# Makiato1999/HRI-EMO

Measured on AMD Instinct MI355X. Metric: utterances/sec fwd+bwd, d=768 T_a=400 T_t=128 N_e=6, higher is better.
Workload: dtype bf16; 1 GPU; FusionWithEmotionDecoder fwd+bwd (train mode, dropout 0.1), d=768 T_a=400 T_t=128 N_e=6 H=8, 2 fusion + 2 decoder layers, all-False masks (BASELINE cfg2); global_batch=64, batch_per_gpu=64, parallelism=dp1, grad_allreduce=none, launch=hipGraph replay, streams=2

## Files before the change

hri-emo_amd/__init__.py:

```python
from . import _lib
from .models.cross_modal_block_tacfn import CrossModalBlock, CrossModalTransformer
from .models.beta_gate_tacfn import BetaGate
from .models.emotion_decoder import EmotionDecoder, ExplainableDecoderLayer
from .models.fusion_with_emotion_decoder import FusionWithEmotionDecoder
from .models.mosei_fusion_with_emotion_decoder import MoseiFusionWithEmotionDecoder
from .models.fusion_classifier import FusionClassifier

from .dp import EvalStep
from ._ops import set_gemm_mode, gemm_mode, enable_fused_wgrad, set_precision, precision, set_varlen, varlen, set_varlen_maps, varlen_maps, set_mfma_maps, mfma_maps, set_ingest, ingest, set_pooled_gate_fp32, pooled_gate_fp32

__all__ = ["EvalStep", "set_gemm_mode", "gemm_mode", "enable_fused_wgrad", "set_precision", "precision", "set_varlen", "varlen", "set_varlen_maps", "varlen_maps", "set_mfma_maps", "mfma_maps", "set_ingest", "ingest", "set_pooled_gate_fp32", "pooled_gate_fp32", "CrossModalBlock", "CrossModalTransformer", "BetaGate", "EmotionDecoder", "ExplainableDecoderLayer",
           "FusionWithEmotionDecoder", "MoseiFusionWithEmotionDecoder", "FusionClassifier"]
```

hri-emo_amd/_lib.py:

```python
import ctypes
import os

_HERE = os.path.dirname(os.path.abspath(__file__))
LIB_PATH = os.environ.get("HRIEMO_LIB") or os.path.join(_HERE, "libhriemo.so")

_C = {"p": ctypes.c_void_p, "i": ctypes.c_int, "l": ctypes.c_long, "f": ctypes.c_float,
      "Q": ctypes.c_ulonglong, "I": ctypes.c_uint}

_SIGS = {
    "hriemo_gemm_bf16": ("iiiiiplplplipipliplp", "i"),
    "hriemo_gemm_force_config": ("i", "i"),
    "hriemo_gemm_debug_flags": ("i", "i"),
    "hriemo_gemm_colsum_rows": ("iiiii", "i"),
    "hriemo_gemm_plan": ("iiiiiilppp", "i"),
    "hriemo_gemm_bf16_group_tn": ("piip", "i"),
    "hriemo_gemm_bf16_split": ("iiiiiplplplpliiplp", "i"),
    "hriemo_gemm_bf16_colsum": ("iiiiiplplplplpp", "i"),
    "hriemo_mx8_scale_ld": ("i", "l"),
    "hriemo_quant_mx8": ("pliiiplplp", "i"),
    "hriemo_gemm_mx8": ("iiiplplplplplipiplp", "i"),
    "hriemo_gemm_mx8_q": ("iiiplplplplplpiplplp", "i"),
    "hriemo_gemm_mx8_force_config": ("i", "i"),
    "hriemo_attn_fwd": ("plplplplppiiiiifQpIipp", "i"),
    "hriemo_attn_fwd_q": ("plplplplppiiiiifQpIipplplp", "i"),
# ... 10 lines not shown
    "hriemo_attn_plan": ("iiiiiipppppp", "i"),
    "hriemo_split_bf16x3": ("pliipiip", "i"),
    "hriemo_attn_fwd_f32": ("plplplplppiiiiifQpIip", "i"),
    "hriemo_attn_probs_f32": ("plplpppiiiiifQpIip", "i"),
    "hriemo_add_ln_f32": ("ppppppiiffQpIlp", "i"),
    "hriemo_dropout_f32": ("ppliipfQpIlp", "i"),
    "hriemo_masked_mean_f32": ("pppiiip", "i"),
    "hriemo_gate_input_f32": ("pppiip", "i"),
    "hriemo_sigmoid_beta_f32": ("pppiip", "i"),
    "hriemo_fuse_f32": ("ppipippiiip", "i"),
    "hriemo_split3_f32": ("pliipiiplp", "i"),
    "hriemo_colsum_f32_workspace_bytes": ("ii", "l"),
    "hriemo_colsum_f32": ("pliiplpipp", "i"),
    "hriemo_add_ln_bwd_f32_workspace_bytes": ("ii", "l"),
    "hriemo_add_ln_bwd_f32": ("pppppppppiiiffQpIlpp", "i"),
    "hriemo_attn_bwd_f32": ("plplplplplppplplplpiiiiifQpIip", "i"),
    "hriemo_gate_dpre_f32": ("ppipipppiiip", "i"),
    "hriemo_gate_input_bwd_f32": ("pppppiip", "i"),
    "hriemo_gate_dy_f32": ("ppipppiiiip", "i"),
    "hriemo_rowdot_bwd_f32": ("ppppppiiip", "i"),
    "hriemo_attn_fwd_f32_varlen": ("plplplplpppiiiiifQpIip", "i"),
    "hriemo_attn_bwd_f32_varlen": ("plplplplplpppplplplpiiiiifQpIip", "i"),
    "hriemo_add_ln_f32_rows": ("ppppppiiffQpIlpp", "i"),
    "hriemo_add_ln_bwd_f32_rows": ("pppppppppiiiffQpIlppp", "i"),
    "hriemo_masked_mean_f32_packed": ("ppipiiip", "i"),
    "hriemo_fuse_f32_packed": ("pppiippiipppiiiip", "i"),
    "hriemo_gate_dpre_f32_packed": ("ppippiippiipppiiip", "i"),
    "hriemo_gate_dy_f32_packed": ("ppipippipiiiip", "i"),
    "hriemo_attn_probs": ("plplpppiiiiifQpIip", "i"),
    "hriemo_attn_probs_mfma": ("plplpppiiiiifQpIip", "i"),
    "hriemo_attn_probs_varlen": ("plplppppiiiiiiifQpIip", "i"),
    "hriemo_attn_probs_f32_varlen": ("plplppppiiiiiiifQpIip", "i"),
    "hriemo_add_ln_fwd": ("pppppppppiiffQpIlp", "i"),
    "hriemo_add_ln_fwd_mx8": ("pppppppppiiffQpIlpplp", "i"),
    "hriemo_add_ln_fwd_rows": ("pppppppppiiffQpIlpplpp", "i"),
    "hriemo_add_ln_bwd_rows": ("ppppppppppppiiifQpIlppp", "i"),
    "hriemo_add_ln_bwd_workspace_bytes": ("ii", "l"),
    "hriemo_add_ln_bwd": ("ppppppppppppiiifQpIlpp", "i"),
    "hriemo_colsum_workspace_bytes": ("ii", "l"),
    "hriemo_colsum_bf16": ("pliipipp", "i"),
    "hriemo_cast_f32_to_bf16": ("pplp", "i"),
    "hriemo_cast_bf16_to_f32": ("pplp", "i"),
    "hriemo_cast_f32_to_bf16_batch": ("pip", "i"),
    "hriemo_cast_copy_batch": ("pip", "i"),
    "hriemo_pack_rows": ("pppiiiipppp", "i"),
    "hriemo_unpack_rows": ("pppiiippp", "i"),
    "hriemo_ingest_rows": ("pilpiiiiipppplpp", "i"),
    "hriemo_seq_tables": ("ppiiiiippppppp", "i"),
    "hriemo_gather_rows": ("plppiplp", "i"),
    "hriemo_gather_rows_aug": ("piippipllQIiIIiIIfp", "i"),
    "hriemo_dropout_bf16": ("pplifQpIlp", "i"),
    "hriemo_gemm_ln_supported": ("i", "i"),
    "hriemo_gemm_ln_fwd": ("iiiplplppppppppppffQpIlpp", "i"),
    "hriemo_expand_rows": ("pppilp", "i"),
    "hriemo_seed_bump": ("pp", "i"),
    "hriemo_rowdot_fwd": ("pppppiip", "i"),
    "hriemo_rowdot_bwd": ("pppppppiiip", "i"),
    "hriemo_pool_chunks": ("i", "i"),
    "hriemo_ln_pool_fwd": ("pppppppppiiiifp", "i"),
    "hriemo_gate_input": ("ppppiiiipppp" + "p", "i"),
    "hriemo_sigmoid_beta": ("pppiip", "i"),
    "hriemo_fuse_fwd": ("ppppiiip", "i"),
    "hriemo_add_ln_bwd_partial_rows": ("ii", "i"),
    "hriemo_rowops_force_variant": ("i", "i"),
    "hriemo_colsum_partial_rows": ("ii", "i"),
    "hriemo_colreduce_batch": ("pipip", "i"),
    "hriemo_debug_hog": ("iipp", "i"),
    "hriemo_sumsq_f32": ("plpip", "i"),
    "hriemo_adamw_flat": ("pppplfffffifpp", "i"),
    "hriemo_optim_finalize": ("pippppp", "i"),
    "hriemo_adamw_flat_dev": ("pppplppp", "i"),
    "hriemo_grad_begin": ("plpp", "i"),
    "hriemo_optim_finalize_ctl": ("pipppppp", "i"),
    "hriemo_optim_finalize_groups": ("pipippppp", "i"),
    "hriemo_adamw_flat_groups": ("pppplppippip", "i"),
    "hriemo_optim_finalize_avg": ("pipippppppp", "i"),
    "hriemo_adamw_flat_dev_avg": ("pppplppppp", "i"),
    "hriemo_adamw_flat_groups_avg": ("pppplppippippp", "i"),
    "hriemo_swap_fp32": ("pplp", "i"),
    "hriemo_sumsq_units": ("plpipp", "i"),
    "hriemo_optim_finalize_units": ("pippipipppppppp", "i"),
    "hriemo_adamw_flat_units": ("pppplpppippipip", "i"),
    "hriemo_adamw_flat_units_avg": ("pppplpppippipippp", "i"),
    "hriemo_health_sweep": ("pppplpippipipp", "i"),
    "hriemo_health_fold": ("ppiipppiipp", "i"),
    "hriemo_act_probe_rows": ("", "i"),
    "hriemo_act_log_plan": ("iiiippppp", "i"),
    "hriemo_act_probe": ("piiilppiippiiiippp", "i"),
    "hriemo_act_log_fold": ("pppiiiipp", "i"),
    "hriemo_masked_mean_fwd": ("ppppiiip", "i"),
    "hriemo_rowsum_f32": ("ppilp", "i"),
    "hriemo_gate_input_pooled": ("pppiip", "i"),
    "hriemo_fusion_loss": ("ppppiiiffpppp", "i"),
    "hriemo_fusion_loss_ce": ("pppiiiffpppp", "i"),
    "hriemo_fusion_loss_n": ("ppppiiiffppppp", "i"),
    "hriemo_fusion_loss_ce_n": ("pppiiiffppppp", "i"),
    "hriemo_stats_update": ("ppppfpipiiippippp", "i"),
    "hriemo_predict_log": ("ppipiiipppipp", "i"),
    "hriemo_attn_log_plan": ("ppiipppp", "i"),
    "hriemo_attn_log_close": ("pp", "i"),
    "hriemo_attn_log_append": ("piippip", "i"),
    "hriemo_attn_probs_varlen_log": ("plplppppiiiiiiifQpIipip", "i"),
    "hriemo_attn_probs_varlen_log_fp32": ("plplppppiiiiiiifQpIipip", "i"),
    "hriemo_stats_counts": ("ppiippipp", "i"),
    "hriemo_stats_auc_tiles": ("i", "i"),
    "hriemo_stats_auc": ("ppiipppp", "i"),
    "hriemo_scalar_gate_dx":("pipippppiiip", "i"),
    "hriemo_fuse_bwd_dw": ("ppppiiip", "i"),
    "hriemo_gate_dpre": ("pippp" + "iip", "i"),
    "hriemo_gate_input_bwd": ("ppppppiip", "i"),
    "hriemo_ln_pool_bwd_chunks": ("i", "i"),
    "hriemo_ln_pool_pair_supported": ("i", "i"),
    "hriemo_ln_pool_fwd_pair": ("pppppppppi" * 2 + "iiifp", "i"),
    "hriemo_ln_pool_bwd_pair": ("pip" + "ppppppppppip" * 2 + "iiip", "i"),
    "hriemo_ln_pool_bwd_workspace_bytes": ("iii", "l"),
    "hriemo_ln_pool_bwd": ("pipipppppppppp" + "iiiipp", "i"),
    "hriemo_ln_pool2_fwd": ("p" * 9 + "iiiifp", "i"),
    "hriemo_ln_pool2_fwd_pair": (("p" * 9 + "i") * 2 + "iiifp", "i"),
    "hriemo_pooled_fuse_fwd": ("pipipipppiip", "i"),
    "hriemo_pooled_fuse_bwd": ("ppppipppiip", "i"),
    "hriemo_ln_pool_vec_bwd": ("pi" + "p" * 10 + "iiiipp", "i"),
    "hriemo_ln_pool_vec_bwd_pair": ("i" + ("p" * 11 + "ip") * 2 + "iiip", "i"),
    "hriemo_pool32_ln_fwd": ("pppppp" + "iiiifp", "i"),
    "hriemo_pool32_gate_input": ("ppippipppiip", "i"),
    "hriemo_pool32_ln_bwd_workspace_bytes": ("iii", "l"),
    "hriemo_pool32_ln_bwd": ("pippppppp" + "iiiifpp", "i"),
    "hriemo_ingest_padded": ("pilpiiiippp", "i"),
    "hriemo_ln_pool_fwd_packed": ("pppiippppppipiiifp", "i"),
    "hriemo_ln_pool_fwd_packed_pair": ("pppiippppppi" * 2 + "piiifp", "i"),
    "hriemo_fuse_fwd_packed": ("pppppiiiip", "i"),
    "hriemo_fuse_fwd_packed_q": ("pppppiiiipplp", "i"),
    "hriemo_fuse_bwd_dw_packed": ("pppppiiiip", "i"),
    "hriemo_ln_pool_bwd_packed": ("ppipippppiipppppp" + "iiiipp", "i"),
    "hriemo_ln_pool_bwd_packed_pair": ("ppip" + "ppppiippppppip" * 2 + "iiip", "i"),
    "hriemo_prof_enable": ("i", "i"),
    "hriemo_prof_nclass": ("", "i"),
    "hriemo_prof_collect": ("ippp", "i"),
    "hriemo_abi_version": ("", "i"),
}

_lib = None


def lib():
    global _lib
    if _lib is None:
        if not os.path.exists(LIB_PATH):
            raise RuntimeError(
                f"{LIB_PATH} not found: build it with `make -C hri-emo_amd/csrc` (or __graft_entry__.build()). "
                "There is no CPU/eager fallback for this path.")
        L = ctypes.CDLL(LIB_PATH)
        for name, (args, res) in _SIGS.items():
            fn = getattr(L, name)
            fn.argtypes = [_C[c] for c in args]
            fn.restype = _C[res]
        L.hriemo_last_error.restype = ctypes.c_char_p
        L.hriemo_last_error.argtypes = []
        L.hriemo_prof_name.restype = ctypes.c_char_p
        L.hriemo_prof_name.argtypes = [ctypes.c_int]
        _lib = L
    return _lib


def call(name, *args):
    L = lib()
    rc = getattr(L, name)(*args)
# ... 3 lines not shown
```

hri-emo_amd/_ops.py:

```python
import itertools
import os as _os
import threading
from collections import namedtuple

import torch

from . import _lib

BF16 = torch.bfloat16
_EPS = 1e-5
_apply_tls = threading.local()


def _stream():
    return torch.cuda.current_stream().cuda_stream


def _p(t):
    return None if t is None else t.data_ptr()


def _require_fp32_master(p):
    if p.dtype != torch.float32:
        raise TypeError(f"hri_emo_amd: parameter of dtype {p.dtype}; keep the module's parameters in fp32 "
                        "(the bf16 compute copies are made internally, as under torch.autocast)")


def _require_fp32_masters(*ps):
    for p in ps:
        if p is not None:
            _require_fp32_master(p)


def _require_gpu(t):
    if not t.is_cuda:
        raise RuntimeError(
            "hri_emo_amd runs on MI355X only: got a CPU tensor. There is no CPU fallback for this path "
            "(move the module and its inputs to 'cuda').")


_ws_cache = {}
_ws_retired = []
GRAPHS_ALIVE = 0


def workspace(nbytes, device, slot=0):
    key = (device.index, slot, torch.cuda.current_stream(device).cuda_stream)
    t = _ws_cache.get(key)
    if t is None or t.numel() * 4 < nbytes:
        if t is not None and GRAPHS_ALIVE > 0:
            _ws_retired.append(t)
        n = max(int(nbytes), 64 << 20) // 4 + 16
        t = torch.empty(n, dtype=torch.float32, device=device)
        _ws_cache[key] = t
    return t


_side_streams = {}
TWO_STREAMS = _os_env_flag = None


def side_stream(device):
    global TWO_STREAMS
    if TWO_STREAMS is None:
        import os
        TWO_STREAMS = os.environ.get("HRIEMO_TWO_STREAMS", "1") != "0"
    if not TWO_STREAMS:
        return None
    s = _side_streams.get(device.index)
    if s is None:
        s = torch.cuda.Stream(device=device)
        _side_streams[device.index] = s
    return s


class StepContext:
    __slots__ = ("capturing", "capture_origin", "seq_override", "join_scope", "half_reports", "stationary", "forms", "prologue",
                 "act_log")

    def __init__(self):
        self.capturing, self.capture_origin, self.seq_override, self.join_scope, self.half_reports = False, None, None, 0, {}
        self.stationary, self.forms, self.prologue = False, None, None
        self.act_log = None


CTX = StepContext()


class use_context:

    def __init__(self, ctx):
        self.ctx, self.prev = ctx, None

    def __enter__(self):
        global CTX
        self.prev, CTX = CTX, self.ctx
        return self.ctx

    def __exit__(self, *exc):
        global CTX
        CTX = self.prev
        return False


def probe(key, half, x, seq):
    log = CTX.act_log
    if log is None or not log.open[half]:
        return
    site = log.index.get(key)
    if site is not None:
        log.probe(site, half, x.detach(), seq)


def fork(child, parent):
    if CTX.capturing and CTX.capture_origin is not None and parent != CTX.capture_origin and child != CTX.capture_origin:
        raise RuntimeError("hri_emo_amd: a stream was forked from a stream that is itself a fork of the capture stream; ROCm 7.2 "
                           "crashes in hipStreamEndCapture on nested forks -- fork helper streams from the capturing stream only "
                           "(join the side stream back first), or run this step eagerly")
    child.wait_stream(parent)


_main_streams = {}


def note_main_stream(stream):
    _main_streams[stream.device.index] = stream


def branch_streams(device):
    out = [_main_streams.get(device.index, torch.cuda.current_stream(device))]
    side = _side_streams.get(device.index)
    if side is not None:
        out.append(side)
    return out


def share(t, stream):
    if t is not None:
        t.record_stream(stream)
    return t


class TextBranch:

    def __init__(self, side, main):
        self.side, self.main = side, main

    def fork(self, *handed):
        if self.side is not None:
            fork(self.side, self.main)
            for x in handed:
                share(x, self.side)

    def run(self):
        return torch.cuda.stream(self.side)

    def join(self, *back):
        if self.side is not None:
            self.main.wait_stream(self.side)
            for x in back:
                share(x, self.main)


_site_counter = itertools.count(1)


def new_site_base():
    return next(_site_counter) * 4


_seed_words = {}
STEP_ID = 0


def begin_step():
    global STEP_ID
    STEP_ID += 1
    CTX.half_reports.clear()

WEIGHTS_EPOCH = 0


def bump_weights_epoch():
    global WEIGHTS_EPOCH
    WEIGHTS_EPOCH += 1


def seed_word(device):
    t = _seed_words.get(device.index)
    if t is None:
        t = torch.zeros(1, dtype=torch.int64, device=device)
        _seed_words[device.index] = t
    return t


DROP_LOG = None
_ones = {}


def one(device):
    t = _ones.get(device.index)
    if t is None:
        t = _ones[device.index] = torch.ones((), dtype=torch.float32, device=device)
    return t


def _is_one(g):
    t = _ones.get(g.device.index) if g.is_cuda else None
    return t is not None and g.data_ptr() == t.data_ptr() and g.dim() == 0


def bump_seed_word(device):
    _lib.call("hriemo_seed_bump", _p(seed_word(device)), _stream())


def next_seed(training):
    if not training:
        return 0
    return int(torch.randint(0, 2 ** 62, (1,)).item())


def form_stale(ent, ver, device=None, once_per_step=True):
    fresh = ent is not None and ent[0] == ver and (device is None or ent[1].device == device)
    if not CTX.capturing:
        return not fresh
    if CTX.stationary:
        if not fresh:
            raise RuntimeError("hri_emo_amd: a weight form is stale inside the capture of a stationary step (internal error: the "
                               "weights pass should have refreshed it) -- no cast is recorded")
        return False
    return not once_per_step or not fresh or len(ent) < 3 or ent[2] != STEP_ID


class FormLog:

    def __init__(self):
        self.known, self.new = set(), []

    def take(self):
        new, self.new = self.new, []
        self.known.update(k for k, _, _ in new)
        return new


def _note_form(key, fn, *args):
    log = CTX.forms
    if log is not None and key not in log.known:
        log.new.append((key, fn, args))


class Shadows:

    def __init__(self):
        self._d = {}

    def get(self, p):
        key = id(p)
        _note_form(("get", id(self), key), self.get, p)
        ent = self._d.get(key)
        ver = (p._version, p.data_ptr(), WEIGHTS_EPOCH)
        if form_stale(ent, ver, p.device):
            s = ent[1] if ent is not None and ent[1].device == p.device and ent[1].shape == p.shape else \
                torch.empty(p.shape, dtype=BF16, device=p.device)
            _require_gpu(p)
            _require_fp32_master(p)
            src = p.detach()
            if not src.is_contiguous():
                src = src.contiguous()
            _lib.call("hriemo_cast_f32_to_bf16", _p(src), _p(s), src.numel(), _stream())
            ent = (ver, s, STEP_ID)
            self._d[key] = ent
        return ent[1]

    def prefetch(self, params):
        for p in params:
            self.get(p)

    def stale(self, p):
        ent = self._d.get(id(p))
        ver = (p._version, p.data_ptr(), WEIGHTS_EPOCH)
        need = form_stale(ent, ver, p.device)
        dst = ent[1] if ent is not None and ent[1].device == p.device and ent[1].shape == p.shape else None
        return need, dst, ver

    def get_cat(self, parts):
        key = ("cat",) + tuple((id(p), r0, r1) for p, r0, r1 in parts)
        _note_form(("get_cat", id(self), key), self.get_cat, parts)
        ent = self._d.get(key)
        ver = tuple((p._version, p.data_ptr()) for p, _, _ in parts) + (WEIGHTS_EPOCH,)
        dev = parts[0][0].device
        if form_stale(ent, ver, dev):
            rows = sum(r1 - r0 for _, r0, r1 in parts)
            K = parts[0][0].shape[1]
            s = ent[1] if ent is not None and ent[1].device == dev else torch.empty((rows, K), dtype=BF16, device=dev)
            at = 0
            for p, r0, r1 in parts:
                _require_gpu(p)
                _require_fp32_master(p)
                src = p.detach()
                if not src.is_contiguous():
                    src = src.contiguous()
                _lib.call("hriemo_cast_f32_to_bf16", _p(src[r0:r1]), _p(s[at:at + (r1 - r0)]), (r1 - r0) * K, _stream())
                at += r1 - r0
            ent = (ver, s, STEP_ID)
            self._d[key] = ent
        return ent[1]

    def get_cat_wb(self, wparts, bparts):
# ... 80 lines not shown


FUSED_WGRAD = True


def enable_fused_wgrad(params, on=True):
    for p in params:
        p._hriemo_fused_grad = bool(on)


class GradSink:

    def __init__(self, params):
        self.params = params
        self.fused = FUSED_WGRAD and all(
            getattr(p, "_hriemo_fused_grad", False)
            and p.grad is not None and p.grad.dtype == torch.float32 and p.grad.is_contiguous()
            and p.grad.device == p.device and p.grad.shape == p.shape for p in params)
        if self.fused:
            for p in params:
                if hasattr(p, "_hriemo_grad_ready"):
                    p._hriemo_sink_managed = True

    def buf(self, p):
        return p.grad if self.fused else torch.empty(p.shape, dtype=torch.float32, device=p.device)

    def ret(self, t):
        return None if self.fused else t

    def done(self, skip=(), after_flush=()):
        if self.fused:
            for p in self.params:
                if any(p is q for q in skip):
                    continue
                hook = getattr(p, "_hriemo_grad_ready", None)
                if hook is not None:
                    if (p.dim() < 2 or any(p is q for q in after_flush)) and _small_dw.touches(p.grad):
                        _small_dw.add_hook(hook, p, True)
                    elif (p.dim() < 2 or any(p is q for q in after_flush)) and DEFER_REDUCE and _in_backward():
                        _deferred.add_hook(hook, p)
                    elif p.dim() >= 2 and _small_dw.touches(p.grad):
                        _small_dw.add_hook(hook, p)
                    else:
                        hook(p)


def prefetch_batch(pairs):
    _note_form(("prefetch_batch",) + tuple((id(sh), id(p)) for sh, p in pairs), prefetch_batch, pairs)
    jobs, upd = [], []
    for sh, p in pairs:
        need, dst, ver = sh.stale(p)
        if not need:
            continue
        _require_gpu(p)
        _require_fp32_master(p)
        if not p.is_contiguous() or p.data_ptr() % 16:
            sh.get(p)
            continue
        if dst is None:
            dst = torch.empty(p.shape, dtype=BF16, device=p.device)
        jobs.append((p.data_ptr(), dst.data_ptr(), p.numel()))
        upd.append((sh, id(p), ver, dst))
    if jobs:
        host = torch.tensor(jobs, dtype=torch.int64)
        _lib.call("hriemo_cast_f32_to_bf16_batch", host.data_ptr(), len(jobs), _stream())
        for sh, key, ver, dst in upd:
            sh._d[key] = (ver, dst, STEP_ID)


def padded_shadow(sh, p, kp):
    key = (id(p), "pad")
    _note_form(("padded_shadow", id(sh), key), padded_shadow, sh, p, kp)
    ent = sh._d.get(key)
    ver = (p._version, p.data_ptr(), WEIGHTS_EPOCH)
    if form_stale(ent, ver, p.device, once_per_step=False):
        _require_gpu(p)
        _require_fp32_master(p)
        s_ = ent[1] if ent is not None and ent[1].device == p.device else \
            torch.zeros((p.shape[0], kp), dtype=BF16, device=p.device)
        s_[:, :p.shape[1]].copy_(p.detach())
        ent = (ver, s_)
        sh._d[key] = ent
    return ent[1]


def to_bf16(x):
    return x if x.dtype == BF16 else x.to(BF16)


def mask_u8(mask, B, L):
    if mask is None:
        return None
    if mask.shape != (B, L):
        raise ValueError(f"key_padding_mask shape {tuple(mask.shape)} != {(B, L)}")
    m = mask.contiguous()
    return m.view(torch.uint8) if m.dtype == torch.bool else m.to(torch.uint8)


def gemm(ta, tb, M, N, K, A, lda, B, ldb, C, ldc, c_f32=False, bias=None, epi=0, aux=None, ldaux=0, accumulate=False):
    ws = workspace(64 << 20, C.device) if c_f32 else None
    _lib.call("hriemo_gemm_bf16", ta, tb, M, N, K, _p(A), lda, _p(B), ldb, _p(C), ldc, int(c_f32), _p(bias), epi,
              _p(aux), ldaux, int(accumulate), _p(ws), ws.numel() * 4 if ws is not None else 0, _stream())


def linear_fwd(x, w16, bias, relu=False, out_f32=False):
    M, K = x.shape
    N = w16.shape[0]
    y = torch.empty((M, N), dtype=torch.float32 if out_f32 else BF16, device=x.device)
    gemm(0, 0, M, N, K, x, x.stride(0), w16, w16.stride(0), y, N, c_f32=out_f32, bias=bias, epi=1 if relu else 0)
    return y


def linear_dx(dy, w16, epi=0, aux=None):
    M, N = dy.shape
    K = w16.shape[1]
    dx = torch.empty((M, K), dtype=BF16, device=dy.device)
    gemm(0, 1, M, K, N, dy, dy.stride(0), w16, w16.stride(0), dx, K, epi=epi, aux=aux,
         ldaux=aux.stride(0) if aux is not None else 0)
    return dx


FOLD_FFN_BIAS = True


def fold_ffn_bias():
    return FOLD_FFN_BIAS


def linear_dx_masked_colsum(dy, w16, aux, bias_out, accumulate):
    M, N = dy.shape
    K = w16.shape[1]
    dx = torch.empty((M, K), dtype=BF16, device=dy.device)
    rows = _lib.lib().hriemo_gemm_colsum_rows(0, 1, M, K, N)
    part = torch.empty(rows * K, dtype=torch.float32, device=dy.device)
    _lib.call("hriemo_gemm_bf16_colsum", 0, 1, M, K, N, _p(dy), dy.stride(0), _p(w16), w16.stride(0), _p(dx), K, _p(aux), aux.stride(0),
              _p(part), _stream())
    if accumulate and DEFER_REDUCE and _in_backward():
        _deferred.add(part, K, rows, K, 1, [bias_out], True)
    else:
        red = _DeferredReduce()
        red.device = dy.device
        red.add(part, K, rows, K, 1, [bias_out], accumulate, schedule=False)
        red.flush()
    return dx


def linear_dw(dy, x, out, accumulate=False):
    M, N = dy.shape
    K = x.shape[1]
    if accumulate and M <= SMALL_DW_ROWS and _small_dw.enabled():
        _small_dw.add(dy, x, out)
        return
    gemm(1, 1, N, K, M, dy, dy.stride(0), x, x.stride(0), out, out.stride(0), c_f32=True, accumulate=accumulate)


def linear_dw_split(dy, x, out, out2, split, accumulate=False):
    M, N = dy.shape
    K = x.shape[1]
    ws = workspace(64 << 20, out.device)
    _lib.call("hriemo_gemm_bf16_split", 1, 1, N, K, M, _p(dy), dy.stride(0), _p(x), x.stride(0), _p(out), out.stride(0), _p(out2),
              out2.stride(0), split, int(accumulate), _p(ws), ws.numel() * 4, _stream())


GEMM_MODE = None


# ... 2118 lines not shown
```

hri-emo_amd/csrc/optim.hip:

```cpp
#include "common.h"

enum { HY_LR = 0, HY_BETA1, HY_BETA2, HY_EPS, HY_WD, HY_MAX_NORM };
enum { ST_STEP = 0, ST_SKIP, ST_COEF, ST_STEP_SIZE, ST_ISB2, ST_DECAY, ST_GRAD_NORM, ST_SKIPPED };
enum { CTL_N_VALID = 0, CTL_FIRST, CTL_LAST };
enum { AG_MAX_GROUPS = 16, AG_MAX_SEGS = 2048 };
enum { AH_MODE = 0, AH_DECAY, AH_START, AH_EVERY };
enum { AS_N = 0, AS_W, AS_FLAG, AS_STAMP };
enum { AV_NONE = 0, AV_UPDATE = 1, AV_FIRST = 2, AV_EMA = 1, AV_SWA = 2 };

template <bool HOLD>
__global__ __launch_bounds__(256) void optim_finalize_kernel(const float* __restrict__ partial, int nblocks, const float* __restrict__ hyper,
                                                             const float* __restrict__ grad_scale, const float* __restrict__ found_inf,
                                                             float* __restrict__ state, const int* __restrict__ ctl) {
  __shared__ float red[4];
  if (HOLD && ctl[CTL_LAST] == 0) {
    if (threadIdx.x == 0) state[ST_SKIP] = 1.f;
    return;
  }
  float s = 0.f;
  for (int i = threadIdx.x; i < nblocks; i += 256) s += partial[i];
  s = wave_sum(s);
  if ((threadIdx.x & 63) == 0) red[threadIdx.x >> 6] = s;
  __syncthreads();
  if (threadIdx.x != 0) return;
  const float sum = red[0] + red[1] + red[2] + red[3];
  const float gs = grad_scale != nullptr ? grad_scale[0] : 1.f;
  const float norm = sqrtf(sum) / gs;
  const bool finite = (__float_as_uint(norm) & 0x7f800000u) != 0x7f800000u;
  const bool skip = !finite || (found_inf != nullptr && !(found_inf[0] == 0.f));
  state[ST_GRAD_NORM] = norm;
  if (skip) {
    state[ST_SKIP] = 1.f;
    state[ST_SKIPPED] += 1.f;
    return;
  }
  const float lr = hyper[HY_LR], b1 = hyper[HY_BETA1], b2 = hyper[HY_BETA2], wd = hyper[HY_WD], max_norm = hyper[HY_MAX_NORM];
  const float step = state[ST_STEP] + 1.f;
  const float bc1 = 1.f - powf(b1, step), bc2 = 1.f - powf(b2, step);
  float coef = 1.f;
  if (max_norm > 0.f) coef = fminf(1.f, max_norm / (norm + 1e-6f));
  state[ST_STEP] = step;
  state[ST_SKIP] = 0.f;
  state[ST_COEF] = coef / gs;
  state[ST_STEP_SIZE] = lr / bc1;
  state[ST_ISB2] = 1.f / sqrtf(bc2);
  state[ST_DECAY] = 1.f - lr * wd;
}

struct AdamScalars { float b1, b2, eps, coef, step, isb2, decay; };

__device__ __forceinline__ f32x4 adamw_vec4(float* __restrict__ p, const float* __restrict__ g, float* __restrict__ m, float* __restrict__ v,
                                           long i, const AdamScalars& s) {
  const float b1 = s.b1, b2 = s.b2, eps = s.eps, coef = s.coef, step = s.step, isb2 = s.isb2, decay = s.decay;
  f32x4 pp = *(const f32x4*)(p + i * 4), mm = *(const f32x4*)(m + i * 4), vv = *(const f32x4*)(v + i * 4);
  const f32x4 gg = *(const f32x4*)(g + i * 4) * coef;
#pragma unroll
  for (int e = 0; e < 4; ++e) {
    pp[e] *= decay;
    mm[e] += (gg[e] - mm[e]) * (1.f - b1);
    vv[e] = vv[e] * b2 + gg[e] * gg[e] * (1.f - b2);
    pp[e] -= step * mm[e] / (sqrtf(vv[e]) * isb2 + eps);
  }
  *(f32x4*)(p + i * 4) = pp; *(f32x4*)(m + i * 4) = mm; *(f32x4*)(v + i * 4) = vv;
  return pp;
}

struct AvgStep { int kind; float w; };

__device__ __forceinline__ AvgStep avg_step(const float* __restrict__ state, const float* __restrict__ avg_state) {
  const float flag = avg_state[AS_FLAG];
  AvgStep a = {AV_NONE, 0.f};
  if (avg_state[AS_STAMP] == state[ST_STEP] && (flag == (float)AV_UPDATE || flag == (float)AV_FIRST)) {
    a.kind = flag == (float)AV_FIRST ? AV_FIRST : AV_UPDATE;
    a.w = avg_state[AS_W];
  }
  return a;
}

__device__ __forceinline__ void avg_vec4(float* __restrict__ avg, long i, const f32x4 pp, const AvgStep a) {
  if (a.kind == AV_FIRST) {
    *(f32x4*)(avg + i * 4) = pp;
    return;
  }
  f32x4 aa = *(const f32x4*)(avg + i * 4);
#pragma unroll
  for (int e = 0; e < 4; ++e) aa[e] = __builtin_fmaf(a.w, pp[e] - aa[e], aa[e]);
  *(f32x4*)(avg + i * 4) = aa;
}

template <bool AVG>
__device__ __forceinline__ void adamw_flat_dev_body(float* __restrict__ p, const float* __restrict__ g, float* __restrict__ m,
                                                    float* __restrict__ v, long n, const float* __restrict__ hyper,
                                                    const float* __restrict__ state, float* __restrict__ avg,
                                                    const float* __restrict__ avg_state) {
  if (state[ST_SKIP] != 0.f) return;
  const AdamScalars s = {hyper[HY_BETA1], hyper[HY_BETA2], hyper[HY_EPS], state[ST_COEF], state[ST_STEP_SIZE], state[ST_ISB2], state[ST_DECAY]};
  const long nv = n >> 2;
  if (AVG) {
    const AvgStep a = avg_step(state, avg_state);
    if (a.kind != AV_NONE) {
      for (long i = (long)blockIdx.x * 256 + threadIdx.x; i < nv; i += (long)gridDim.x * 256) avg_vec4(avg, i, adamw_vec4(p, g, m, v, i, s), a);
      return;
    }
  }
  for (long i = (long)blockIdx.x * 256 + threadIdx.x; i < nv; i += (long)gridDim.x * 256) adamw_vec4(p, g, m, v, i, s);
}

__global__ __launch_bounds__(256) void adamw_flat_dev_kernel(float* __restrict__ p, const float* __restrict__ g, float* __restrict__ m,
                                                             float* __restrict__ v, long n, const float* __restrict__ hyper,
                                                             const float* __restrict__ state) {
  adamw_flat_dev_body<false>(p, g, m, v, n, hyper, state, nullptr, nullptr);
}

__global__ __launch_bounds__(256) void adamw_flat_dev_avg_kernel(float* __restrict__ p, const float* __restrict__ g, float* __restrict__ m,
                                                                 float* __restrict__ v, long n, const float* __restrict__ hyper,
                                                                 const float* __restrict__ state, float* __restrict__ avg,
                                                                 const float* __restrict__ avg_state) {
  adamw_flat_dev_body<true>(p, g, m, v, n, hyper, state, avg, avg_state);
}

struct ClipUnits {
  const int* __restrict__ unit_chunks;
  const int* __restrict__ unit_group;
  int U;
  float* __restrict__ clip_state;
};

__device__ __forceinline__ float wave_min(float v) {
#pragma unroll
  for (int o = 32; o >= 1; o >>= 1) v = fminf(v, __shfl_xor(v, o));
  return v;
}

template <bool AVG, bool UNITS>
__device__ __forceinline__ void optim_finalize_groups_body(const float* __restrict__ partial, int nblocks, const float* __restrict__ hyper,
                                                           int G, const float* __restrict__ grad_scale,
                                                           const float* __restrict__ found_inf, float* __restrict__ state,
                                                           const int* __restrict__ ctl, const float* __restrict__ avg_hyper,
                                                           float* __restrict__ avg_state, const ClipUnits units) {
  __shared__ float red[4];
  extern __shared__ float unit_sum[];
  if (ctl != nullptr && ctl[CTL_LAST] == 0) {
    if (threadIdx.x == 0) state[ST_SKIP] = 1.f;
    return;
  }
  const float step = state[ST_STEP] + 1.f;
  if (UNITS) {
    constexpr int UF = 8, UW = 8;
    const int lane = threadIdx.x & 63;
    for (int u0 = (threadIdx.x >> 6) * UF; u0 < units.U; u0 += 4 * UF) {
      int c1[UF], c[UF];
      float a[UF];
#pragma unroll
      for (int k = 0; k < UF; ++k) {
        const int u = u0 + k < units.U ? u0 + k : units.U - 1;
        int lo = units.unit_chunks[u], hi = units.unit_chunks[u + 1];
        lo = lo < 0 ? 0 : (lo > nblocks ? nblocks : lo);
        hi = hi < lo ? lo : (hi > nblocks ? nblocks : hi);
        c[k] = lo + lane; c1[k] = hi;
      }
#pragma unroll
      for (int k = 0; k < UF; ++k) {
        a[k] = c[k] < c1[k] ? partial[c[k]] : 0.f;
        c[k] += 64;
      }
#pragma unroll
      for (int k = 0; k < UF; ++k)
        for (; c[k] < c1[k]; c[k] += 64 * UW) {
          float x[UW];
#pragma unroll
          for (int j = 0; j < UW; ++j) x[j] = c[k] + 64 * j < c1[k] ? partial[c[k] + 64 * j] : 0.f;
#pragma unroll
          for (int j = 0; j < UW; ++j) a[k] += x[j];
        }
#pragma unroll
      for (int k = 0; k < UF; ++k) a[k] = wave_sum(a[k]);
      if (lane == 0) {
#pragma unroll
        for (int k = 0; k < UF; ++k)
          if (u0 + k < units.U) unit_sum[u0 + k] = a[k];
      }
    }
    __syncthreads();
  }
  const float* __restrict__ terms = UNITS ? unit_sum : partial;
  const int nterms = UNITS ? units.U : nblocks;
  float s = 0.f;
  for (int i = threadIdx.x; i < nterms; i += 256) s += terms[i];
  s = wave_sum(s);
  if ((threadIdx.x & 63) == 0) red[threadIdx.x >> 6] = s;
  __syncthreads();
  const int grp = threadIdx.x;
  if (!UNITS && grp >= G) return;
  const float sum = red[0] + red[1] + red[2] + red[3];
  const float gs = grad_scale != nullptr ? grad_scale[0] : 1.f;
  const float norm = sqrtf(sum) / gs;
  const bool finite = (__float_as_uint(norm) & 0x7f800000u) != 0x7f800000u;
  const bool skip = !finite || (found_inf != nullptr && !(found_inf[0] == 0.f));
  float min_coef = 0.f;
  if (UNITS) {
    float lo = __builtin_inff();
// ... 22 lines not shown
  if (skip) {
    if (grp == 0) {
      state[ST_SKIP] = 1.f;
      state[ST_SKIPPED] += 1.f;
    }
    return;
  }
  const float* hy = hyper + grp * 8;
  float* stg = state + grp * 8;
  const float lr = hy[HY_LR], b1 = hy[HY_BETA1], b2 = hy[HY_BETA2], wd = hy[HY_WD], max_norm = hyper[HY_MAX_NORM];
  const float bc1 = 1.f - powf(b1, step), bc2 = 1.f - powf(b2, step);
  if (grp == 0) {
    float coef = 1.f;
    if (max_norm > 0.f) coef = fminf(1.f, max_norm / (norm + 1e-6f));
    state[ST_STEP] = step;
    state[ST_SKIP] = 0.f;
    state[ST_COEF] = UNITS ? min_coef : coef / gs;
  }
  stg[ST_STEP_SIZE] = lr / bc1;
  stg[ST_ISB2] = 1.f / sqrtf(bc2);
  stg[ST_DECAY] = 1.f - lr * wd;
  if (AVG && grp == 0) {
    const float mode = avg_hyper[AH_MODE], since = step - avg_hyper[AH_START];
    float flag = (float)AV_NONE;
    if ((mode == (float)AV_EMA || mode == (float)AV_SWA) && since > 0.f && fmodf(since, avg_hyper[AH_EVERY]) == 0.f) {
      const float n_avg = avg_state[AS_N];
      flag = n_avg == 0.f ? (float)AV_FIRST : (float)AV_UPDATE;
      avg_state[AS_W] = mode == (float)AV_EMA ? 1.f - avg_hyper[AH_DECAY] : 1.f / (n_avg + 1.f);
      avg_state[AS_N] = n_avg + 1.f;
    }
    avg_state[AS_FLAG] = flag;
    avg_state[AS_STAMP] = step;
  }
}

__global__ __launch_bounds__(256) void optim_finalize_groups_kernel(const float* __restrict__ partial, int nblocks, const float* __restrict__ hyper,
                                                                    int G, const float* __restrict__ grad_scale,
                                                                    const float* __restrict__ found_inf, float* __restrict__ state,
                                                                    const int* __restrict__ ctl) {
  optim_finalize_groups_body<false, false>(partial, nblocks, hyper, G, grad_scale, found_inf, state, ctl, nullptr, nullptr, ClipUnits{});
}

__global__ __launch_bounds__(256) void optim_finalize_avg_kernel(const float* __restrict__ partial, int nblocks, const float* __restrict__ hyper,
                                                                 int G, const float* __restrict__ grad_scale,
                                                                 const float* __restrict__ found_inf, float* __restrict__ state,
                                                                 const int* __restrict__ ctl, const float* __restrict__ avg_hyper,
                                                                 float* __restrict__ avg_state) {
  optim_finalize_groups_body<true, false>(partial, nblocks, hyper, G, grad_scale, found_inf, state, ctl, avg_hyper, avg_state, ClipUnits{});
}

template <bool AVG>
__global__ __launch_bounds__(256) void optim_finalize_units_kernel(const float* __restrict__ partial, int C, const int* __restrict__ unit_chunks,
                                                                   const int* __restrict__ unit_group, int U, const float* __restrict__ hyper,
                                                                   int G, const float* __restrict__ grad_scale,
                                                                   const float* __restrict__ found_inf, float* __restrict__ state,
                                                                   const int* __restrict__ ctl, float* __restrict__ clip_state,
                                                                   const float* __restrict__ avg_hyper, float* __restrict__ avg_state) {
  const ClipUnits units = {unit_chunks, unit_group, U, clip_state};
  optim_finalize_groups_body<AVG, true>(partial, C, hyper, G, grad_scale, found_inf, state, ctl, avg_hyper, avg_state, units);
}

__global__ __launch_bounds__(256) void sumsq_units_kernel(const float* __restrict__ g, long n, const long long* __restrict__ chunks,
                                                          float* __restrict__ partial) {
  __shared__ float red[4];
  const long long* row = chunks + (long)blockIdx.x * 4;
  long long start = row[0], len = row[1];
  start = (start < 0 ? 0 : (start > n ? n : start)) & ~3LL;
  len = (len < 0 ? 0 : (len > n - start ? n - start : len)) & ~3LL;
  const long nv = (long)(len >> 2);
  const float* gb = g + start;
  float s = 0.f;
#pragma unroll 4
  for (long i = threadIdx.x; i < nv; i += 256) {
    const f32x4 t = *(const f32x4*)(gb + i * 4);
#pragma unroll
    for (int e = 0; e < 4; ++e) s = __builtin_fmaf(t[e], t[e], s);
  }
  s = wave_sum(s);
  if ((threadIdx.x & 63) == 0) red[threadIdx.x >> 6] = s;
  __syncthreads();
  if (threadIdx.x == 0) partial[blockIdx.x] = ((red[0] + red[1]) + red[2]) + red[3];
}

template <bool AVG, bool UNITS>
__device__ __forceinline__ void adamw_flat_groups_body(float* __restrict__ p, const float* __restrict__ g, float* __restrict__ m,
                                                       float* __restrict__ v, long n, const long long* __restrict__ seg,
                                                       const int* __restrict__ seg_group, int S, const float* __restrict__ hyper,
                                                       const float* __restrict__ state, int G, float* __restrict__ avg,
                                                       const float* __restrict__ avg_state, const int* __restrict__ seg_unit,
                                                       const float* __restrict__ clip_state, int U) {
  if (state[ST_SKIP] != 0.f) return;
  AvgStep a = {AV_NONE, 0.f};
  if (AVG) a = avg_step(state, avg_state);
  extern __shared__ __attribute__((aligned(16))) long long ag_lds[];
  long long* segb = ag_lds;
  float* sc = (float*)(segb + (S + 1));
  float* uc = sc + G * 8;
  unsigned short* su = (unsigned short*)(uc + (UNITS ? U : 0));
  unsigned char* sg = (unsigned char*)(su + (UNITS ? S : 0));
  for (int i = threadIdx.x; i <= S; i += 256) {
    segb[i] = seg[i];
    if (i < S) {
      const int q = seg_group[i];
      sg[i] = (unsigned char)(q < 0 ? 0 : (q >= G ? G - 1 : q));
      if (UNITS) {
        const int w = seg_unit[i];
        su[i] = (unsigned short)(w < 0 ? 0 : (w >= U ? U - 1 : w));
      }
    }
  }
  if (UNITS)
    for (int u = threadIdx.x; u < U; u += 256) uc[u] = clip_state[2 * u + 1];
  if (threadIdx.x < G) {
    const float* hy = hyper + threadIdx.x * 8;
    const float* stg = state + threadIdx.x * 8;
    float* o = sc + threadIdx.x * 8;
    o[0] = hy[HY_BETA1]; o[1] = hy[HY_BETA2]; o[2] = hy[HY_EPS]; o[3] = state[ST_COEF];
    o[4] = stg[ST_STEP_SIZE]; o[5] = stg[ST_ISB2]; o[6] = stg[ST_DECAY]; o[7] = 0.f;
  }
  __syncthreads();
  AdamScalars s = {0.f, 0.f, 0.f, 0.f, 0.f, 0.f, 0.f};
  long long cur_lo = 0, cur_hi = 0;
  const long nv = n >> 2;
  for (long i = (long)blockIdx.x * 256 + threadIdx.x; i < nv; i += (long)gridDim.x * 256) {
    const long long x = (long long)i * 4;
    if (x < cur_lo || x >= cur_hi) {
      int lo = 1, hi = S;
      while (lo < hi) {
        const int mid = (lo + hi) >> 1;
        if (segb[mid] > x) hi = mid; else lo = mid + 1;
      }
      cur_lo = segb[lo - 1]; cur_hi = segb[lo];
      const float* o = sc + (int)sg[lo - 1] * 8;
      s.b1 = o[0]; s.b2 = o[1]; s.eps = o[2]; s.coef = UNITS ? uc[su[lo - 1]] : o[3]; s.step = o[4]; s.isb2 = o[5]; s.decay = o[6];
    }
    const f32x4 pp = adamw_vec4(p, g, m, v, i, s);
    if (AVG && a.kind != AV_NONE) avg_vec4(avg, i, pp, a);
  }
}

__global__ __launch_bounds__(256) void adamw_flat_groups_kernel(float* __restrict__ p, const float* __restrict__ g, float* __restrict__ m,
                                                                float* __restrict__ v, long n, const long long* __restrict__ seg,
                                                                const int* __restrict__ seg_group, int S, const float* __restrict__ hyper,
                                                                const float* __restrict__ state, int G) {
  adamw_flat_groups_body<false, false>(p, g, m, v, n, seg, seg_group, S, hyper, state, G, nullptr, nullptr, nullptr, nullptr, 0);
}

__global__ __launch_bounds__(256) void adamw_flat_groups_avg_kernel(float* __restrict__ p, const float* __restrict__ g, float* __restrict__ m,
                                                                    float* __restrict__ v, long n, const long long* __restrict__ seg,
                                                                    const int* __restrict__ seg_group, int S, const float* __restrict__ hyper,
                                                                    const float* __restrict__ state, int G, float* __restrict__ avg,
                                                                    const float* __restrict__ avg_state) {
  adamw_flat_groups_body<true, false>(p, g, m, v, n, seg, seg_group, S, hyper, state, G, avg, avg_state, nullptr, nullptr, 0);
}

template <bool AVG>
__global__ __launch_bounds__(256) void adamw_flat_units_kernel(float* __restrict__ p, const float* __restrict__ g, float* __restrict__ m,
                                                               float* __restrict__ v, long n, const long long* __restrict__ seg,
                                                               const int* __restrict__ seg_group, const int* __restrict__ seg_unit, int S,
                                                               const float* __restrict__ hyper, const float* __restrict__ state, int G,
                                                               const float* __restrict__ clip_state, int U, float* __restrict__ avg,
                                                               const float* __restrict__ avg_state) {
  adamw_flat_groups_body<AVG, true>(p, g, m, v, n, seg, seg_group, S, hyper, state, G, avg, avg_state, seg_unit, clip_state, U);
}

typedef __attribute__((ext_vector_type(4))) unsigned u32x4;

__global__ __launch_bounds__(256) void swap_fp32_kernel(float* __restrict__ a, float* __restrict__ b, long n) {
  const long nv = n >> 2;
  for (long i = (long)blockIdx.x * 256 + threadIdx.x; i < nv; i += (long)gridDim.x * 256) {
    const u32x4 x = *(const u32x4*)(a + i * 4), y = *(const u32x4*)(b + i * 4);
    *(u32x4*)(a + i * 4) = y; *(u32x4*)(b + i * 4) = x;
  }
}

__global__ __launch_bounds__(256) void grad_begin_kernel(float* __restrict__ flat, long n, const int* __restrict__ ctl) {
  if (ctl[CTL_FIRST] == 0) return;
  const long nv = n >> 2;
  const f32x4 zero = {0.f, 0.f, 0.f, 0.f};
  for (long i = (long)blockIdx.x * 256 + threadIdx.x; i < nv; i += (long)gridDim.x * 256) *(f32x4*)(flat + i * 4) = zero;
}

extern "C" int hriemo_grad_begin(float* flat, long n, const int* ctl, hipStream_t st) {
  HRIEMO_CHECK(flat != nullptr && n > 0 && n % 4 == 0, "grad_begin: n=%ld must be a positive multiple of 4", n);
  HRIEMO_CHECK(((uintptr_t)flat % 16) == 0, "grad_begin: unaligned buffer");
  HRIEMO_CHECK(ctl != nullptr && ((uintptr_t)ctl % 4) == 0, "grad_begin: ctl is the int32 step-control block in device memory");
  long gsz = (n / 4 + 255) / 256;
  if (gsz > 4096) gsz = 4096;
  hipLaunchKernelGGL(grad_begin_kernel, dim3((int)gsz), dim3(256), 0, st, flat, n, ctl);
  HRIEMO_LAUNCH_CHECK("grad_begin_kernel");
  return 0;
}

extern "C" int hriemo_optim_finalize(const float* partial, int nblocks, const float* hyper, const float* grad_scale, const float* found_inf,
                                     float* state, hipStream_t st) {
  HRIEMO_CHECK(partial != nullptr && hyper != nullptr && state != nullptr, "optim_finalize: partial, hyper and state are required");
  HRIEMO_CHECK(nblocks > 0 && nblocks <= 4096, "optim_finalize: nblocks=%d out of range (1..4096)", nblocks);
  hipLaunchKernelGGL(optim_finalize_kernel<false>, dim3(1), dim3(256), 0, st, partial, nblocks, hyper, grad_scale, found_inf, state,
                     (const int*)nullptr);
  HRIEMO_LAUNCH_CHECK("optim_finalize_kernel");
  return 0;
}

extern "C" int hriemo_optim_finalize_ctl(const float* partial, int nblocks, const float* hyper, const float* grad_scale,
                                         const float* found_inf, float* state, const int* ctl, hipStream_t st) {
  HRIEMO_CHECK(partial != nullptr && hyper != nullptr && state != nullptr, "optim_finalize_ctl: partial, hyper and state are required");
  HRIEMO_CHECK(nblocks > 0 && nblocks <= 4096, "optim_finalize_ctl: nblocks=%d out of range (1..4096)", nblocks);
  HRIEMO_CHECK(ctl != nullptr && ((uintptr_t)ctl % 4) == 0, "optim_finalize_ctl: ctl is the int32 step-control block in device memory");
  hipLaunchKernelGGL(optim_finalize_kernel<true>, dim3(1), dim3(256), 0, st, partial, nblocks, hyper, grad_scale, found_inf, state, ctl);
  HRIEMO_LAUNCH_CHECK("optim_finalize_kernel<hold>");
  return 0;
}

extern "C" int hriemo_adamw_flat_dev(float* p, const float* g, float* m, float* v, long n, const float* hyper, const float* state,
                                     hipStream_t st) {
  HRIEMO_CHECK(n > 0 && n % 4 == 0, "adamw_flat_dev: n=%ld must be a positive multiple of 4", n);
  HRIEMO_CHECK(((uintptr_t)p % 16) == 0 && ((uintptr_t)g % 16) == 0 && ((uintptr_t)m % 16) == 0 && ((uintptr_t)v % 16) == 0,
               "adamw_flat_dev: unaligned buffer");
  HRIEMO_CHECK(hyper != nullptr && state != nullptr, "adamw_flat_dev: hyper and state are required");
  long gsz = (n / 4 + 255) / 256;
  if (gsz > 4096) gsz = 4096;
  hipLaunchKernelGGL(adamw_flat_dev_kernel, dim3((int)gsz), dim3(256), 0, st, p, g, m, v, n, hyper, state);
  HRIEMO_LAUNCH_CHECK("adamw_flat_dev_kernel");
  return 0;
}

extern "C" int hriemo_optim_finalize_groups(const float* partial, int nblocks, const float* hyper, int G, const float* grad_scale,
                                            const float* found_inf, float* state, const int* ctl, hipStream_t st) {
  HRIEMO_CHECK(partial != nullptr && hyper != nullptr && state != nullptr, "optim_finalize_groups: partial, hyper and state are required");
  HRIEMO_CHECK(nblocks > 0 && nblocks <= 4096, "optim_finalize_groups: nblocks=%d out of range (1..4096)", nblocks);
  HRIEMO_CHECK(G >= 1 && G <= AG_MAX_GROUPS, "optim_finalize_groups: G=%d groups (1 .. %d)", G, (int)AG_MAX_GROUPS);
  HRIEMO_CHECK(((uintptr_t)ctl % 4) == 0, "optim_finalize_groups: ctl is the int32 step-control block in device memory (or NULL)");
  hipLaunchKernelGGL(optim_finalize_groups_kernel, dim3(1), dim3(256), 0, st, partial, nblocks, hyper, G, grad_scale, found_inf, state, ctl);
  HRIEMO_LAUNCH_CHECK("optim_finalize_groups_kernel");
  return 0;
}

extern "C" int hriemo_adamw_flat_groups(float* p, const float* g, float* m, float* v, long n, const long long* seg, const int* seg_group,
                                        int S, const float* hyper, const float* state, int G, hipStream_t st) {
  HRIEMO_CHECK(n > 0 && n % 4 == 0, "adamw_flat_groups: n=%ld must be a positive multiple of 4", n);
  HRIEMO_CHECK(p != nullptr && g != nullptr && m != nullptr && v != nullptr, "adamw_flat_groups: p, g, m and v are required");
  HRIEMO_CHECK(((uintptr_t)p % 16) == 0 && ((uintptr_t)g % 16) == 0 && ((uintptr_t)m % 16) == 0 && ((uintptr_t)v % 16) == 0,
               "adamw_flat_groups: unaligned buffer");
  HRIEMO_CHECK(hyper != nullptr && state != nullptr, "adamw_flat_groups: hyper and state are required");
  HRIEMO_CHECK(G >= 1 && G <= AG_MAX_GROUPS, "adamw_flat_groups: G=%d groups (1 .. %d)", G, (int)AG_MAX_GROUPS);
  HRIEMO_CHECK(S >= 1 && S <= AG_MAX_SEGS, "adamw_flat_groups: S=%d segments (1 .. %d)", S, (int)AG_MAX_SEGS);
// ... 100 lines not shown
  HRIEMO_CHECK(G >= 1 && G <= AG_MAX_GROUPS, "optim_finalize_units: G=%d groups (1 .. %d)", G, (int)AG_MAX_GROUPS);
  HRIEMO_CHECK(unit_chunks != nullptr && unit_group != nullptr && ((uintptr_t)unit_chunks % 4) == 0 && ((uintptr_t)unit_group % 4) == 0,
               "optim_finalize_units: unit_chunks (int32 [U + 1]) and unit_group (int32 [U]) are required, 4-byte aligned");
  HRIEMO_CHECK(clip_state != nullptr && ((uintptr_t)clip_state % 4) == 0, "optim_finalize_units: clip_state (fp32 [U][2]) is required, 4-byte aligned");
  HRIEMO_CHECK(((uintptr_t)ctl % 4) == 0, "optim_finalize_units: ctl is the int32 step-control block in device memory (or NULL)");
  HRIEMO_CHECK((avg_hyper == nullptr) == (avg_state == nullptr) && ((uintptr_t)avg_hyper % 4) == 0 && ((uintptr_t)avg_state % 4) == 0,
               "optim_finalize_units: avg_hyper and avg_state (fp32 [4] each, device memory) come together or not at all");
  const size_t cb = (size_t)U * 8;
  HRIEMO_CHECK(!spans_overlap(clip_state, cb, partial, (size_t)C * 4) && !spans_overlap(clip_state, cb, state, (size_t)G * 32) &&
                   !spans_overlap(clip_state, cb, hyper, (size_t)G * 32) && !spans_overlap(clip_state, cb, unit_chunks, (size_t)(U + 1) * 4) &&
                   !spans_overlap(clip_state, cb, unit_group, (size_t)U * 4),
               "optim_finalize_units: clip_state overlaps partial, state, hyper, unit_chunks or unit_group");
  const size_t lds = (size_t)U * sizeof(float);
  if (avg_hyper != nullptr)
    hipLaunchKernelGGL(optim_finalize_units_kernel<true>, dim3(1), dim3(256), lds, st, partial, C, unit_chunks, unit_group, U, hyper, G,
                       grad_scale, found_inf, state, ctl, clip_state, avg_hyper, avg_state);
  else
    hipLaunchKernelGGL(optim_finalize_units_kernel<false>, dim3(1), dim3(256), lds, st, partial, C, unit_chunks, unit_group, U, hyper, G,
                       grad_scale, found_inf, state, ctl, clip_state, avg_hyper, avg_state);
  HRIEMO_LAUNCH_CHECK("optim_finalize_units_kernel");
  return 0;
}

static int adamw_flat_units_launch(const char* who, float* p, const float* g, float* m, float* v, long n, const long long* seg,
                                   const int* seg_group, const int* seg_unit, int S, const float* hyper, const float* state, int G,
                                   const float* clip_state, int U, float* avg, const float* avg_state, hipStream_t st) {
  HRIEMO_CHECK(n > 0 && n % 4 == 0, "%s: n=%ld must be a positive multiple of 4", who, n);
  HRIEMO_CHECK(p != nullptr && g != nullptr && m != nullptr && v != nullptr, "%s: p, g, m and v are required", who);
  HRIEMO_CHECK(((uintptr_t)p % 16) == 0 && ((uintptr_t)g % 16) == 0 && ((uintptr_t)m % 16) == 0 && ((uintptr_t)v % 16) == 0 &&
                   ((uintptr_t)avg % 16) == 0, "%s: unaligned buffer", who);
  HRIEMO_CHECK(hyper != nullptr && state != nullptr, "%s: hyper and state are required", who);
  HRIEMO_CHECK(G >= 1 && G <= AG_MAX_GROUPS, "%s: G=%d groups (1 .. %d)", who, G, (int)AG_MAX_GROUPS);
  HRIEMO_CHECK(S >= 1 && S <= AG_MAX_SEGS, "%s: S=%d segments (1 .. %d)", who, S, (int)AG_MAX_SEGS);
  HRIEMO_CHECK(U >= 1 && U <= CU_MAX_UNITS, "%s: U=%d units (1 .. %d)", who, U, (int)CU_MAX_UNITS);
  HRIEMO_CHECK(U <= S, "%s: U=%d units over S=%d segments: every unit owns at least one segment", who, U, S);
  HRIEMO_CHECK((long)S <= n / 4, "%s: S=%d segments over n=%ld elements: more segments than 16-byte vectors", who, S, n);
  HRIEMO_CHECK(seg != nullptr && seg_group != nullptr && seg_unit != nullptr,
               "%s: seg (int64 [S + 1]), seg_group and seg_unit (int32 [S]) are required", who);
  HRIEMO_CHECK(((uintptr_t)seg % 8) == 0, "%s: seg (int64 [S + 1]) is not 8-byte aligned", who);
  HRIEMO_CHECK(((uintptr_t)seg_group % 4) == 0 && ((uintptr_t)seg_unit % 4) == 0, "%s: seg_group / seg_unit (int32 [S]) is not 4-byte aligned", who);
  HRIEMO_CHECK(clip_state != nullptr && ((uintptr_t)clip_state % 4) == 0, "%s: clip_state (fp32 [U][2]) is required, 4-byte aligned", who);
  long gsz = (n / 4 + 255) / 256;
  if (gsz > 4096) gsz = 4096;
  const size_t lds = (size_t)(S + 1) * sizeof(long long) + (size_t)G * 8 * sizeof(float) + (size_t)U * sizeof(float) + (size_t)S * 2 + (size_t)S;
  if (avg != nullptr) {
    HRIEMO_CHECK(avg_state != nullptr, "%s: avg_state is required", who);
    HRIEMO_CHECK(!ranges_overlap(avg, p, (size_t)n * 4) && !ranges_overlap(avg, g, (size_t)n * 4) && !ranges_overlap(avg, m, (size_t)n * 4) &&
                     !ranges_overlap(avg, v, (size_t)n * 4), "%s: avg overlaps p, g, m or v", who);
    hipLaunchKernelGGL(adamw_flat_units_kernel<true>, dim3((int)gsz), dim3(256), lds, st, p, g, m, v, n, seg, seg_group, seg_unit, S, hyper, state,
                       G, clip_state, U, avg, avg_state);
  } else {
    hipLaunchKernelGGL(adamw_flat_units_kernel<false>, dim3((int)gsz), dim3(256), lds, st, p, g, m, v, n, seg, seg_group, seg_unit, S, hyper, state,
                       G, clip_state, U, (float*)nullptr, (const float*)nullptr);
  }
  HRIEMO_LAUNCH_CHECK("adamw_flat_units_kernel");
  return 0;
}

extern "C" int hriemo_adamw_flat_units(float* p, const float* g, float* m, float* v, long n, const long long* seg, const int* seg_group,
                                       const int* seg_unit, int S, const float* hyper, const float* state, int G, const float* clip_state,
                                       int U, hipStream_t st) {
  return adamw_flat_units_launch("adamw_flat_units", p, g, m, v, n, seg, seg_group, seg_unit, S, hyper, state, G, clip_state, U, nullptr,
                                 nullptr, st);
}

extern "C" int hriemo_adamw_flat_units_avg(float* p, const float* g, float* m, float* v, long n, const long long* seg, const int* seg_group,
                                           const int* seg_unit, int S, const float* hyper, const float* state, int G,
                                           const float* clip_state, int U, float* avg, const float* avg_state, hipStream_t st) {
  HRIEMO_CHECK(avg != nullptr, "adamw_flat_units_avg: avg is required");
  return adamw_flat_units_launch("adamw_flat_units_avg", p, g, m, v, n, seg, seg_group, seg_unit, S, hyper, state, G, clip_state, U, avg,
                                 avg_state, st);
}

extern "C" int hriemo_swap_fp32(float* a, float* b, long n, hipStream_t st) {
  HRIEMO_CHECK(n > 0 && n % 4 == 0, "swap_fp32: n=%ld must be a positive multiple of 4", n);
  HRIEMO_CHECK(a != nullptr && b != nullptr && ((uintptr_t)a % 16) == 0 && ((uintptr_t)b % 16) == 0, "swap_fp32: two 16-byte aligned buffers are required");
  HRIEMO_CHECK(!ranges_overlap(a, b, (size_t)n * 4), "swap_fp32: the buffers overlap (or are one buffer)");
  long gsz = (n / 4 + 255) / 256;
  if (gsz > 4096) gsz = 4096;
  hipLaunchKernelGGL(swap_fp32_kernel, dim3((int)gsz), dim3(256), 0, st, a, b, n);
  HRIEMO_LAUNCH_CHECK("swap_fp32_kernel");
  return 0;
}
```

hri-emo_amd/csrc/rowops.hip:

```cpp
#include "common.h"
#include <string.h>
#include <stdlib.h>

#define EPS_DEFAULT 1e-5f

struct RowDrop { uint64_t seed; const unsigned long long* seed_dev; uint32_t site, thr16; float inv_keep; const long long* rowmap; };
static RowDrop row_drop(float p, uint64_t seed, const unsigned long long* seed_dev, uint32_t site) {
  DropCfg d = make_drop(p, seed, site);
  RowDrop r; r.seed = seed; r.seed_dev = seed_dev; r.site = site; r.thr16 = d.thr16; r.inv_keep = d.inv_keep; r.rowmap = nullptr;
  return r;
}
__device__ __forceinline__ uint32_t row_key(const RowDrop& dr) {
  return dr.thr16 != 0 ? site_key(eff_seed(dr.seed, dr.seed_dev), dr.site, 0u) : 0u;
}

template <int NCH>
__device__ __forceinline__ void block_colsum(float* lds_row, const float (&acc)[NCH][8], int nchunk, int lane, int wave, int nwave) {
  for (int w = 0; w < nwave; ++w) {
    if (wave == w) {
#pragma unroll
      for (int c = 0; c < NCH; ++c) {
        const int ch = lane + 64 * c;
        if (ch < nchunk) {
#pragma unroll
          for (int j = 0; j < 8; ++j) {
            if (w == 0) lds_row[ch * 8 + j] = acc[c][j];
            else lds_row[ch * 8 + j] += acc[c][j];
          }
        }
      }
    }
    __syncthreads();
  }
}

__device__ __forceinline__ void row_keep8(uint32_t key32, uint32_t thr16, uint32_t row, int ch, bool (&kp)[8]) {
  if (thr16 == 0) {
#pragma unroll
    for (int j = 0; j < 8; ++j) kp[j] = true;
    return;
  }
  const uint32_t hb = drop_base(key32, row, (uint32_t)(ch * 4));
#pragma unroll
  for (int pr = 0; pr < 4; ++pr) {
    const uint32_t x = mix24(hb + (uint32_t)pr * DROP_CB);
    kp[2 * pr] = keep_lo(x, thr16);
    kp[2 * pr + 1] = keep_hi(x, thr16);
  }
}

__device__ __forceinline__ void load_resid(const bf16_t* X, const float* X32, long off, float* xf) {
  if (X32 != nullptr) {
    const f32x4 a = *(const f32x4*)(X32 + off), b = *(const f32x4*)(X32 + off + 4);
    xf[0] = a[0]; xf[1] = a[1]; xf[2] = a[2]; xf[3] = a[3]; xf[4] = b[0]; xf[5] = b[1]; xf[6] = b[2]; xf[7] = b[3];
  } else if (X != nullptr) {
    bf8_to_f32(*(const bf16x8*)(X + off), xf);
  } else {
#pragma unroll
    for (int j = 0; j < 8; ++j) xf[j] = 0.f;
  }
}

template <int NCH>
__device__ __forceinline__ void load_cols(const float* __restrict__ v, int nchunk, int lane, float (&out)[NCH][8]) {
#pragma unroll
  for (int c = 0; c < NCH; ++c) {
    const int ch = lane + 64 * c;
#pragma unroll
    for (int j = 0; j < 8; ++j) out[c][j] = 0.f;
    if (ch < nchunk) {
      const f32x4 a = *(const f32x4*)(v + ch * 8), b = *(const f32x4*)(v + ch * 8 + 4);
#pragma unroll
      for (int e = 0; e < 4; ++e) { out[c][e] = a[e]; out[c][4 + e] = b[e]; }
    }
  }
}

template <int NCH>
__global__ __launch_bounds__(256) void add_ln_fwd_kernel(const bf16_t* __restrict__ G, const bf16_t* __restrict__ X,
                                                         const float* __restrict__ X32, const float* __restrict__ gamma,
                                                         const float* __restrict__ beta, bf16_t* __restrict__ Y,
                                                         float* __restrict__ Y32, float* __restrict__ mean_o,
                                                         float* __restrict__ rstd_o, int M, int d, float eps, RowDrop dr,
// ... 1953 lines not shown
  for (int l = wave; l < L; l += 4) {
    const bool valid = mask == nullptr || mask[(long)b * L + l] == 0;
    if (lane == 0 && valid) c += 1.f;
    if (valid && ch < nchunk) {
      const bf16x8 v = *(const bf16x8*)(X + ((long)b * L + l) * d + ch * 8);
#pragma unroll
      for (int j = 0; j < 8; ++j) acc[j] += (float)v[j];
    }
  }
#pragma unroll
  for (int j = 0; j < 8; ++j) red[wave][lane][j] = acc[j];
  if (lane == 0) cred[wave] = c;
  __syncthreads();
  if (wave == 0) {
    const float n = fmaxf(cred[0] + cred[1] + cred[2] + cred[3], 1.f);
    if (ch < nchunk) {
#pragma unroll
      for (int j = 0; j < 8; ++j)
        pooled[(long)b * d + ch * 8 + j] = (red[0][lane][j] + red[1][lane][j] + red[2][lane][j] + red[3][lane][j]) / n;
    }
    if (lane == 0 && blockIdx.x == 0) cnt[b] = n;
  }
}

__global__ __launch_bounds__(256) void rowsum_f32_kernel(const float* __restrict__ x, float* __restrict__ out, long n) {
  __shared__ float red[4];
  const int b = blockIdx.x;
  float s = 0.f;
  for (long i = threadIdx.x; i < n; i += 256) s += x[(long)b * n + i];
  s = wave_sum(s);
  if ((threadIdx.x & 63) == 0) red[threadIdx.x >> 6] = s;
  __syncthreads();
  if (threadIdx.x == 0) out[b] = red[0] + red[1] + red[2] + red[3];
}

__global__ void scalar_gate_dx_kernel(const bf16_t* __restrict__ dH, int Lf, const float* __restrict__ beta, int is_a,
                                      const float* __restrict__ dpool, const float* __restrict__ cnt, const uint8_t* __restrict__ mask,
                                      bf16_t* __restrict__ dX, int B, int L, int d) {
  const int nch = d >> 3;
  const long nv = (long)B * L * nch;
  for (long v = (long)blockIdx.x * blockDim.x + threadIdx.x; v < nv; v += (long)gridDim.x * blockDim.x) {
    const int ch = (int)(v % nch);
    const long row = v / nch;
    const int b = (int)(row / L), l = (int)(row - (long)b * L);
    const float coef = is_a ? beta[b] : 1.f - beta[b];
    const bool valid = mask == nullptr || mask[row] == 0;
    const float ic = valid ? 1.f / cnt[b] : 0.f;
    float o[8];
#pragma unroll
    for (int j = 0; j < 8; ++j) o[j] = ic * dpool[(long)b * d + ch * 8 + j];
    if (l < Lf) {
      const bf16x8 g = *(const bf16x8*)(dH + ((long)b * Lf + l) * d + ch * 8);
#pragma unroll
      for (int j = 0; j < 8; ++j) o[j] += coef * (float)g[j];
    }
    *(bf16x8*)(dX + row * d + ch * 8) = f32_to_bf8(o);
  }
}

__global__ __launch_bounds__(256) void gate_input_pooled_kernel(const float* __restrict__ a_pool, const float* __restrict__ t_pool,
                                                                bf16_t* __restrict__ gin, int d) {
  const int b = blockIdx.x;
  bf16_t* g = gin + (long)b * 4 * d;
  for (int c = threadIdx.x; c < d; c += 256) {
    const float a = a_pool[(long)b * d + c], t = t_pool[(long)b * d + c];
    g[c] = (bf16_t)a; g[d + c] = (bf16_t)t; g[2 * d + c] = (bf16_t)fabsf(a - t); g[3 * d + c] = (bf16_t)(a * t);
  }
}

__global__ __launch_bounds__(256) void sumsq_f32_kernel(const float* __restrict__ x, long n, float* __restrict__ partial) {
  __shared__ float red[4];
  float s = 0.f;
  const long nv = n >> 2;
  for (long v = (long)blockIdx.x * 256 + threadIdx.x; v < nv; v += (long)gridDim.x * 256) {
    const f32x4 t = *(const f32x4*)(x + v * 4);
    s += t[0] * t[0] + t[1] * t[1] + t[2] * t[2] + t[3] * t[3];
  }
  s = wave_sum(s);
  if ((threadIdx.x & 63) == 0) red[threadIdx.x >> 6] = s;
  __syncthreads();
  if (threadIdx.x == 0) partial[blockIdx.x] = red[0] + red[1] + red[2] + red[3];
}

__global__ __launch_bounds__(256) void adamw_flat_kernel(float* __restrict__ p, const float* __restrict__ g, float* __restrict__ m,
                                                         float* __restrict__ v, long n, float lr, float b1, float b2, float eps,
                                                         float wd, float bc1, float bc2, float max_norm, const float* __restrict__ norm2) {
  float coef = 1.f;
  if (max_norm > 0.f) coef = fminf(1.f, max_norm / (sqrtf(norm2[0]) + 1e-6f));
  const float step = lr / bc1, isb2 = 1.f / sqrtf(bc2);
  const long nv = n >> 2;
  for (long i = (long)blockIdx.x * 256 + threadIdx.x; i < nv; i += (long)gridDim.x * 256) {
    f32x4 pp = *(const f32x4*)(p + i * 4), mm = *(const f32x4*)(m + i * 4), vv = *(const f32x4*)(v + i * 4);
    const f32x4 gg = *(const f32x4*)(g + i * 4) * coef;
#pragma unroll
    for (int e = 0; e < 4; ++e) {
      pp[e] *= 1.f - lr * wd;
      mm[e] += (gg[e] - mm[e]) * (1.f - b1);
      vv[e] = vv[e] * b2 + gg[e] * gg[e] * (1.f - b2);
      pp[e] -= step * mm[e] / (sqrtf(vv[e]) * isb2 + eps);
    }
    *(f32x4*)(p + i * 4) = pp; *(f32x4*)(m + i * 4) = mm; *(f32x4*)(v + i * 4) = vv;
  }
}

extern "C" int hriemo_sumsq_f32(const float* x, long n, float* partial, int nblocks, hipStream_t st) {
  HRIEMO_CHECK(n > 0 && n % 4 == 0 && nblocks > 0 && nblocks <= 4096, "sumsq_f32: n=%ld must be a positive multiple of 4, 0 < nblocks <= 4096", n);
  HRIEMO_CHECK(((uintptr_t)x % 16) == 0, "sumsq_f32: unaligned buffer");
  hipLaunchKernelGGL(sumsq_f32_kernel, dim3(nblocks), dim3(256), 0, st, x, n, partial);
  HRIEMO_LAUNCH_CHECK("sumsq_f32_kernel");
  return 0;
}

extern "C" int hriemo_adamw_flat(float* p, const float* g, float* m, float* v, long n, float lr, float beta1, float beta2, float eps,
                                 float weight_decay, int step, float max_norm, const float* norm2, hipStream_t st) {
  HRIEMO_CHECK(n > 0 && n % 4 == 0 && step >= 1, "adamw_flat: n=%ld must be a positive multiple of 4 and step >= 1", n);
  HRIEMO_CHECK(((uintptr_t)p % 16) == 0 && ((uintptr_t)g % 16) == 0 && ((uintptr_t)m % 16) == 0 && ((uintptr_t)v % 16) == 0, "adamw_flat: unaligned buffer");
  HRIEMO_CHECK(max_norm <= 0.f || norm2 != nullptr, "adamw_flat: clipping needs the squared gradient norm");
  const float bc1 = 1.f - powf(beta1, (float)step), bc2 = 1.f - powf(beta2, (float)step);
  long gsz = (n / 4 + 255) / 256;
  if (gsz > 4096) gsz = 4096;
  hipLaunchKernelGGL(adamw_flat_kernel, dim3((int)gsz), dim3(256), 0, st, p, g, m, v, n, lr, beta1, beta2, eps, weight_decay, bc1, bc2,
                     max_norm, norm2);
  HRIEMO_LAUNCH_CHECK("adamw_flat_kernel");
  return 0;
}

#define LAUNCH_PF(KERNEL, N, ...)                                         \
  if ((N) <= 2) hipLaunchKernelGGL((KERNEL<N, ((N) <= 2)>), __VA_ARGS__); \
  else hipLaunchKernelGGL((KERNEL<N, false>), __VA_ARGS__)
#define LAUNCH_PAIR(D, K1, K2, ...) \
  if ((D) <= 512) hipLaunchKernelGGL(K1, __VA_ARGS__); else hipLaunchKernelGGL(K2, __VA_ARGS__)

extern "C" int hriemo_ln_pool_pair_supported(int d) { return d % 8 == 0 && d <= 1024 ? 1 : 0; }
static int check_pair_width(const char* who, int d) {
  HRIEMO_CHECK(hriemo_ln_pool_pair_supported(d), "%s: d=%d (pairs are built for d <= 1024; use two hriemo_%.*s calls)", who, d, (int)strlen(who) - 5, who);
  return 0;
}
static int check_pair_bwd(const char* who, int d, const float* ws_a, const float* ws_t, const float* dgamma_a, const float* dbeta_a,
                          const float* dgamma_t, const float* dbeta_t) {
  HRIEMO_CHECK(ws_a != nullptr && ws_t != nullptr && ws_a != ws_t, "%s: bad arguments", who);
  if (check_pair_width(who, d)) return 1;
  HRIEMO_CHECK((dgamma_a == nullptr) == (dbeta_a == nullptr) && (dgamma_t == nullptr) == (dbeta_t == nullptr) && (dgamma_a == nullptr) == (dgamma_t == nullptr),
               "%s: the four LayerNorm gradients come together or not at all", who);
  return 0;
}
static int reduce_affine(float* ws, int B, int nc, int d, float* dgamma, float* dbeta, int accumulate, hipStream_t st) {
  if (dgamma == nullptr) return 0;
  ReduceOut ro; ro.o[0] = dgamma; ro.o[1] = dbeta; ro.o[2] = nullptr;
  launch_colreduce(ws, (long)2 * d, B * nc, ro, d, 2, accumulate, ws + (long)B * nc * 2 * d, st);
  HRIEMO_LAUNCH_CHECK("colreduce_kernel");
  return 0;
}

extern "C" int hriemo_pool_chunks(int L) { return (L + 31) / 32; }

extern "C" int hriemo_ln_pool_fwd(const void* X, const float* X32, const unsigned char* mask, const float* gamma, const float* beta, void* Yn,
                                  float* mean, float* rstd, float* partials, int B, int L, int Lkeep, int d, float eps,
                                  hipStream_t st) {
  if (check_rows(B * L, d)) return 1;
  HRIEMO_CHECK(Lkeep >= 0 && Lkeep <= L, "ln_pool_fwd: Lkeep=%d out of range (L=%d)", Lkeep, L);
  const int nc = (L + 31) / 32;
  hriemo_prof_begin(HP_ROWOPS, st);
#define CALL(N) LAUNCH_PF(ln_pool_fwd_kernel, N, dim3(nc, B), dim3(256), d * 4, st, (const bf16_t*)X, X32, mask, gamma, beta, (bf16_t*)Yn, mean, rstd, partials, L, Lkeep, d, eps)
  DISPATCH_NCH(d, CALL)
#undef CALL
  HRIEMO_LAUNCH_CHECK("ln_pool_fwd_kernel");
  hriemo_prof_end(HP_ROWOPS, st, ((double)B * L + (double)B * Lkeep) * d * 2);
  return 0;
}

extern "C" int hriemo_ln_pool_fwd_pair(const void* Xa, const float* Xa32, const unsigned char* mask_a, const float* gamma_a, const float* beta_a,
                                       void* Yna, float* mean_a, float* rstd_a, float* partials_a, int La,
                                       const void* Xt, const float* Xt32, const unsigned char* mask_t, const float* gamma_t, const float* beta_t,
                                       void* Ynt, float* mean_t, float* rstd_t, float* partials_t, int Lt,
                                       int B, int Lkeep, int d, float eps, hipStream_t st) {
  if (check_rows(B * La, d) || check_rows(B * Lt, d)) return 1;
  HRIEMO_CHECK(Lkeep >= 0 && Lkeep <= La && Lkeep <= Lt, "ln_pool_fwd_pair: Lkeep=%d out of range (La=%d, Lt=%d)", Lkeep, La, Lt);
  if (check_pair_width("ln_pool_fwd_pair", d)) return 1;
  PoolFwdPair p;
  p.s[0] = PoolFwdSide{(const bf16_t*)Xa, Xa32, mask_a, gamma_a, beta_a, (bf16_t*)Yna, mean_a, rstd_a, partials_a, La, Lkeep, (La + 31) / 32};
  p.s[1] = PoolFwdSide{(const bf16_t*)Xt, Xt32, mask_t, gamma_t, beta_t, (bf16_t*)Ynt, mean_t, rstd_t, partials_t, Lt, Lkeep, (Lt + 31) / 32};
  const int nc = p.s[0].nc + p.s[1].nc;
  hriemo_prof_begin(HP_ROWOPS, st);
  LAUNCH_PAIR(d, (ln_pool_fwd_pair_kernel<1, true>), (ln_pool_fwd_pair_kernel<2, true>), dim3(nc, B), dim3(256), d * 4, st, p, d, eps);
  HRIEMO_LAUNCH_CHECK("ln_pool_fwd_pair_kernel");
  hriemo_prof_end(HP_ROWOPS, st, ((double)B * (La + Lt) + 2.0 * B * Lkeep) * d * 2);
  return 0;
}

extern "C" int hriemo_gate_input(const float* partials_a, const float* partials_t, const unsigned char* mask_a,
                                 const unsigned char* mask_t, int B, int La, int Lt, int d, void* gate_in, float* a_pool,
                                 float* t_pool, float* cnt, hipStream_t st) {
  HRIEMO_CHECK(B > 0 && d > 0, "gate_input: empty");
  hipLaunchKernelGGL(gate_input_kernel, dim3(B), dim3(256), 0, st, partials_a, (La + 31) / 32, partials_t, (Lt + 31) / 32, mask_a,
                     mask_t, La, Lt, d, (bf16_t*)gate_in, a_pool, t_pool, cnt);
  HRIEMO_LAUNCH_CHECK("gate_input_kernel");
  return 0;
}

extern "C" int hriemo_sigmoid_beta(const float* pre, float* w, float* beta, int B, int d, hipStream_t st) {
  HRIEMO_CHECK(B > 0 && d > 0, "sigmoid_beta: empty");
  hipLaunchKernelGGL(sigmoid_beta_kernel, dim3(B), dim3(256), 0, st, pre, w, beta, d);
  HRIEMO_LAUNCH_CHECK("sigmoid_beta_kernel");
  return 0;
}

// ... 327 lines not shown
```

hri-emo_amd/dp.py:

```python
import collections
import itertools
import logging
import os

import torch
import torch.distributed as dist

log = logging.getLogger("hri_emo_amd.dp")

_VARLEN_BUCKETS = max(1, int(os.environ.get("HRIEMO_VARLEN_BUCKETS", "64")))
_VARLEN_MAX_GRAPHS = max(1, int(os.environ.get("HRIEMO_VARLEN_MAX_GRAPHS", "48")))


def bucket_rows(n, B, L):
    g = max(8, (B * L) // _VARLEN_BUCKETS // 8 * 8)
    g = min(g, L)
    return (n // g + 1) * g


def packed_tables(la, lt, B, La, Lt):
    key = (bucket_rows(sum(la), B, La), bucket_rows(sum(lt), B, Lt))
    cu = lambda lens, rows: list(itertools.accumulate(lens, initial=0)) + [rows]
    return key, cu(la, key[0]), cu(lt, key[1]), cu([min(x, y) for x, y in zip(la, lt)], key[1])

# ... 439 lines not shown
        return self._pb is not None and len(self._pb.graphs) > 0

    @property
    def _replaying(self):
        return self._replay and self.captured

    @property
    def store(self):
        return None if self._feed is None else self._feed.store

    def _packed_graph(self, key):
        return self._pb.graph(key, self.max_graphs if self.max_graphs is not None else _VARLEN_MAX_GRAPHS, self._capture_bucket, self._label)

    def _release_buckets(self):
        if self._pb is not None and self._pb.graphs:
            torch.cuda.synchronize()
            for rec in self._pb.graphs.values():
                rec.release()
        if self._feed is not None:
            self._feed.close()
            self._feed = None

    def _need_forward_packed(self, who):
        if not hasattr(self.model, "_forward_rows"):
            raise TypeError(f"{who}: the model has no forward_packed entry")

    def _need_n_valid(self, who):
        if not _accepts_n_valid(self.loss_fn):
            raise TypeError(f"{who}: loss_fn takes no n_valid= keyword -- the ghost utterances of a short batch must stay out of "
                            "the loss (hri_emo_amd.train's losses accept it)")

    def _store_capture(self, who, store, ids, pad_to, targets=True):
        from .data import DeviceFeatureStore
        if not isinstance(store, DeviceFeatureStore):
            raise TypeError(f"{who}: store is a data.DeviceFeatureStore")
        ids = store.check_ids(ids)
        dev = next(self.model.parameters()).device
        if store.device != dev:
            raise ValueError(f"{who}: the store lives on {store.device}, the model on {dev}")
        La, Lt = (int(v) for v in (pad_to if pad_to is not None else store.pad_to))
        if Lt > La:
            raise RuntimeError(f"{who}: L_t={Lt} > L_a={La}: the gate fuses over the text length and needs L_a >= L_t")
        if not hasattr(self.model, "audio_proj") and store.widths[0] != store.widths[1]:
            raise ValueError(f"{who}: the store's rows differ in width {store.widths}")
        la, lt = _store_batch(store, ids, (La, Lt), who)
        y_static = torch.zeros((len(ids),) + tuple(store.y.shape[1:]), dtype=store.y.dtype, device=dev) if targets else None
        return ids, la, lt, (La, Lt), y_static

    def _capture_ragged(self, begin, widths, dtype, y_static, la, lt, pad, load, store=None, partial=True, accum=1, ctl=True, augment=None):
        from . import _ops
        _ops._require_gpu(next(self.model.parameters()))
        begin()
        self._pb, self._static = _ragged_state(self.model, len(la), pad, widths, dtype, y_static, partial, accum, ctl)
        try:
            if store is not None:
                self._feed = _StoreFeed(store, len(la), pad, self._static[0].device, augment)
            self._packed_graph(load())
        except BaseException:
            self.release_graph()
            raise

    def _check_batch(self, who, rows_a, rows_t, n, y):
        B, sy = self._pb.B, self._static[4]
        _check_count(who, n, B, self._pb.front.partial)
        for name, rows, src in (("rows_a", rows_a, self._static[0]), ("rows_t", rows_t, self._static[1])):
            if rows.shape[1] != src.shape[1] or rows.dtype != src.dtype:
                raise ValueError(f"{who}: {name} of width {rows.shape[1]} / {rows.dtype}; captured with width {src.shape[1]} / {src.dtype}")
        if sy is not None:
            want = (n,) + tuple(sy.shape[1:])
            if tuple(y.shape) != want:
                raise ValueError(f"{who}: targets of shape {tuple(y.shape)}; captured with {tuple(sy.shape)}"
                                 + (f", this batch needs {want}" if n != B else ""))

    def _load_packed(self, rows_a, rows_t, la, lt, y, ctl=None):
        return _load_ragged(self._pb, self._static, _caller_rows(rows_a, rows_t, y), la, lt, ctl)

    def _load_store(self, ids, la, lt, ctl=None):
        return _load_ragged(self._pb, self._static, self._feed.fill(ids, self._static[4] is not None), la, lt, ctl)


class DataParallelStep(_RaggedStep):

    _label = "packed step"

    def __init__(self, model, loss_fn, group=None, bucket_bytes=32 << 20, overlap=True, comm_dtype=torch.float32, force_exchange=False,
                 launch_from="notify", force_queue=None):
        super().__init__(model, loss_fn)
        self.force_queue = force_queue
        self._exchange_in_graph = False
        self.rank = dist.get_rank(group) if dist.is_initialized() else 0
        self.world = dist.get_world_size(group) if dist.is_initialized() else 1
        self.buckets = GradBuckets(model.parameters(), bucket_bytes, group, overlap, comm_dtype, force_exchange, launch_from)
        self._record = None
        self._mask_seen = None
        self._optimizer = None
        self._micro = 0
        self._stats = None
        self._stats_scale = 1.0
        self._outputs = None
        self._act_log = None

    @property
    def captured(self):
        return self._record is not None or (self._pb is not None and len(self._pb.graphs) > 0)

    def set_global_batch(self, global_batch):
        lo, hi = shard_bounds(global_batch, self.rank, self.world)
        if hasattr(self.model, "set_batch_offset"):
            self.model.set_batch_offset(lo)
        return lo, hi

    def attach_stats(self, stats, loss_scale=1.0):
        if self.captured:
            raise RuntimeError("attach_stats() comes before capture() / capture_packed(): the update is part of the captured step "
                               "(release_graph() first to change it)")
        self._stats, self._stats_scale, self._outputs = stats, float(loss_scale), None

    def attach_activations(self, log):
        if self.captured:
            raise RuntimeError("attach_activations() comes before capture() / capture_packed(): the probes are part of the captured "
                               "step (release_graph() first to change it)")
        if log is not None:
            log._guard()
        self._act_log = self.ctx.act_log = log

    def _update_stats(self):
        out, self._outputs = self._outputs, None
        if self._stats is not None and out is not None:
            logits, beta, y, loss, n_valid = out
            self._stats.update(logits, beta, y, loss, n_valid=n_valid, loss_scale=self._stats_scale)

    def _fwd_bwd(self, h_a, h_t, m_a, m_t, y, zero=True, scale=None, ragged=None):
        from . import _ops
        pb = self._pb
        front = pb.front if (pb is not None and ragged is None) else None
        if front is not None:
            seqs = _ops.CTX.seq_override
            if seqs is None:
                raise RuntimeError("DataParallelStep: after capture_packed() the static rows are fed by step_packed() only")
            _ops.seq_tables(front.lens.dev, pb.La, pb.Lt, rows=(seqs[0].N, seqs[1].N), cu=(pb.cu_a, pb.cu_t, pb.cu_f), masks=front.masks)
        b = self.buckets
        if self.force_queue is None:
            _ops.gemm_contended(bool(b._hooks) and not b.suspended and b.world > 1)
        else:
            _ops.gemm_contended(bool(self.force_queue), force=True)
        ctl = front.ctl.dev if (front is not None and front.ctl is not None) else None
        if ctl is not None and front.accum > 1:
            from . import _lib
            _lib.call("hriemo_grad_begin", self.buckets.flat.data_ptr(), self.buckets.flat.numel(), ctl.data_ptr(), _ops._stream())
            self.buckets._rebind()
        elif zero:
            self.buckets.zero_grad()
        act = self._act_log
        if act is not None:
            act.n_valid = ctl[:1] if (ctl is not None and front.partial) else None
        if ragged is not None:
            logits, beta, _ = self.model.forward_packed(h_a, h_t, ragged[0], ragged[1], pad_to=ragged[2])
        elif front is not None:
            logits, beta, _ = self.model._forward_rows(h_a, h_t, tuple(seqs), front.bool, (pb.La, pb.Lt))
        else:
            logits, beta, _ = self.model(h_a, h_t, m_a, m_t)
        if ctl is not None and front.partial:
            loss = self.loss_fn(logits, beta, y, n_valid=ctl[:1])
        else:
            loss = self.loss_fn(logits, beta, y)
        if self._stats is not None:
# ... 67 lines not shown
        self._exchange_in_graph = bool(collectives)
        self._optimizer = optimizer
        self._mask_seen = None

    def _end_capture(self):
        self._replay = True
        if self._exchange_in_graph:
            self.buckets.suspended = True

    @_in_step_context
    def capture_packed(self, rows_a, rows_t, lengths_a, lengths_t, y, pad_to, optimizer=None, collectives=False, partial_batches=False,
                       grad_accum=1):
        from . import _ops
        self._check_ragged_capture("capture_packed", partial_batches, grad_accum)
        same_width = not hasattr(self.model, "audio_proj")
        la, lt, pad = _ops.packed_lengths(rows_a, rows_t, lengths_a, lengths_t, pad_to, same_width=same_width)
        if pad_to is None:
            raise ValueError("capture_packed: pad_to=(L_a, L_t) is required")
        dev = next(self.model.parameters()).device
        self._capture_ragged(lambda: self._begin_ragged("capture_packed", optimizer, collectives), (rows_a.shape[1], rows_t.shape[1]),
                             rows_a.dtype, y.to(dev, copy=True), la, lt, pad, lambda: self._load_packed(rows_a, rows_t, la, lt, y),
                             partial=partial_batches, accum=grad_accum, ctl=partial_batches or grad_accum > 1)
        self._end_capture()

    def _check_ragged_capture(self, entry, partial_batches, grad_accum):
        self._need_forward_packed(entry)
        if int(grad_accum) != grad_accum or grad_accum < 1:
            raise ValueError(f"{entry}: grad_accum = {grad_accum!r} (an integer >= 1)")
        if partial_batches:
            self._need_n_valid(f"{entry}(partial_batches=True)")

    def _begin_ragged(self, entry, optimizer, collectives):
        self._begin_capture(entry, optimizer, collectives, packed=True)
        self._micro = 0

    @_in_step_context
    def capture_store(self, store, ids, pad_to=None, optimizer=None, collectives=False, partial_batches=False, grad_accum=1, augment=None):
        self._check_ragged_capture("capture_store", partial_batches, grad_accum)
        ids, la, lt, pad, y_static = self._store_capture("capture_store", store, ids, pad_to)
        if augment is not None:
            store._check_augment("capture_store", augment)
        self._capture_ragged(lambda: self._begin_ragged("capture_store", optimizer, collectives), store.widths, store.dtype, y_static, la, lt,
                             pad, lambda: self._load_store(ids, la, lt), store, partial=partial_batches, accum=grad_accum,
                             ctl=partial_batches or grad_accum > 1, augment=augment)
        self._end_capture()

    @_in_step_context
    def step_store(self, ids):
        feed = self._feed
        if feed is None or self._pb is None or self._pb.front is None:
            raise RuntimeError("step_store needs capture_store() first")
        ids, la, lt = feed.batch(ids, self._pb.front.partial or not self._replaying, "step_store")
        aug = feed.augment
        if self._replaying:
            loss = self._replay_ragged(lambda ctl: self._load_store(ids, la, lt, ctl=ctl))
        else:
            rows_a, _, rows_t, _, y = feed.store.fetch(ids, augment=aug)
            loss = self._eager_ragged(rows_a, rows_t, la, lt, y)
        if aug is not None:
            aug.draw += 1
        return loss

    @_in_step_context
    def step_packed(self, rows_a, rows_t, lengths_a, lengths_t, y):
        from . import _ops
        pb = self._pb
        front = pb.front if pb is not None else None
        if front is None:
            raise RuntimeError("step_packed needs capture_packed() first")
        la, lt, _ = _ops.packed_lengths(rows_a, rows_t, lengths_a, lengths_t, (pb.La, pb.Lt), same_width=front.same_width)
        if self._replaying:
            self._check_batch("step_packed", rows_a, rows_t, len(la), y)
            return self._replay_ragged(lambda ctl: self._load_packed(rows_a, rows_t, la, lt, y, ctl=ctl))
        return self._eager_ragged(rows_a, rows_t, la, lt, y)

    def _replay_ragged(self, load):
        first, last = micro_flags(self._micro, self._pb.front.accum)
        if self._optimizer is not None and self._optimizer._swapped is True:
            self._optimizer._refuse_while_averaged("a training replay")
        if self._optimizer is not None and last:
            self._optimizer._upload_hyper()
        key = load((first, last))
        rec = self._packed_graph(key)
        rec.graph.replay()
        self._micro = 0 if last else self._micro + 1
        if last:
            self._after_replay()
        return rec.loss

    def _eager_ragged(self, rows_a, rows_t, la, lt, y):
        pb = self._pb
        first, last = micro_flags(self._micro, pb.front.accum)
        dev = self._static[0].device
        was = self.buckets.suspended
        if not last:
            self.buckets.suspended = True
        try:
            loss = self._fwd_bwd(rows_a.to(dev, non_blocking=True), rows_t.to(dev, non_blocking=True), None, None, y.to(dev, non_blocking=True),
                                 zero=first, ragged=(la, lt, (pb.La, pb.Lt)))
        finally:
            self.buckets.suspended = was
        self._update_stats()
        self._micro = 0 if last else self._micro + 1
        if last:
            self.buckets.finish()
            if self._optimizer is not None:
                self._optimizer.step()
        return loss

    @property
    def micro_step(self):
        return self._micro

    @_in_step_context
    def flush_accumulated(self):
        n = self._micro
        if n == 0:
            return 0
        self._micro = 0
        if not self._exchange_in_graph or not self._replaying:
            self.buckets.finish()
        if self._optimizer is not None:
            self._optimizer.step()
        return n

    def _packed_key(self, m_a, m_t, lengths):
        pb = self._pb
        la, lt = mask_lengths(m_a, m_t, lengths, pb.B, pb.La, pb.Lt)
        key, *tables = packed_tables(la, lt, pb.B, pb.La, pb.Lt)
        for buf, cu in zip((pb.cu_a, pb.cu_t, pb.cu_f), tables):
            buf.copy_(torch.tensor(cu, dtype=torch.int32))
        return key

    def _capture_bucket(self, seqs):
        front = self._pb.front
        held = self.buckets.flat.clone() if (front is not None and front.accum > 1 and self._micro > 0) else None
        try:
            return self._capture_graph(seqs)
        finally:
            if held is not None:
                self.buckets.flat.copy_(held)

    def _capture_graph(self, seqs):
        from . import _ops
        collectives = self._exchange_in_graph

        def warm():
            if self._act_log is not None:
                with self._act_log.paused():
                    self._fwd_bwd(*self._static)
            else:
                self._fwd_bwd(*self._static)
            if collectives:
                self.buckets.finish()

        def warmed():
            self._outputs = None

        def body():
            _ops.bump_seed_word(self._static[0].device)
            loss = self._fwd_bwd(*self._static)
            self._update_stats()
            if collectives:
                self.buckets.finish()
            if self._optimizer is not None:
                front = self._pb.front if self._pb is not None else None
                ctl = front.ctl.dev if (front is not None and front.accum > 1) else None
                self._optimizer._enqueue(ctl=ctl)
            return loss, None

        return _record_graph(self._static[0].device, seqs, self._pb.pool if seqs is not None else None, warm, body, warmed,
                             settle=0.25 if collectives else 0.0)

    def release_graph(self):
        was = self.captured
        if self._record is not None:
            torch.cuda.synchronize()
            self._record.release()
        self._release_buckets()
        if was:
            self._record = self._pb = self._optimizer = None

    def use_graph(self, on):
        self._replay = bool(on) and self.captured
        self.buckets.suspended = self._replay

    def _after_replay(self):
        if not self._exchange_in_graph:
            self.buckets.finish()
        if self._optimizer is not None:
            from . import _ops
            _ops.bump_weights_epoch()
            self._optimizer._opt_called = True

    @_in_step_context
    def step(self, h_a, h_t, m_a, m_t, y, lengths=None):
        if self._replaying:
            pb = self._pb
            if self._optimizer is not None:
                self._optimizer._upload_hyper()
            if pb is not None and pb.front is not None:
                raise RuntimeError("DataParallelStep: this step was captured by capture_packed(); feed it with step_packed()")
            if pb is not None:
                if m_a is None or m_t is None:
                    raise RuntimeError("DataParallelStep (packed mode): both padding masks are needed")
                ident = (m_a.data_ptr(), m_a._version, m_t.data_ptr(), m_t._version)
                seen = self._mask_seen
                if lengths is None and seen is not None and seen.ident == ident:
                    key = seen.key
                    for buf, saved in zip((pb.cu_a, pb.cu_t, pb.cu_f), seen.cu):
                        buf.copy_(saved)
                else:
                    key = self._packed_key(m_a, m_t, lengths)
                    self._mask_seen = _MaskSeen(ident, key, (pb.cu_a.clone(), pb.cu_t.clone(), pb.cu_f.clone()), (m_a, m_t))
            for s, t in zip(self._static, (h_a, h_t, m_a, m_t, y)):
                if s is not None and t is not None and s.data_ptr() != t.data_ptr():
                    s.copy_(t)
            rec = self._packed_graph(key) if pb is not None else self._record
            rec.graph.replay()
            self._after_replay()
            return rec.loss
        loss = self._fwd_bwd(h_a, h_t, m_a, m_t, y)
        self._update_stats()
        self.buckets.finish()
        if self._optimizer is not None:
            self._optimizer.step()
        return loss


def _mode_switches():
    from . import _ops
    six = (("precision", _ops.precision()), ("gemm_mode", _ops.gemm_mode()), ("PACKED_TAIL", bool(_ops.PACKED_TAIL)),
           ("PACKED_TAIL_FP32", bool(_ops.PACKED_TAIL_FP32)), ("PACKED_TAIL_MX8", bool(_ops.PACKED_TAIL_MX8)), ("ingest", _ops.ingest()))
    if _ops.precision() != "fp32":
        return six
    return six + (("POOLED_GATE_FP32", bool(_ops.POOLED_GATE_FP32)),)


class _WeightsPass:

    def __init__(self, model, B):
        from . import _ops
        from .models.emotion_decoder import EmotionDecoder
        self.model, self.params = model, list(model.parameters())
        self.shadows = [m._sh for m in model.modules() if hasattr(m, "_sh")]
        decoders = [m for m in model.modules() if isinstance(m, EmotionDecoder)]
        self.decoder, self.B = (decoders[0] if decoders else None), B
        self.log, self.records, self.entries = _ops.FormLog(), [], []
        self.seen, self.ptrs, self.forms = None, tuple(p.data_ptr() for p in self.params), {}

    def _body(self, entries, prologue):
        from . import _ops
        ctx = _ops.CTX
        held, ctx.act_log = ctx.act_log, None
        try:
            with torch.no_grad():
                for _, fn, args in entries:
                    fn(*args)
                out = self.decoder.prologue(self.B) if prologue else None
        finally:
            ctx.act_log = held
        return None, out

    def eager(self):
        from . import _ops
        was = self.model.training
        self.model.eval()
        try:
            _ops.begin_step()
            return self._body(self.entries, self.decoder is not None)[1]
        finally:
            self.model.train(was)

    def record(self, dev, new):
        prologue = not self.records and self.decoder is not None
        self.records.append(_record_graph(dev, None, None, lambda: self._body(new, prologue), lambda: self._body(new, prologue)))
        self.entries += new
        self.replay()

    def handed(self, decoder, B):
        if decoder is not self.decoder or B != self.B or not self.records:
            raise RuntimeError("EvalStep (stationary): the decoder asks for a prologue the weights pass did not record")
        return self.records[0].out

    def state(self):
        from . import _ops
        return (_ops.WEIGHTS_EPOCH, tuple(p._version for p in self.params))

    def moved(self):
        return self.seen != self.state()

    def replay(self):
        for rec in self.records:
            rec.graph.replay()
        self.seen = self.state()

    def _form_ptrs(self):
        out = {}
        for sh in self.shadows:
            for key, ent in sh._d.items():
                form = ent[1]
# ... 250 lines not shown
```

hri-emo_amd/optim.py:

```python
import contextlib

import torch

from . import _lib
from . import _ops
from ._ops import _p, _stream, _require_gpu


class FusedClipAdamW:
    def __init__(self, buckets, lr=1e-4, betas=(0.9, 0.999), eps=1e-8, weight_decay=1e-2, max_norm=5.0):
        self.buckets = buckets
        flat_g = buckets.flat
        _require_gpu(flat_g)
        self.lr, self.betas, self.eps, self.wd, self.max_norm = lr, betas, eps, weight_decay, max_norm
        self.flat_p = torch.zeros_like(flat_g)
        self.m = torch.zeros_like(flat_g)
        self.v = torch.zeros_like(flat_g)
        with torch.no_grad():
            for p in buckets.params:
                off, n = buckets._offsets[id(p)], p.numel()
                view = self.flat_p[off:off + n].view_as(p)
                view.copy_(p.data)
                p.data = view
        self.nblocks = 1024
        self._partial = torch.empty(self.nblocks, dtype=torch.float32, device=flat_g.device)
        self._norm2 = torch.zeros(1, dtype=torch.float32, device=flat_g.device)
        self.steps = 0

    @torch.no_grad()
    def step(self):
        g = self.buckets.flat
        n = g.numel()
        st = _stream()
        self.steps += 1
        _lib.call("hriemo_sumsq_f32", _p(g), n, _p(self._partial), self.nblocks, st)
        _lib.call("hriemo_rowsum_f32", _p(self._partial), _p(self._norm2), 1, self.nblocks, st)
        _lib.call("hriemo_adamw_flat", _p(self.flat_p), _p(g), _p(self.m), _p(self.v), n, self.lr, self.betas[0], self.betas[1],
                  self.eps, self.wd, self.steps, self.max_norm if self.max_norm else 0.0, _p(self._norm2), st)
        _ops.bump_weights_epoch()
        return self._norm2.sqrt()


MAX_GROUPS = 16
MAX_SEGMENTS = 2048
AVERAGING_MODES = {"ema": 1.0, "swa": 2.0}


def is_averaging_step(t, avg_start, avg_every):
    return t > avg_start and (t - avg_start) % avg_every == 0


def averaging_weight(mode, n_averaged, avg_decay):
    return 1.0 - avg_decay if mode == "ema" else 1.0 / (n_averaged + 1)


def decay_groups(named_parameters, weight_decay, no_decay=lambda name, p: p.dim() < 2):
    decay, rest = [], []
    for name, p in named_parameters:
        if p.requires_grad:
            (rest if no_decay(name, p) else decay).append(p)
    groups = [{"params": decay, "weight_decay": weight_decay}, {"params": rest, "weight_decay": 0.0}]
    return [g for g in groups if g["params"]]


def _describe(p):
    return f"shape {tuple(p.shape)}"


def _materialise(param_groups):
    groups = list(param_groups)
    if not groups or not all(isinstance(g, dict) and "params" in g for g in groups):
        raise ValueError("DeviceAdamW: param_groups is a non-empty list of dicts with a 'params' entry")
    return [{**g, "params": [g["params"]] if isinstance(g["params"], torch.Tensor) else list(g["params"])} for g in groups]


def _group_of_params(buckets, groups):
    if len(groups) > MAX_GROUPS:
        raise ValueError(f"DeviceAdamW: {len(groups)} param groups; the grouped update kernel takes at most {MAX_GROUPS}")
    index = {id(p): i for i, p in enumerate(buckets.params)}
    owner = {}
    for gi, g in enumerate(groups):
        for j, p in enumerate(g["params"]):
            if not isinstance(p, torch.Tensor) or id(p) not in index:
                what = _describe(p) if isinstance(p, torch.Tensor) else repr(type(p))
                raise ValueError(f"DeviceAdamW: param_groups[{gi}]['params'][{j}] ({what}) is foreign: not one of the buckets' parameters")
            if id(p) in owner:
                raise ValueError(f"DeviceAdamW: buckets.params[{index[id(p)]}] ({_describe(p)}) is repeated: it appears in "
                                 f"param_groups[{owner[id(p)]}] and again in param_groups[{gi}]")
            owner[id(p)] = gi
    for i, p in enumerate(buckets.params):
        if id(p) not in owner:
            raise ValueError(f"DeviceAdamW: buckets.params[{i}] ({_describe(p)}) is missing: it appears in no param group "
                             "(the groups must partition the buckets' parameters)")
    return owner


def group_segments(buckets, param_groups):
    owner = _group_of_params(buckets, _materialise(param_groups))
    seg, seg_group = [0], []
    for p in sorted(buckets.params, key=lambda q: buckets._offsets[id(q)]):
        off, g = buckets._offsets[id(p)], owner[id(p)]
        if seg_group and seg_group[-1] == g:
            continue
        if seg_group:
            seg.append(off)
        seg_group.append(g)
    seg.append(buckets.flat.numel())
    return seg, seg_group


HEALTH_CHUNK = 32768
MAX_HEALTH_PARAMS = 4096
MAX_HEALTH_CAPACITY = 1 << 20


def health_chunks(slots, chunk=HEALTH_CHUNK):
    if isinstance(chunk, bool) or not isinstance(chunk, int) or chunk < 1024 or chunk % 1024:
        raise ValueError(f"health_chunks: chunk={chunk!r} must be a positive multiple of 1024")
    rows, end = [], 0
    for i, (start, length, group) in enumerate(slots):
        if start % 64 or length % 64 or length <= 0 or start < end:
            raise ValueError(f"health_chunks: slot {i} (start {start}, length {length}): slots start at multiples of 64 elements, are "
                             "padded to 64 and ascend without overlap")
# ... 185 lines not shown
            health._check_attach(buckets)
        if param_groups is None:
            _require_gpu(flat_g)
        self._check_scalars(lr, betas, eps, weight_decay, "")
        groups, seg, seg_group, units = None, None, None, None
        if param_groups is not None:
            groups = _materialise(param_groups)
            if clip == "global":
                seg, seg_group = group_segments(buckets, groups)
            else:
                units = clip_units(buckets, groups, clip)
                seg, seg_group = units["seg"], units["seg_group"]
            if len(seg_group) > MAX_SEGMENTS:
                raise ValueError(f"DeviceAdamW: the groups cut the flat buffer into {len(seg_group)} segments; the grouped update "
                                 f"kernel takes at most {MAX_SEGMENTS} (group neighbouring parameters together)")
            for gi, g in enumerate(groups):
                if clip == "global" and "max_norm" in g and g["max_norm"] != max_norm:
                    raise ValueError(f"DeviceAdamW: param_groups[{gi}] names max_norm={g['max_norm']!r}, the optimizer {max_norm!r}: "
                                     "the clip is global (one norm over all groups); clip='group' or clip='parameter' gives every "
                                     "group its own max_norm")
                mn = g.get("max_norm")
                if clip != "global" and mn is not None and (isinstance(mn, bool) or not isinstance(mn, (int, float)) or mn != mn):
                    raise ValueError(f"DeviceAdamW: param_groups[{gi}] names max_norm={mn!r}; a number (<= 0 or None: no clipping)")
                self._check_scalars(g.get("lr", lr), g.get("betas", betas), g.get("eps", eps), g.get("weight_decay", weight_decay),
                                    f" (param_groups[{gi}])")
                if "betas" in g:
                    g["betas"] = tuple(g["betas"])
            _require_gpu(flat_g)
        self.buckets = buckets
        self._grouped = groups is not None
        G = len(groups) if self._grouped else 1
        dev = flat_g.device
        self.flat_p = torch.zeros_like(flat_g)
        self.m = torch.zeros_like(flat_g)
        self.v = torch.zeros_like(flat_g)
        self.nblocks = 1024
        self.clip = clip
        self._partial = torch.zeros(self.nblocks if units is None else len(units["chunks"]), dtype=torch.float32, device=dev)
        self.averaging, self.avg_decay, self.avg_start, self.avg_every = averaging, avg_decay, avg_start, avg_every
        self._swapped = False
        if averaging is None:
            self._hyper = torch.zeros(G * 8, dtype=torch.float32, device=dev)
        else:
            self._hyper_block = torch.zeros(G * 8 + 4, dtype=torch.float32, device=dev)
            self._hyper, self._avg_hyper = self._hyper_block[:G * 8], self._hyper_block[G * 8:]
            self._avg_state = torch.zeros(4, dtype=torch.float32, device=dev)
            self.n_averaged = self._avg_state[0]
        self._state = torch.zeros(G * 8, dtype=torch.float32, device=dev)
        self._hyper_host = None
        if self._grouped:
            self._seg = torch.tensor(seg, dtype=torch.int64, device=dev)
            self._seg_group = torch.tensor(seg_group, dtype=torch.int32, device=dev)
        if units is not None:
            self._seg_unit = torch.tensor(units["seg_unit"], dtype=torch.int32, device=dev)
            self._unit_group = torch.tensor(units["unit_group"], dtype=torch.int32, device=dev)
            self._unit_chunks = torch.tensor(units["unit_chunks"], dtype=torch.int32, device=dev)
            self._chunks = torch.tensor(units["chunks"], dtype=torch.int64, device=dev)
            self._unit_group_host = list(units["unit_group"])
            self._clip_state = torch.zeros(2 * len(units["unit_group"]), dtype=torch.float32, device=dev)
            self._clip_params = sorted(buckets.params, key=lambda q: buckets._offsets[id(q)])
            self._clip_names = None
        defaults = dict(lr=lr, betas=tuple(betas), eps=eps, weight_decay=weight_decay, amsgrad=False, maximize=False, foreach=None,
                        capturable=False, differentiable=False, fused=None, decoupled_weight_decay=True, max_norm=max_norm)
        self._constructing = True
        try:
            super().__init__(groups if self._grouped else list(buckets.params), defaults)
        finally:
            self._constructing = False
        with torch.no_grad():
            for group in self.param_groups:
                for p in group["params"]:
                    off, n = buckets._offsets[id(p)], p.numel()
                    view = self.flat_p[off:off + n].view_as(p)
                    view.copy_(p.data)
                    p.data = view
                    self.state[p] = {"step": self._state[0], "exp_avg": self.m[off:off + n].view_as(p),
                                     "exp_avg_sq": self.v[off:off + n].view_as(p)}
        self.grad_norm, self.device_step, self.skipped = self._state[6], self._state[0], self._state[7]
        if averaging is not None:
            self.avg = self.flat_p.clone()
        self.health = health
        if health is not None:
            health._attach(self, {id(p): gi for gi, group in enumerate(self.param_groups) for p in group["params"]})

    @staticmethod
    def _check_scalars(lr, betas, eps, weight_decay, where):
        if lr < 0 or eps < 0 or weight_decay < 0 or not 0 <= betas[0] < 1 or not 0 <= betas[1] < 1:
            raise ValueError(f"DeviceAdamW: lr, eps, weight_decay >= 0 and betas in [0, 1) are required{where}")

    @staticmethod
    def _check_averaging(averaging, avg_decay, avg_start, avg_every):
        if averaging is None:
            if (avg_decay, avg_start, avg_every) != (0.999, 0, 1):
                raise ValueError("DeviceAdamW: avg_decay / avg_start / avg_every are given without averaging= ('ema' or 'swa'): "
                                 "nothing would be averaged")
            return
        if averaging not in AVERAGING_MODES:
            raise ValueError(f"DeviceAdamW: averaging={averaging!r}; the modes are None, 'ema' and 'swa'")
        if not (isinstance(avg_decay, (int, float)) and 0 <= avg_decay < 1):
            raise ValueError(f"DeviceAdamW: avg_decay={avg_decay!r} must lie in [0, 1)")
        for name, val, low in (("avg_start", avg_start, 0), ("avg_every", avg_every, 1)):
            if isinstance(val, bool) or not isinstance(val, int) or not low <= val < 2 ** 24:
                raise ValueError(f"DeviceAdamW: {name}={val!r} must be an integer >= {low} (and below 2**24)")

    def _refuse_while_averaged(self, what):
        if self._swapped:
            raise RuntimeError(f"DeviceAdamW: {what} inside `with opt.averaged_weights():` -- the parameter buffer holds the AVERAGE "
                               "there; leave the block first")

    def add_param_group(self, param_group):
        if self.param_groups and not getattr(self, "_constructing", False):
            raise RuntimeError("DeviceAdamW updates ONE flat buffer laid out like its GradBuckets: its param groups are fixed at "
                               "construction (DeviceAdamW(buckets, param_groups=[...])) and partition the buckets' parameters")
        super().add_param_group(param_group)

    def _upload_hyper(self):
        self._refuse_while_averaged("step() / a replay that carries the update")
        img = []
        for g in self.param_groups:
            if g["amsgrad"] or g["maximize"]:
                raise RuntimeError("DeviceAdamW: amsgrad / maximize are not built; there is no fallback to torch.optim.AdamW")
            mn = g["max_norm"]
            if self.clip == "global" and mn != self.param_groups[0]["max_norm"]:
                raise RuntimeError("DeviceAdamW: the param groups carry different max_norm values; the clip is global")
            img += [float(g["lr"]), float(g["betas"][0]), float(g["betas"][1]), float(g["eps"]), float(g["weight_decay"]),
                    float(mn) if mn else 0.0, 0.0, 0.0]
        block = self._hyper
        if self.averaging is not None:
            self._check_averaging(self.averaging, self.avg_decay, self.avg_start, self.avg_every)
            img += [AVERAGING_MODES[self.averaging], float(self.avg_decay), float(self.avg_start), float(self.avg_every)]
            block = self._hyper_block
        img = tuple(img)
        if img != self._hyper_host:
            block.copy_(torch.tensor(img, dtype=torch.float32).pin_memory(), non_blocking=True)
            self._hyper_host = img

    def _enqueue(self, grad_scale=None, found_inf=None, ctl=None):
        self._enqueue_update(grad_scale, found_inf, ctl)
        if self.health is not None:
            self.health._enqueue(self, grad_scale, ctl)

    def _enqueue_update(self, grad_scale, found_inf, ctl):
        self._refuse_while_averaged("an update")
        g = self.buckets.flat
        n = g.numel()
        st = _stream()
        if self.clip != "global":
            G, S, U, C = len(self.param_groups), self._seg_group.numel(), self._unit_group.numel(), self._partial.numel()
            avg = self.averaging is not None
            _lib.call("hriemo_sumsq_units", _p(g), n, _p(self._chunks), C, _p(self._partial), st)
            _lib.call("hriemo_optim_finalize_units", _p(self._partial), C, _p(self._unit_chunks), _p(self._unit_group), U, _p(self._hyper), G,
                      _p(grad_scale), _p(found_inf), _p(self._state), _p(ctl), _p(self._clip_state),
                      _p(self._avg_hyper) if avg else None, _p(self._avg_state) if avg else None, st)
            if avg:
                _lib.call("hriemo_adamw_flat_units_avg", _p(self.flat_p), _p(g), _p(self.m), _p(self.v), n, _p(self._seg), _p(self._seg_group),
                          _p(self._seg_unit), S, _p(self._hyper), _p(self._state), G, _p(self._clip_state), U, _p(self.avg),
                          _p(self._avg_state), st)
            else:
                _lib.call("hriemo_adamw_flat_units", _p(self.flat_p), _p(g), _p(self.m), _p(self.v), n, _p(self._seg), _p(self._seg_group),
                          _p(self._seg_unit), S, _p(self._hyper), _p(self._state), G, _p(self._clip_state), U, st)
            return
        _lib.call("hriemo_sumsq_f32", _p(g), n, _p(self._partial), self.nblocks, st)
        if self.averaging is not None:
            G = len(self.param_groups)
            _lib.call("hriemo_optim_finalize_avg", _p(self._partial), self.nblocks, _p(self._hyper), G, _p(grad_scale), _p(found_inf),
                      _p(self._state), _p(ctl), _p(self._avg_hyper), _p(self._avg_state), st)
            if self._grouped:
                _lib.call("hriemo_adamw_flat_groups_avg", _p(self.flat_p), _p(g), _p(self.m), _p(self.v), n, _p(self._seg),
                          _p(self._seg_group), self._seg_group.numel(), _p(self._hyper), _p(self._state), G, _p(self.avg),
                          _p(self._avg_state), st)
            else:
                _lib.call("hriemo_adamw_flat_dev_avg", _p(self.flat_p), _p(g), _p(self.m), _p(self.v), n, _p(self._hyper), _p(self._state),
                          _p(self.avg), _p(self._avg_state), st)
            return
        if self._grouped:
            G = len(self.param_groups)
            _lib.call("hriemo_optim_finalize_groups", _p(self._partial), self.nblocks, _p(self._hyper), G, _p(grad_scale), _p(found_inf),
                      _p(self._state), _p(ctl), st)
            _lib.call("hriemo_adamw_flat_groups", _p(self.flat_p), _p(g), _p(self.m), _p(self.v), n, _p(self._seg), _p(self._seg_group),
                      self._seg_group.numel(), _p(self._hyper), _p(self._state), G, st)
            return
        if ctl is None:
            _lib.call("hriemo_optim_finalize", _p(self._partial), self.nblocks, _p(self._hyper), _p(grad_scale), _p(found_inf),
                      _p(self._state), st)
        else:
            _lib.call("hriemo_optim_finalize_ctl", _p(self._partial), self.nblocks, _p(self._hyper), _p(grad_scale), _p(found_inf),
                      _p(self._state), _p(ctl), st)
        _lib.call("hriemo_adamw_flat_dev", _p(self.flat_p), _p(g), _p(self.m), _p(self.v), n, _p(self._hyper), _p(self._state), st)

    def _amp_word(self, name):
        t = getattr(self, name, None)
        if t is None:
            return None
        if not (isinstance(t, torch.Tensor) and t.is_cuda and t.dtype == torch.float32 and t.numel() == 1):
            raise RuntimeError(f"DeviceAdamW: {name} must be one fp32 value on the GPU (torch.amp.GradScaler's), got {t!r}")
        return t

    @torch.no_grad()
    def step(self, closure=None):
        if closure is not None:
            raise RuntimeError("DeviceAdamW.step() takes no closure: the gradients are read from the flat buffer")
        self._upload_hyper()
        self._enqueue(self._amp_word("grad_scale"), self._amp_word("found_inf"))
        _ops.bump_weights_epoch()

    def zero_grad(self, set_to_none=True):
        self.buckets.zero_grad()

    def _require_units(self, what):
        if self.clip == "global":
            raise RuntimeError(f"DeviceAdamW.{what}: built with clip='global', there are no clip units (grad_norm is the one norm)")

    def name_parameters(self, named_parameters):
        self._require_units("name_parameters()")
        given = {id(p): name for name, p in named_parameters}
        for i, p in enumerate(self._clip_params):
            if id(p) not in given:
                raise ValueError(f"DeviceAdamW.name_parameters: parameter {i} of the optimizer ({_describe(p)}) has no name")
        self._clip_names = [given[id(p)] for p in self._clip_params]

    def clip_arrays(self):
        self._require_units("clip_arrays()")
        img = self._clip_state.cpu().numpy().reshape(-1, 2)
        if self.clip == "parameter" and self._clip_names is not None:
            unit = list(self._clip_names)
        else:
            unit = list(range(img.shape[0]))
        max_norm = [self.param_groups[gi]["max_norm"] for gi in self._unit_group_host]
        return {"mode": self.clip, "unit": unit, "norm": img[:, 0].copy(), "coef": img[:, 1].copy(), "max_norm": max_norm}

    def _require_averaging(self, what):
        if self.averaging is None:
            raise RuntimeError(f"DeviceAdamW.{what}: built without averaging= ('ema' or 'swa'), there is no average")

    def _swap_avg(self):
        _lib.call("hriemo_swap_fp32", _p(self.flat_p), _p(self.avg), self.flat_p.numel(), _stream())
        _ops.bump_weights_epoch()

    @contextlib.contextmanager
    def averaged_weights(self):
        self._require_averaging("averaged_weights()")
        self._refuse_while_averaged("a nested averaged_weights()")
        self._swap_avg()
        self._swapped = True
        try:
            yield self
        finally:
            self._swapped = False
            self._swap_avg()

    @torch.no_grad()
    def averaged_state_dict(self, model):
        self._require_averaging("averaged_state_dict()")
        self._refuse_while_averaged("averaged_state_dict()")
        sd = model.state_dict()
        for name, p in model.named_parameters():
            off = self.buckets._offsets.get(id(p))
            if off is not None and name in sd:
                sd[name] = self.avg[off:off + p.numel()].view_as(p).clone()
        return sd

    def state_dict(self):
        self._refuse_while_averaged("state_dict()")
        sd = super().state_dict()
        steps = self._state[0].expand(len(sd["state"])).clone().unbind(0)
        sd["state"] = {k: {**ent, "step": s} for (k, ent), s in zip(sd["state"].items(), steps)}
        if self.averaging is not None:
            keys = [k for g in sd["param_groups"] for k in g["params"]]
            params = [p for g in self.param_groups for p in g["params"]]
            sd["averaging"] = {"mode": self.averaging, "decay": self.avg_decay, "start": self.avg_start, "every": self.avg_every,
                               "n_averaged": self._avg_state[0].clone(), "avg": {k: self._avg_view(p) for k, p in zip(keys, params)}}
        if self.clip != "global":
            sd["clip"] = {"mode": self.clip}
        return sd

    def _avg_view(self, p):
        off = self.buckets._offsets[id(p)]
        return self.avg[off:off + p.numel()].view_as(p)

    @torch.no_grad()
    def load_state_dict(self, state_dict):
        self._refuse_while_averaged("load_state_dict()")
        groups, state = state_dict["param_groups"], state_dict["state"]
        mine_groups = self.param_groups
        n_params = len(self.buckets.params)
        if len(groups) != len(mine_groups) or any(len(a["params"]) != len(b["params"]) for a, b in zip(groups, mine_groups)):
            raise ValueError("DeviceAdamW.load_state_dict: a different grouping: the state dict has %d param group(s) over %s "
# ... 65 lines not shown
```

include/hriemo.h:

```cpp
#ifndef HRIEMO_H_
#define HRIEMO_H_

#ifdef __cplusplus
extern "C" {
#endif

typedef struct ihipStream_t* hriemo_stream_t;

const char* hriemo_last_error(void);
int hriemo_abi_version(void);

int hriemo_gemm_bf16(int ta, int tb, int M, int N, int K, const void* A, long lda, const void* B, long ldb,
                     void* C, long ldc, int c_is_f32, const float* bias, int epilogue, const void* aux,
                     long ldaux, int accumulate, float* workspace, long workspace_bytes, hriemo_stream_t stream);

int hriemo_gemm_bf16_group_tn(const void* jobs_host, int njobs, int accumulate, hriemo_stream_t stream);
int hriemo_gemm_bf16_split(int ta, int tb, int M, int N, int K, const void* A, long lda, const void* B, long ldb, void* C, long ldc,
                           void* C2, long ldc2, int split_m, int accumulate, float* workspace, long workspace_bytes,
                           hriemo_stream_t stream);
int hriemo_gemm_colsum_rows(int ta, int tb, int M, int N, int K);
int hriemo_gemm_bf16_colsum(int ta, int tb, int M, int N, int K, const void* A, long lda, const void* B, long ldb, void* C, long ldc,
                            const void* aux, long ldaux, float* colsum_partials, hriemo_stream_t stream);
int hriemo_gemm_force_config(int cfg);
int hriemo_gemm_debug_flags(int flags);
// ... 121 lines not shown
                      const unsigned char* mask_t, int B, int La, int Lt, int d, void* gate_in, float* a_pool,
                      float* t_pool, float* cnt, hriemo_stream_t stream);
int hriemo_sigmoid_beta(const float* pre, float* w, float* beta, int B, int d, hriemo_stream_t stream);
int hriemo_fuse_fwd(const float* w, const void* A, const void* T, void* H, int B, int L, int d, hriemo_stream_t stream);
int hriemo_fuse_bwd_dw(const void* dH, const void* A, const void* T, float* partials, int B, int L, int d,
                       hriemo_stream_t stream);
int hriemo_gate_dpre(const float* partials, int L, const float* dbeta, const float* w, void* dpre, int B, int d,
                     hriemo_stream_t stream);
int hriemo_gate_input_bwd(const void* dgin, const float* a_pool, const float* t_pool, const float* cnt, float* da,
                          float* dt, int B, int d, hriemo_stream_t stream);
int hriemo_masked_mean_fwd(const void* X, const unsigned char* mask, float* pooled, float* cnt, int B, int L, int d,
                           hriemo_stream_t stream);
int hriemo_rowsum_f32(const float* x, float* out, int B, long n, hriemo_stream_t stream);
int hriemo_gate_input_pooled(const float* a_pool, const float* t_pool, void* gate_in, int B, int d, hriemo_stream_t stream);
int hriemo_fusion_loss(const float* logits, const float* targets, const float* pos_weight, const float* beta, int B, int Ne,
                       int reg_mode, float reg_coef, float scale, float* loss, float* dlogits, float* dbeta, hriemo_stream_t stream);
int hriemo_fusion_loss_ce(const float* logits, const long long* labels, const float* beta, int B, int C, int reg_mode,
                          float reg_coef, float scale, float* loss, float* dlogits, float* dbeta, hriemo_stream_t stream);
int hriemo_fusion_loss_n(const float* logits, const float* targets, const float* pos_weight, const float* beta, int B, int Ne,
                         int reg_mode, float reg_coef, float scale, float* loss, float* dlogits, float* dbeta, const int* n_valid,
                         hriemo_stream_t stream);
int hriemo_fusion_loss_ce_n(const float* logits, const long long* labels, const float* beta, int B, int C, int reg_mode,
                            float reg_coef, float scale, float* loss, float* dlogits, float* dbeta, const int* n_valid,
                            hriemo_stream_t stream);
int hriemo_stats_update(const float* logits, const float* targets, const long long* labels, const float* loss, float loss_scale,
                        const float* beta, int beta_per_sample, const int* n_valid, int B, int C, int skip_nonfinite,
                        float* probs, unsigned char* truth, int capacity, int* counters, double* sums, hriemo_stream_t stream);
int hriemo_stats_counts(const float* probs, const unsigned char* truth, int capacity, int C, const int* counters,
                        const float* thresholds, int S, int* out, hriemo_stream_t stream);
int hriemo_stats_auc_tiles(int capacity);
int hriemo_stats_auc(const float* probs, const unsigned char* truth, int capacity, int C, const int* counters,
                     unsigned long long* partial, int* npn, hriemo_stream_t stream);
int hriemo_predict_log(const float* logits, const float* beta, int beta_per_sample, const int* n_valid, int B, int C, int kind,
                       float* probs, float* beta_mean, int* pred, int capacity, int* counters, hriemo_stream_t stream);
int hriemo_attn_log_plan(const int* lens, const int* n_valid, int B, int capacity, int* counters, int* window, int* lengths,
                         hriemo_stream_t stream);
int hriemo_attn_log_close(int* window, hriemo_stream_t stream);
int hriemo_attn_log_append(const float* maps, int B, int map_elems, const int* window, float* log, int capacity,
                           hriemo_stream_t stream);
int hriemo_attn_probs_varlen_log(const void* Q, long ldq, const void* K, long ldk, const int* cu_seqlens_q, const int* cu_seqlens_k,
                                 const float* lse, float* probs, int B, int H, int max_len_q, int max_len_k, int out_lq, int out_lk,
                                 int head_dim, float p_drop, unsigned long long seed, const unsigned long long* seed_dev, unsigned site,
                                 int b_offset, const int* window, int capacity, hriemo_stream_t stream);
int hriemo_attn_probs_varlen_log_fp32(const float* Q, long ldq, const float* K, long ldk, const int* cu_seqlens_q,
                                     const int* cu_seqlens_k, const float* lse, float* probs, int B, int H, int max_len_q, int max_len_k,
                                     int out_lq, int out_lk, int head_dim, float p_drop, unsigned long long seed,
                                     const unsigned long long* seed_dev, unsigned site, int b_offset, const int* window, int capacity,
                                     hriemo_stream_t stream);
int hriemo_scalar_gate_dx(const void* dH, int Lf, const float* beta, int is_a, const float* dpool, const float* cnt,
                          const unsigned char* mask, void* dX, int B, int L, int d, hriemo_stream_t stream);
int hriemo_sumsq_f32(const float* x, long n, float* partial, int nblocks, hriemo_stream_t stream);
int hriemo_adamw_flat(float* p, const float* g, float* m, float* v, long n, float lr, float beta1, float beta2, float eps,
                      float weight_decay, int step, float max_norm, const float* norm2, hriemo_stream_t stream);
int hriemo_optim_finalize(const float* partial, int nblocks, const float* hyper, const float* grad_scale, const float* found_inf,
                          float* state, hriemo_stream_t stream);
int hriemo_adamw_flat_dev(float* p, const float* g, float* m, float* v, long n, const float* hyper, const float* state,
                          hriemo_stream_t stream);
int hriemo_grad_begin(float* flat, long n, const int* ctl, hriemo_stream_t stream);
int hriemo_optim_finalize_ctl(const float* partial, int nblocks, const float* hyper, const float* grad_scale, const float* found_inf,
                              float* state, const int* ctl, hriemo_stream_t stream);
int hriemo_optim_finalize_groups(const float* partial, int nblocks, const float* hyper, int G, const float* grad_scale,
                                 const float* found_inf, float* state, const int* ctl, hriemo_stream_t stream);
int hriemo_adamw_flat_groups(float* p, const float* g, float* m, float* v, long n, const long long* seg, const int* seg_group, int S,
                             const float* hyper, const float* state, int G, hriemo_stream_t stream);
int hriemo_optim_finalize_avg(const float* partial, int nblocks, const float* hyper, int G, const float* grad_scale,
                              const float* found_inf, float* state, const int* ctl, const float* avg_hyper, float* avg_state,
                              hriemo_stream_t stream);
int hriemo_adamw_flat_dev_avg(float* p, const float* g, float* m, float* v, long n, const float* hyper, const float* state, float* avg,
                              const float* avg_state, hriemo_stream_t stream);
int hriemo_adamw_flat_groups_avg(float* p, const float* g, float* m, float* v, long n, const long long* seg, const int* seg_group, int S,
                                 const float* hyper, const float* state, int G, float* avg, const float* avg_state,
                                 hriemo_stream_t stream);
int hriemo_swap_fp32(float* a, float* b, long n, hriemo_stream_t stream);
int hriemo_sumsq_units(const float* g, long n, const long long* chunks, int C, float* partial, hriemo_stream_t stream);
int hriemo_optim_finalize_units(const float* partial, int C, const int* unit_chunks, const int* unit_group, int U, const float* hyper,
                                int G, const float* grad_scale, const float* found_inf, float* state, const int* ctl, float* clip_state,
                                const float* avg_hyper, float* avg_state, hriemo_stream_t stream);
int hriemo_adamw_flat_units(float* p, const float* g, float* m, float* v, long n, const long long* seg, const int* seg_group,
                            const int* seg_unit, int S, const float* hyper, const float* state, int G, const float* clip_state, int U,
                            hriemo_stream_t stream);
int hriemo_adamw_flat_units_avg(float* p, const float* g, float* m, float* v, long n, const long long* seg, const int* seg_group,
                                const int* seg_unit, int S, const float* hyper, const float* state, int G, const float* clip_state, int U,
                                float* avg, const float* avg_state, hriemo_stream_t stream);
int hriemo_health_sweep(const float* g, const float* p, const float* m, const float* v, long n, const long long* chunks, int C,
                        const float* hyper, const float* state, int G, const int* ctl, int every, float* partial,
                        hriemo_stream_t stream);
int hriemo_health_fold(const float* partial, const long long* chunks, int C, int P, const float* state, const int* ctl,
                       const float* grad_scale, int every, int capacity, int* log, hriemo_stream_t stream);
int hriemo_act_probe_rows(void);
int hriemo_act_log_plan(int record, int every, int capacity, int n_sites, int* counters, int* window, int* counts, int* ring,
                        hriemo_stream_t stream);
int hriemo_act_probe(const void* x, int dtype, int n_rows, int d, long ld, const int* cu_seqlens, const unsigned char* kpm, int B, int L,
                     const int* n_valid, const int* window, int site, int half, int n_sites, int chunk_cap, float* partial, int* counts,
                     hriemo_stream_t stream);
int hriemo_act_log_fold(const float* partial, const int* counts, const int* window, int half, int n_sites, int chunk_cap, int capacity,
                        int* ring, hriemo_stream_t stream);
int hriemo_add_ln_bwd_partial_rows(int M, int d);
int hriemo_rowops_force_variant(int variant);
int hriemo_colsum_partial_rows(int M, int N);
int hriemo_colreduce_batch(const void* jobs_host, int njobs, void* jobs_dev, int nblocks, hriemo_stream_t stream);
int hriemo_debug_hog(int blocks, int micros, float* sink, hriemo_stream_t stream);
int hriemo_ln_pool_pair_supported(int d);
int hriemo_ln_pool_fwd_pair(const void* Xa, const float* Xa32, const unsigned char* mask_a, const float* gamma_a, const float* beta_a,
                            void* Yna, float* mean_a, float* rstd_a, float* partials_a, int La,
                            const void* Xt, const float* Xt32, const unsigned char* mask_t, const float* gamma_t, const float* beta_t,
                            void* Ynt, float* mean_t, float* rstd_t, float* partials_t, int Lt,
                            int B, int Lkeep, int d, float eps, hriemo_stream_t stream);
int hriemo_ln_pool_bwd_pair(const void* dH, int Lf, const float* w,
                            const float* dpool_a, const unsigned char* mask_a, const void* Xa, const float* Xa32, const float* gamma_a,
                            const float* mean_a, const float* rstd_a, void* dXa, float* dgamma_a, float* dbeta_a, int La, float* workspace_a,
                            const float* dpool_t, const unsigned char* mask_t, const void* Xt, const float* Xt32, const float* gamma_t,
                            const float* mean_t, const float* rstd_t, void* dXt, float* dgamma_t, float* dbeta_t, int Lt, float* workspace_t,
                            int accumulate, int B, int d, hriemo_stream_t stream);
int hriemo_ln_pool_bwd_chunks(int L);
long hriemo_ln_pool_bwd_workspace_bytes(int B, int L, int d);
int hriemo_ln_pool_bwd(const void* dH, int Lf, const float* w, int is_a, const float* dpool, const unsigned char* mask,
                       const void* X, const float* X32, const float* gamma, const float* mean, const float* rstd, void* dX,
                       float* dgamma, float* dbeta, int accumulate, int B, int L, int d, float* workspace, hriemo_stream_t stream);

int hriemo_ln_pool2_fwd(const void* X, const float* X32, const unsigned char* mask, const float* gamma, const float* beta,
                        float* mean, float* rstd, float* partials, float* partials_keep, int B, int L, int Lkeep, int d, float eps,
                        hriemo_stream_t stream);
int hriemo_ln_pool2_fwd_pair(const void* Xa, const float* Xa32, const unsigned char* mask_a, const float* gamma_a, const float* beta_a,
                             float* mean_a, float* rstd_a, float* partials_a, float* partials_keep_a, int La,
                             const void* Xt, const float* Xt32, const unsigned char* mask_t, const float* gamma_t, const float* beta_t,
                             float* mean_t, float* rstd_t, float* partials_t, float* partials_keep_t, int Lt,
                             int B, int Lkeep, int d, float eps, hriemo_stream_t stream);
int hriemo_pooled_fuse_fwd(const float* partials_keep_a, int La, const float* partials_keep_t, int Lt, const float* w, int Lkeep,
                           float* abar, float* tbar, float* pooled, int B, int d, hriemo_stream_t stream);
int hriemo_pooled_fuse_bwd(const float* dpooled, const float* abar, const float* tbar, const float* w, int Lkeep, float* dw,
                           float* g_a, float* g_t, int B, int d, hriemo_stream_t stream);
int hriemo_ln_pool_vec_bwd(const float* g, int Lkeep, const float* dpool, const unsigned char* mask, const void* X, const float* X32,
                           const float* gamma, const float* mean, const float* rstd, void* dX, float* dgamma, float* dbeta,
                           int accumulate, int B, int L, int d, float* workspace, hriemo_stream_t stream);
int hriemo_ln_pool_vec_bwd_pair(int Lkeep,
                                const float* g_a, const float* dpool_a, const unsigned char* mask_a, const void* Xa, const float* Xa32, const float* gamma_a,
                                const float* mean_a, const float* rstd_a, void* dXa, float* dgamma_a, float* dbeta_a, int La, float* workspace_a,
                                const float* g_t, const float* dpool_t, const unsigned char* mask_t, const void* Xt, const float* Xt32, const float* gamma_t,
                                const float* mean_t, const float* rstd_t, void* dXt, float* dgamma_t, float* dbeta_t, int Lt, float* workspace_t,
                                int accumulate, int B, int d, hriemo_stream_t stream);
int hriemo_ingest_padded(const void* X, int x_dtype, long ldx, const int* cu_seqlens, int n_rows, int B, int L, int d, void* Y16,
                         float* Y32, hriemo_stream_t stream);

int hriemo_ln_pool_fwd_packed(const void* X, const float* X32, const int* cu_seqlens, int nseq, int n_rows, const float* gamma,
                              const float* beta, void* Yn, float* mean, float* rstd, float* partials, int L,
                              const int* cu_fused, int n_fused, int B, int d, float eps, hriemo_stream_t stream);
int hriemo_ln_pool_fwd_packed_pair(const void* Xa, const float* Xa32, const int* cu_a, int nseq_a, int n_rows_a, const float* gamma_a,
                                   const float* beta_a, void* Yna, float* mean_a, float* rstd_a, float* partials_a, int La,
                                   const void* Xt, const float* Xt32, const int* cu_t, int nseq_t, int n_rows_t, const float* gamma_t,
                                   const float* beta_t, void* Ynt, float* mean_t, float* rstd_t, float* partials_t, int Lt,
                                   const int* cu_fused, int n_fused, int B, int d, float eps, hriemo_stream_t stream);
int hriemo_fuse_fwd_packed(const float* w, const void* A, const void* T, void* H, const int* cu_fused, int n_fused, int B, int L, int d,
                           hriemo_stream_t stream);
int hriemo_fuse_fwd_packed_q(const float* w, const void* A, const void* T, void* H, const int* cu_fused, int n_fused, int B, int L, int d,
                             void* Hq, void* Hs, long lds, hriemo_stream_t stream);
int hriemo_fuse_bwd_dw_packed(const void* dH, const void* A, const void* T, float* partials, const int* cu_fused, int n_fused, int B,
                              int L, int d, hriemo_stream_t stream);
int hriemo_ln_pool_bwd_packed(const void* dH, const int* cu_fused, int n_fused, const float* w, int is_a, const float* dpool,
                              const void* X, const float* X32, const int* cu_seqlens, int nseq, int n_rows, const float* gamma,
                              const float* mean, const float* rstd, void* dX, float* dgamma, float* dbeta, int accumulate, int B, int L,
                              int d, float* workspace, hriemo_stream_t stream);
int hriemo_ln_pool_bwd_packed_pair(const void* dH, const int* cu_fused, int n_fused, const float* w,
                                   const float* dpool_a, const void* Xa, const float* Xa32, const int* cu_a, int nseq_a, int n_rows_a,
                                   const float* gamma_a, const float* mean_a, const float* rstd_a, void* dXa, float* dgamma_a,
                                   float* dbeta_a, int La, float* workspace_a,
                                   const float* dpool_t, const void* Xt, const float* Xt32, const int* cu_t, int nseq_t, int n_rows_t,
// ... 103 lines not shown
```

Measured before the change: 8793 utterances/s.

## Write bf16/fp32 weight forms directly from the AdamW update kernel

The flat AdamW kernels can now also write the updated parameters into the cached bf16 and concatenated fp32 weight forms, using a span table built once per captured step. The captured step then treats the forms it owns as fresh and skips the separate cast-copy pass that would otherwise run at the start of the next replay. This removes one read of the fp32 masters plus the cast kernel per step. In exchange it adds a binary search per vector in the optimizer kernel and more bookkeeping to keep forms consistent. The measured metric is fwd+bwd replay, so the gain only appears if the cast pass sits inside the timed region.

```diff
diff --git a/hri-emo_amd/__init__.py b/hri-emo_amd/__init__.py
--- a/hri-emo_amd/__init__.py
+++ b/hri-emo_amd/__init__.py
@@ -7,7 +7,7 @@
 from .models.fusion_classifier import FusionClassifier
 
 from .dp import EvalStep
-from ._ops import set_gemm_mode, gemm_mode, enable_fused_wgrad, set_precision, precision, set_varlen, varlen, set_varlen_maps, varlen_maps, set_mfma_maps, mfma_maps, set_ingest, ingest, set_pooled_gate_fp32, pooled_gate_fp32
+from ._ops import set_gemm_mode, gemm_mode, enable_fused_wgrad, set_precision, precision, set_varlen, varlen, set_varlen_maps, varlen_maps, set_mfma_maps, mfma_maps, set_ingest, ingest, set_pooled_gate_fp32, pooled_gate_fp32, set_forms_in_update, forms_in_update
 
-__all__ = ["EvalStep", "set_gemm_mode", "gemm_mode", "enable_fused_wgrad", "set_precision", "precision", "set_varlen", "varlen", "set_varlen_maps", "varlen_maps", "set_mfma_maps", "mfma_maps", "set_ingest", "ingest", "set_pooled_gate_fp32", "pooled_gate_fp32", "CrossModalBlock", "CrossModalTransformer", "BetaGate", "EmotionDecoder", "ExplainableDecoderLayer",
+__all__ = ["EvalStep", "set_gemm_mode", "gemm_mode", "enable_fused_wgrad", "set_precision", "precision", "set_varlen", "varlen", "set_varlen_maps", "varlen_maps", "set_mfma_maps", "mfma_maps", "set_ingest", "ingest", "set_pooled_gate_fp32", "pooled_gate_fp32", "set_forms_in_update", "forms_in_update", "CrossModalBlock", "CrossModalTransformer", "BetaGate", "EmotionDecoder", "ExplainableDecoderLayer",
            "FusionWithEmotionDecoder", "MoseiFusionWithEmotionDecoder", "FusionClassifier"]
diff --git a/hri-emo_amd/_lib.py b/hri-emo_amd/_lib.py
--- a/hri-emo_amd/_lib.py
+++ b/hri-emo_amd/_lib.py
@@ -116,6 +116,11 @@
     "hriemo_optim_finalize_units": ("pippipipppppppp", "i"),
     "hriemo_adamw_flat_units": ("pppplpppippipip", "i"),
     "hriemo_adamw_flat_units_avg": ("pppplpppippipippp", "i"),
+    "hriemo_form_table_build": ("pilpip", "i"),
+    "hriemo_adamw_flat_forms": ("pppplfffffifp" + "pi" + "p", "i"),
+    "hriemo_adamw_flat_dev_forms": ("pppplpppp" + "pi" + "p", "i"),
+    "hriemo_adamw_flat_groups_forms": ("pppplppippipp" + "pi" + "p", "i"),
+    "hriemo_adamw_flat_units_forms": ("pppplpppippipipp" + "pi" + "p", "i"),
     "hriemo_health_sweep": ("pppplpippipipp", "i"),
     "hriemo_health_fold": ("ppiipppiipp", "i"),
     "hriemo_act_probe_rows": ("", "i"),
diff --git a/hri-emo_amd/_ops.py b/hri-emo_amd/_ops.py
--- a/hri-emo_amd/_ops.py
+++ b/hri-emo_amd/_ops.py
@@ -76,12 +76,13 @@
 
 class StepContext:
     __slots__ = ("capturing", "capture_origin", "seq_override", "join_scope", "half_reports", "stationary", "forms", "prologue",
-                 "act_log")
+                 "act_log", "owned")
 
     def __init__(self):
         self.capturing, self.capture_origin, self.seq_override, self.join_scope, self.half_reports = False, None, None, 0, {}
         self.stationary, self.forms, self.prologue = False, None, None
         self.act_log = None
+        self.owned = None
 
 
 CTX = StepContext()
@@ -224,6 +225,11 @@
     fresh = ent is not None and ent[0] == ver and (device is None or ent[1].device == device)
     if not CTX.capturing:
         return not fresh
+    if CTX.owned is not None and ent is not None and id(ent[1]) in CTX.owned:
+        if not fresh:
+            raise RuntimeError("hri_emo_amd: a weight form the captured step owns is stale inside its capture (internal error: the "
+                               "warm-up passes should have left it fresh) -- no cast is recorded")
+        return False
     if CTX.stationary:
         if not fresh:
             raise RuntimeError("hri_emo_amd: a weight form is stale inside the capture of a stationary step (internal error: the "
@@ -470,6 +476,179 @@
         ent = (ver, s_)
         sh._d[key] = ent
     return ent[1]
+
+
+FORMS_IN_UPDATE = _os.environ.get("HRIEMO_FORMS_IN_UPDATE", "1") != "0"
+MAX_FORM_SPANS = 2048
+_flat_masters = []
+
+
+def set_forms_in_update(on=True):
+    global FORMS_IN_UPDATE
+    FORMS_IN_UPDATE = bool(on)
+
+
+def forms_in_update():
+    return FORMS_IN_UPDATE
+
+
+def register_flat_master(opt):
+    import weakref
+    _flat_masters[:] = [r for r in _flat_masters if r() is not None]
+    _flat_masters.append(weakref.ref(opt))
+
+
+def _flat_master_of(params):
+    out = []
+    for r in reversed(_flat_masters):
+        opt = r()
+        if opt is None:
+            continue
+        lo = opt.flat_p.data_ptr()
+        hi = lo + opt.flat_p.numel() * 4
+        if all(lo <= p.data_ptr() and p.data_ptr() + p.numel() * 4 <= hi for p in params):
+            out.append(opt)
+    return out
+
+
+class FormSet:
+
+    def __init__(self, entries):
+        self.segs, self.stamps, self.owned, self._seen_keys = [], [], set(), set()
+        for key, fn, args in entries:
+            kind = key[0]
+            if kind == "get":
+                self._add_get(fn.__self__, args[0])
+            elif kind == "prefetch_batch":
+                for sh, p in args[0]:
+                    self._add_get(sh, p)
+            elif kind == "get_cat":
+                self._add_cat(fn.__self__, [("cat", args[0], 0)])
+            elif kind == "get_cat_vec":
+                self._add_cat(fn.__self__, [("catv", args[0], 1)])
+            elif kind == "get_cat_wb":
+                self._add_cat(fn.__self__, [("cat", args[0], 0), ("catv", args[1], 1)])
+        masters = {}
+        for p, *_ in self.segs:
+            masters[id(p)] = p
+        self.masters = list(masters.values())
+        self.flats = [opt.flat_p for opt in _flat_master_of(self.masters)] if self.masters else []
+        jobs = [(p.data_ptr() + off * 4, form.data_ptr() + foff * (4 if kind else 2), count, kind)
+                for p, off, count, form, foff, kind in self.segs]
+        self._jobs = torch.tensor(jobs, dtype=torch.int64) if jobs else None
+        self.table = None
+        self.passes = 0
+        self.seen = self.state()
+
+    @staticmethod
+    def _plain(p):
+        return p.is_cuda and p.dtype == torch.float32 and p.is_contiguous() and p.data_ptr() % 16 == 0
+
+    def _add_get(self, sh, p):
+        dkey = id(p)
+        if (id(sh), dkey) in self._seen_keys:
+            return
+        self._seen_keys.add((id(sh), dkey))
+        ent = sh._d.get(dkey)
+        if ent is None or not self._plain(p) or ent[1].dtype != BF16 or ent[1].shape != p.shape or ent[1].data_ptr() % 16:
+            return
+        form = ent[1]
+        self.segs.append((p, 0, p.numel(), form, 0, 0))
+        self.owned.add(id(form))
+        self.stamps.append((sh._d, dkey, form, lambda p=p: (p._version, p.data_ptr(), WEIGHTS_EPOCH)))
+
+    def _add_cat(self, sh, forms):
+        segs, stamps = [], []
+        for prefix, parts, kind in forms:
+            dkey = (prefix,) + tuple((id(p), r0, r1) for p, r0, r1 in parts)
+            if (id(sh), dkey) in self._seen_keys:
+                return
+            ent = sh._d.get(dkey)
+            if ent is None or ent[1].dtype != (torch.float32 if kind else BF16) or not ent[1].is_contiguous():
+                return
+            form, esize, at = ent[1], (4 if kind else 2), 0
+            for p, r0, r1 in parts:
+                K = 1 if kind else p.shape[1]
+                off, count = r0 * K, (r1 - r0) * K
+                if not self._plain(p) or (p.data_ptr() + off * 4) % 16 or (form.data_ptr() + at * esize) % 16 or count <= 0:
+                    return
+                segs.append((p, off, count, form, at, kind))
+                at += count
+            if at != form.numel():
+                return
+            stamps.append((sh._d, dkey, form,
+                           lambda parts=parts: tuple((p._version, p.data_ptr()) for p, _, _ in parts) + (WEIGHTS_EPOCH,)))
+        for _, dkey, form, _ in stamps:
+            self._seen_keys.add((id(sh), dkey))
+            self.owned.add(id(form))
+        self.segs += segs
+        self.stamps += stamps
+
+    def state(self):
+        return (WEIGHTS_EPOCH, tuple((p._version, p.data_ptr()) for p in self.masters), tuple(f._version for f in self.flats))
+
+    def current(self):
+        return self.seen == self.state()
+
+    def restamp(self):
+        for d, dkey, form, ver in self.stamps:
+            d[dkey] = (ver(), form, STEP_ID)
+        self.seen = self.state()
+
+    def refresh(self):
+        for d, dkey, form, _ in self.stamps:
+            ent = d.get(dkey)
+            if ent is None or ent[1] is not form:
+                raise RuntimeError("hri_emo_amd: a weight form of the captured step moved to other memory since the capture "
+                                   "(.to(), another precision) -- capture again")
+        if self._jobs is not None:
+            _lib.call("hriemo_cast_copy_batch", self._jobs.data_ptr(), self._jobs.shape[0], _stream())
+        self.passes += 1
+        self.restamp()
+
+    def sync(self, who):
+        now = self.state()
+        if now == self.seen or not self.segs:
+            return False
+        if tuple(ptr for _, ptr in now[1]) != tuple(ptr for _, ptr in self.seen[1]):
+            raise RuntimeError(f"{who}: a parameter moved to other memory since the capture (an optimizer built afterwards, .to()): "
+                               "the captured step still points at the old storage -- capture again")
+        self.refresh()
+        return True
+
+    def attach(self):
+        import weakref
+        owners = _flat_master_of(self.masters) if self.masters else []
+        if not owners or not self.segs:
+            return None
+        opt = owners[0]
+        base = opt.flat_p.data_ptr()
+        rows = sorted(((p.data_ptr() - base) // 4 + off, count, form.data_ptr() + foff * (4 if kind else 2), kind)
+                      for p, off, count, form, foff, kind in self.segs)
+        host = torch.tensor(rows, dtype=torch.int64)
+        spans = torch.zeros((MAX_FORM_SPANS, 6), dtype=torch.int64)
+        n = torch.zeros(1, dtype=torch.int32)
+        try:
+            _lib.call("hriemo_form_table_build", host.data_ptr(), len(rows), opt.flat_p.numel(), spans.data_ptr(), MAX_FORM_SPANS, n.data_ptr())
+        except RuntimeError:
+            return None
+        F = int(n.item())
+        self.table = (weakref.ref(opt), spans[:F].contiguous().to(opt.flat_p.device), F)
+        opt._forms = self
+        return opt
+
+    def table_for(self, opt):
+        t = self.table
+        if not FORMS_IN_UPDATE or t is None or t[0]() is not opt:
+            return None
+        return t[1], t[2]
+
+    def release(self):
+        t, self.table = self.table, None
+        if t is not None:
+            opt = t[0]()
+            if opt is not None and getattr(opt, "_forms", None) is self:
+                opt._forms = None
 
 
 def to_bf16(x):
diff --git a/hri-emo_amd/csrc/forms.h b/hri-emo_amd/csrc/forms.h
--- /dev/null
+++ b/hri-emo_amd/csrc/forms.h
@@ -0,0 +1,78 @@
+#pragma once
+#include "common.h"
+
+enum { FORM_BF16 = 0, FORM_F32 = 1, FORM_MAX_COVER = 2, FORM_MAX_SPANS = 2048, FORM_SPAN_WORDS = 6 };
+
+struct FormTab { const long long* __restrict__ spans; int F; };
+struct FormCur { long long lo, hi; unsigned long long b0, b1; int kinds, nd; };
+
+__device__ __forceinline__ void form_stage(const FormTab t, long long* __restrict__ fb) {
+  for (int i = threadIdx.x; i < t.F; i += 256) fb[i] = t.spans[(long)i * FORM_SPAN_WORDS];
+}
+
+__device__ __forceinline__ void form_seek(FormCur& c, const FormTab t, const long long* __restrict__ fb, long long x, long long n) {
+  int lo = 0, hi = t.F;
+  while (lo < hi) {
+    const int mid = (lo + hi) >> 1;
+    if (fb[mid] > x) hi = mid; else lo = mid + 1;
+  }
+  c.lo = 0; c.b0 = 0; c.b1 = 0; c.kinds = 0; c.nd = 0;
+  if (lo > 0) {
+    const long long* __restrict__ row = t.spans + (long)(lo - 1) * FORM_SPAN_WORDS;
+    const long long end = row[1];
+    if (x < end) {
+      const int nd = (int)row[5];
+      c.lo = fb[lo - 1]; c.hi = end;
+      c.b0 = (unsigned long long)row[2]; c.b1 = (unsigned long long)row[3];
+      c.kinds = (int)row[4]; c.nd = nd < 0 ? 0 : (nd > FORM_MAX_COVER ? FORM_MAX_COVER : nd);
+      return;
+    }
+    c.lo = end;
+  }
+  c.hi = lo < t.F ? fb[lo] : n;
+}
+
+__device__ __forceinline__ void form_put4(unsigned long long base, int kind, long long x, const f32x4 pp) {
+  if (kind == FORM_F32) {
+    float* d = (float*)(base + (unsigned long long)x * 4ull);
+    if (((uintptr_t)d & 15) == 0) {
+      *(f32x4*)d = pp;
+    } else {
+#pragma unroll
+      for (int e = 0; e < 4; ++e) d[e] = pp[e];
+    }
+    return;
+  }
+  bf16_t* d = (bf16_t*)(base + (unsigned long long)x * 2ull);
+  bf16x4 q;
+#pragma unroll
+  for (int e = 0; e < 4; ++e) q[e] = (bf16_t)pp[e];
+  if (((uintptr_t)d & 7) == 0) {
+    *(bf16x4*)d = q;
+  } else {
+#pragma unroll
+    for (int e = 0; e < 4; ++e) d[e] = q[e];
+  }
+}
+
+__device__ __forceinline__ void form_put1(unsigned long long base, int kind, long long x, float val) {
+  if (kind == FORM_F32) *(float*)(base + (unsigned long long)x * 4ull) = val;
+  else *(bf16_t*)(base + (unsigned long long)x * 2ull) = (bf16_t)val;
+}
+
+__device__ __forceinline__ void form_vec4(FormCur& c, const FormTab t, const long long* __restrict__ fb, long i, long long n, const f32x4 pp) {
+  const long long x = (long long)i * 4;
+  if (x < c.lo || x >= c.hi) form_seek(c, t, fb, x, n);
+  if (x + 4 <= c.hi) {
+    if (c.nd >= 1) form_put4(c.b0, c.kinds & 1, x, pp);
+    if (c.nd >= 2) form_put4(c.b1, (c.kinds >> 1) & 1, x, pp);
+    return;
+  }
+#pragma unroll
+  for (int e = 0; e < 4; ++e) {
+    const long long xe = x + e;
+    if (xe >= c.hi) form_seek(c, t, fb, xe, n);
+    if (c.nd >= 1) form_put1(c.b0, c.kinds & 1, xe, pp[e]);
+    if (c.nd >= 2) form_put1(c.b1, (c.kinds >> 1) & 1, xe, pp[e]);
+  }
+}
diff --git a/hri-emo_amd/csrc/optim.hip b/hri-emo_amd/csrc/optim.hip
--- a/hri-emo_amd/csrc/optim.hip
+++ b/hri-emo_amd/csrc/optim.hip
@@ -1,4 +1,7 @@
 #include "common.h"
+#include "forms.h"
+#include <algorithm>
+#include <vector>
 
 enum { HY_LR = 0, HY_BETA1, HY_BETA2, HY_EPS, HY_WD, HY_MAX_NORM };
 enum { ST_STEP = 0, ST_SKIP, ST_COEF, ST_STEP_SIZE, ST_ISB2, ST_DECAY, ST_GRAD_NORM, ST_SKIPPED };
@@ -88,35 +91,56 @@
   *(f32x4*)(avg + i * 4) = aa;
 }
 
-template <bool AVG>
+template <bool AVG, bool FORMS>
 __device__ __forceinline__ void adamw_flat_dev_body(float* __restrict__ p, const float* __restrict__ g, float* __restrict__ m,
                                                     float* __restrict__ v, long n, const float* __restrict__ hyper,
                                                     const float* __restrict__ state, float* __restrict__ avg,
-                                                    const float* __restrict__ avg_state) {
+                                                    const float* __restrict__ avg_state, const FormTab ft) {
   if (state[ST_SKIP] != 0.f) return;
   const AdamScalars s = {hyper[HY_BETA1], hyper[HY_BETA2], hyper[HY_EPS], state[ST_COEF], state[ST_STEP_SIZE], state[ST_ISB2], state[ST_DECAY]};
   const long nv = n >> 2;
+  extern __shared__ __attribute__((aligned(16))) long long ag_lds[];
+  FormCur fc = {0, 0, 0ull, 0ull, 0, 0};
+  if (FORMS) {
+    form_stage(ft, ag_lds);
+    __syncthreads();
+  }
   if (AVG) {
     const AvgStep a = avg_step(state, avg_state);
     if (a.kind != AV_NONE) {
-      for (long i = (long)blockIdx.x * 256 + threadIdx.x; i < nv; i += (long)gridDim.x * 256) avg_vec4(avg, i, adamw_vec4(p, g, m, v, i, s), a);
+      for (long i = (long)blockIdx.x * 256 + threadIdx.x; i < nv; i += (long)gridDim.x * 256) {
+        const f32x4 pp = adamw_vec4(p, g, m, v, i, s);
+        avg_vec4(avg, i, pp, a);
+        if (FORMS) form_vec4(fc, ft, ag_lds, i, n, pp);
+      }
       return;
     }
   }
-  for (long i = (long)blockIdx.x * 256 + threadIdx.x; i < nv; i += (long)gridDim.x * 256) adamw_vec4(p, g, m, v, i, s);
+  for (long i = (long)blockIdx.x * 256 + threadIdx.x; i < nv; i += (long)gridDim.x * 256) {
+    const f32x4 pp = adamw_vec4(p, g, m, v, i, s);
+    if (FORMS) form_vec4(fc, ft, ag_lds, i, n, pp);
+  }
 }
 
 __global__ __launch_bounds__(256) void adamw_flat_dev_kernel(float* __restrict__ p, const float* __restrict__ g, float* __restrict__ m,
                                                              float* __restrict__ v, long n, const float* __restrict__ hyper,
                                                              const float* __restrict__ state) {
-  adamw_flat_dev_body<false>(p, g, m, v, n, hyper, state, nullptr, nullptr);
+  adamw_flat_dev_body<false, false>(p, g, m, v, n, hyper, state, nullptr, nullptr, FormTab{});
 }
 
 __global__ __launch_bounds__(256) void adamw_flat_dev_avg_kernel(float* __restrict__ p, const float* __restrict__ g, float* __restrict__ m,
                                                                  float* __restrict__ v, long n, const float* __restrict__ hyper,
                                                                  const float* __restrict__ state, float* __restrict__ avg,
                                                                  const float* __restrict__ avg_state) {
-  adamw_flat_dev_body<true>(p, g, m, v, n, hyper, state, avg, avg_state);
+  adamw_flat_dev_body<true, false>(p, g, m, v, n, hyper, state, avg, avg_state, FormTab{});
+}
+
+template <bool AVG>
+__global__ __launch_bounds__(256) void adamw_flat_dev_forms_kernel(float* __restrict__ p, const float* __restrict__ g, float* __restrict__ m,
+                                                                   float* __restrict__ v, long n, const float* __restrict__ hyper,
+                                                                   const float* __restrict__ state, float* __restrict__ avg,
+                                                                   const float* __restrict__ avg_state, const FormTab ft) {
+  adamw_flat_dev_body<AVG, true>(p, g, m, v, n, hyper, state, avg, avg_state, ft);
 }
 
 struct ClipUnits {
@@ -305,18 +329,20 @@
   if (threadIdx.x == 0) partial[blockIdx.x] = ((red[0] + red[1]) + red[2]) + red[3];
 }
 
-template <bool AVG, bool UNITS>
+template <bool AVG, bool UNITS, bool FORMS>
 __device__ __forceinline__ void adamw_flat_groups_body(float* __restrict__ p, const float* __restrict__ g, float* __restrict__ m,
                                                        float* __restrict__ v, long n, const long long* __restrict__ seg,
                                                        const int* __restrict__ seg_group, int S, const float* __restrict__ hyper,
                                                        const float* __restrict__ state, int G, float* __restrict__ avg,
                                                        const float* __restrict__ avg_state, const int* __restrict__ seg_unit,
-                                                       const float* __restrict__ clip_state, int U) {
+                                                       const float* __restrict__ clip_state, int U, const FormTab ft) {
   if (state[ST_SKIP] != 0.f) return;
   AvgStep a = {AV_NONE, 0.f};
   if (AVG) a = avg_step(state, avg_state);
   extern __shared__ __attribute__((aligned(16))) long long ag_lds[];
-  long long* segb = ag_lds;
+  long long* fb = ag_lds;
+  long long* segb = ag_lds + (FORMS ? ft.F : 0);
+  if (FORMS) form_stage(ft, fb);
   float* sc = (float*)(segb + (S + 1));
   float* uc = sc + G * 8;
   unsigned short* su = (unsigned short*)(uc + (UNITS ? U : 0));
@@ -344,6 +370,7 @@
   __syncthreads();
   AdamScalars s = {0.f, 0.f, 0.f, 0.f, 0.f, 0.f, 0.f};
   long long cur_lo = 0, cur_hi = 0;
+  FormCur fc = {0, 0, 0ull, 0ull, 0, 0};
   const long nv = n >> 2;
   for (long i = (long)blockIdx.x * 256 + threadIdx.x; i < nv; i += (long)gridDim.x * 256) {
     const long long x = (long long)i * 4;
@@ -359,6 +386,7 @@
     }
     const f32x4 pp = adamw_vec4(p, g, m, v, i, s);
     if (AVG && a.kind != AV_NONE) avg_vec4(avg, i, pp, a);
+    if (FORMS) form_vec4(fc, ft, fb, i, n, pp);
   }
 }
 
@@ -366,7 +394,7 @@
                                                                 float* __restrict__ v, long n, const long long* __restrict__ seg,
                                                                 const int* __restrict__ seg_group, int S, const float* __restrict__ hyper,
                                                                 const float* __restrict__ state, int G) {
-  adamw_flat_groups_body<false, false>(p, g, m, v, n, seg, seg_group, S, hyper, state, G, nullptr, nullptr, nullptr, nullptr, 0);
+  adamw_flat_groups_body<false, false, false>(p, g, m, v, n, seg, seg_group, S, hyper, state, G, nullptr, nullptr, nullptr, nullptr, 0, FormTab{});
 }
 
 __global__ __launch_bounds__(256) void adamw_flat_groups_avg_kernel(float* __restrict__ p, const float* __restrict__ g, float* __restrict__ m,
@@ -374,7 +402,7 @@
                                                                     const int* __restrict__ seg_group, int S, const float* __restrict__ hyper,
                                                                     const float* __restrict__ state, int G, float* __restrict__ avg,
                                                                     const float* __restrict__ avg_state) {
-  adamw_flat_groups_body<true, false>(p, g, m, v, n, seg, seg_group, S, hyper, state, G, avg, avg_state, nullptr, nullptr, 0);
+  adamw_flat_groups_body<true, false, false>(p, g, m, v, n, seg, seg_group, S, hyper, state, G, avg, avg_state, nullptr, nullptr, 0, FormTab{});
 }
 
 template <bool AVG>
@@ -384,7 +412,18 @@
                                                                const float* __restrict__ hyper, const float* __restrict__ state, int G,
                                                                const float* __restrict__ clip_state, int U, float* __restrict__ avg,
                                                                const float* __restrict__ avg_state) {
-  adamw_flat_groups_body<AVG, true>(p, g, m, v, n, seg, seg_group, S, hyper, state, G, avg, avg_state, seg_unit, clip_state, U);
+  adamw_flat_groups_body<AVG, true, false>(p, g, m, v, n, seg, seg_group, S, hyper, state, G, avg, avg_state, seg_unit, clip_state, U, FormTab{});
+}
+
+template <bool AVG, bool UNITS>
+__global__ __launch_bounds__(256) void adamw_flat_groups_forms_kernel(float* __restrict__ p, const float* __restrict__ g, float* __restrict__ m,
+                                                                      float* __restrict__ v, long n, const long long* __restrict__ seg,
+                                                                      const int* __restrict__ seg_group, const int* __restrict__ seg_unit,
+                                                                      int S, const float* __restrict__ hyper, const float* __restrict__ state,
+                                                                      int G, const float* __restrict__ clip_state, int U,
+                                                                      float* __restrict__ avg, const float* __restrict__ avg_state,
+                                                                      const FormTab ft) {
+  adamw_flat_groups_body<AVG, UNITS, true>(p, g, m, v, n, seg, seg_group, S, hyper, state, G, avg, avg_state, seg_unit, clip_state, U, ft);
 }
 
 typedef __attribute__((ext_vector_type(4))) unsigned u32x4;
@@ -651,3 +690,148 @@
   HRIEMO_LAUNCH_CHECK("swap_fp32_kernel");
   return 0;
 }
+
+extern "C" int hriemo_form_table_build(const void* segs_host, int nseg, long n, void* spans_host, int max_spans, int* nspans) {
+  HRIEMO_CHECK(nspans != nullptr, "form_table_build: nspans is required");
+  *nspans = 0;
+  HRIEMO_CHECK(nseg >= 0 && n > 0 && n % 4 == 0, "form_table_build: nseg=%d, n=%ld (a positive multiple of 4)", nseg, n);
+  if (nseg == 0) return 0;
+  HRIEMO_CHECK(segs_host != nullptr && spans_host != nullptr && max_spans > 0, "form_table_build: segs_host, spans_host and max_spans > 0 are required");
+  HRIEMO_CHECK(nseg <= FORM_MAX_SPANS, "form_table_build: %d segments (at most %d)", nseg, (int)FORM_MAX_SPANS);
+  const long long* sg = (const long long*)segs_host;
+  long long* out = (long long*)spans_host;
+  std::vector<long long> cuts;
+  cuts.reserve((size_t)nseg * 2);
+  for (int j = 0; j < nseg; ++j) {
+    const long long b = sg[4 * j], c = sg[4 * j + 1], d = sg[4 * j + 2], k = sg[4 * j + 3];
+    HRIEMO_CHECK(b >= 0 && c > 0 && b <= (long long)n && c <= (long long)n - b, "form_table_build: segment %d [%lld, +%lld) leaves the buffer of %ld elements", j, b, c, n);
+    HRIEMO_CHECK(k == FORM_BF16 || k == FORM_F32, "form_table_build: segment %d has kind %lld (0 = bf16, 1 = fp32)", j, k);
+    HRIEMO_CHECK(d != 0 && d % (k == FORM_F32 ? 4 : 2) == 0, "form_table_build: segment %d has a NULL or misaligned destination", j);
+    HRIEMO_CHECK(j == 0 || b >= sg[4 * (j - 1)], "form_table_build: segment %d begins in front of segment %d (the table is sorted by begin)", j, j - 1);
+    cuts.push_back(b);
+    cuts.push_back(b + c);
+  }
+  std::sort(cuts.begin(), cuts.end());
+  cuts.erase(std::unique(cuts.begin(), cuts.end()), cuts.end());
+  int rows = 0;
+  for (size_t q = 0; q + 1 < cuts.size(); ++q) {
+    const long long lo = cuts[q], hi = cuts[q + 1];
+    long long base[FORM_MAX_COVER] = {0, 0}, kinds = 0;
+    int nd = 0;
+    for (int j = 0; j < nseg && sg[4 * j] <= lo; ++j) {
+      const long long b = sg[4 * j], c = sg[4 * j + 1], d = sg[4 * j + 2], k = sg[4 * j + 3];
+      if (b + c < hi) continue;
+      HRIEMO_CHECK(nd < FORM_MAX_COVER, "form_table_build: element %lld is covered by more than %d segments", lo, (int)FORM_MAX_COVER);
+      base[nd] = (long long)((unsigned long long)d - (unsigned long long)b * (k == FORM_F32 ? 4ull : 2ull));
+      kinds |= k << nd;
+      ++nd;
+    }
+    if (nd == 0) continue;
+    HRIEMO_CHECK(rows < max_spans && rows < FORM_MAX_SPANS, "form_table_build: more than %d spans", max_spans < FORM_MAX_SPANS ? max_spans : (int)FORM_MAX_SPANS);
+    long long* row = out + (long)rows * FORM_SPAN_WORDS;
+    row[0] = lo; row[1] = hi; row[2] = base[0]; row[3] = base[1]; row[4] = kinds; row[5] = nd;
+    ++rows;
+  }
+  *nspans = rows;
+  return 0;
+}
+
+static int form_tab_check(const char* who, const void* spans, int F) {
+  HRIEMO_CHECK(F >= 0 && F <= FORM_MAX_SPANS, "%s: F=%d spans (0 .. %d)", who, F, (int)FORM_MAX_SPANS);
+  HRIEMO_CHECK(F == 0 || (spans != nullptr && ((uintptr_t)spans % 8) == 0), "%s: spans (int64 [F][6], hriemo_form_table_build) is required, 8-byte aligned", who);
+  return 0;
+}
+
+extern "C" int hriemo_adamw_flat_dev_forms(float* p, const float* g, float* m, float* v, long n, const float* hyper, const float* state,
+                                           float* avg, const float* avg_state, const void* spans, int F, hipStream_t st) {
+  if (form_tab_check("adamw_flat_dev_forms", spans, F)) return 1;
+  if (F == 0) return avg != nullptr ? hriemo_adamw_flat_dev_avg(p, g, m, v, n, hyper, state, avg, avg_state, st)
+                                    : hriemo_adamw_flat_dev(p, g, m, v, n, hyper, state, st);
+  HRIEMO_CHECK(n > 0 && n % 4 == 0, "adamw_flat_dev_forms: n=%ld must be a positive multiple of 4", n);
+  HRIEMO_CHECK(p != nullptr && g != nullptr && m != nullptr && v != nullptr, "adamw_flat_dev_forms: p, g, m and v are required");
+  HRIEMO_CHECK(((uintptr_t)p % 16) == 0 && ((uintptr_t)g % 16) == 0 && ((uintptr_t)m % 16) == 0 && ((uintptr_t)v % 16) == 0 &&
+                   ((uintptr_t)avg % 16) == 0, "adamw_flat_dev_forms: unaligned buffer");
+  HRIEMO_CHECK(hyper != nullptr && state != nullptr, "adamw_flat_dev_forms: hyper and state are required");
+  long gsz = (n / 4 + 255) / 256;
+  if (gsz > 4096) gsz = 4096;
+  const FormTab ft = {(const long long*)spans, F};
+  const size_t lds = (size_t)F * sizeof(long long);
+  if (avg != nullptr) {
+    HRIEMO_CHECK(avg_state != nullptr, "adamw_flat_dev_forms: avg_state is required");
+    HRIEMO_CHECK(!ranges_overlap(avg, p, (size_t)n * 4) && !ranges_overlap(avg, g, (size_t)n * 4) && !ranges_overlap(avg, m, (size_t)n * 4) &&
+                     !ranges_overlap(avg, v, (size_t)n * 4), "adamw_flat_dev_forms: avg overlaps p, g, m or v");
+    hipLaunchKernelGGL(adamw_flat_dev_forms_kernel<true>, dim3((int)gsz), dim3(256), lds, st, p, g, m, v, n, hyper, state, avg, avg_state, ft);
+  } else {
+    hipLaunchKernelGGL(adamw_flat_dev_forms_kernel<false>, dim3((int)gsz), dim3(256), lds, st, p, g, m, v, n, hyper, state, (float*)nullptr,
+                       (const float*)nullptr, ft);
+  }
+  HRIEMO_LAUNCH_CHECK("adamw_flat_dev_forms_kernel");
+  return 0;
+}
+
+static int adamw_flat_groups_forms_launch(const char* who, float* p, const float* g, float* m, float* v, long n, const long long* seg,
+                                          const int* seg_group, const int* seg_unit, int S, const float* hyper, const float* state, int G,
+                                          const float* clip_state, int U, float* avg, const float* avg_state, const void* spans, int F,
+                                          hipStream_t st) {
+  const bool units = seg_unit != nullptr;
+  HRIEMO_CHECK(n > 0 && n % 4 == 0, "%s: n=%ld must be a positive multiple of 4", who, n);
+  HRIEMO_CHECK(p != nullptr && g != nullptr && m != nullptr && v != nullptr, "%s: p, g, m and v are required", who);
+  HRIEMO_CHECK(((uintptr_t)p % 16) == 0 && ((uintptr_t)g % 16) == 0 && ((uintptr_t)m % 16) == 0 && ((uintptr_t)v % 16) == 0 &&
+                   ((uintptr_t)avg % 16) == 0, "%s: unaligned buffer", who);
+  HRIEMO_CHECK(hyper != nullptr && state != nullptr, "%s: hyper and state are required", who);
+  HRIEMO_CHECK(G >= 1 && G <= AG_MAX_GROUPS, "%s: G=%d groups (1 .. %d)", who, G, (int)AG_MAX_GROUPS);
+  HRIEMO_CHECK(S >= 1 && S <= AG_MAX_SEGS, "%s: S=%d segments (1 .. %d)", who, S, (int)AG_MAX_SEGS);
+  HRIEMO_CHECK((long)S <= n / 4, "%s: S=%d segments over n=%ld elements: more segments than 16-byte vectors", who, S, n);
+  HRIEMO_CHECK(seg != nullptr && seg_group != nullptr && ((uintptr_t)seg % 8) == 0 && ((uintptr_t)seg_group % 4) == 0,
+               "%s: seg (int64 [S + 1], 8-byte aligned) and seg_group (int32 [S], 4-byte aligned) are required", who);
+  if (units) {
+    HRIEMO_CHECK(U >= 1 && U <= CU_MAX_UNITS && U <= S, "%s: U=%d units (1 .. %d, at most S=%d)", who, U, (int)CU_MAX_UNITS, S);
+    HRIEMO_CHECK(((uintptr_t)seg_unit % 4) == 0, "%s: seg_unit (int32 [S]) is not 4-byte aligned", who);
+    HRIEMO_CHECK(clip_state != nullptr && ((uintptr_t)clip_state % 4) == 0, "%s: clip_state (fp32 [U][2]) is required, 4-byte aligned", who);
+  } else {
+    U = 0;
+  }
+  if (avg != nullptr) {
+    HRIEMO_CHECK(avg_state != nullptr, "%s: avg_state is required", who);
+    HRIEMO_CHECK(!ranges_overlap(avg, p, (size_t)n * 4) && !ranges_overlap(avg, g, (size_t)n * 4) && !ranges_overlap(avg, m, (size_t)n * 4) &&
+                     !ranges_overlap(avg, v, (size_t)n * 4), "%s: avg overlaps p, g, m or v", who);
+  }
+  long gsz = (n / 4 + 255) / 256;
+  if (gsz > 4096) gsz = 4096;
+  const FormTab ft = {(const long long*)spans, F};
+  const size_t lds = (size_t)F * sizeof(long long) + (size_t)(S + 1) * sizeof(long long) + (size_t)G * 8 * sizeof(float) +
+                     (units ? (size_t)U * sizeof(float) + (size_t)S * 2 : 0) + (size_t)S;
+#define HRIEMO_FORMS_LAUNCH(AVG, UNITS)                                                                                              \
+  hipLaunchKernelGGL((adamw_flat_groups_forms_kernel<AVG, UNITS>), dim3((int)gsz), dim3(256), lds, st, p, g, m, v, n, seg, seg_group, \
+                     seg_unit, S, hyper, state, G, clip_state, U, avg, avg_state, ft)
+  if (units) {
+    if (avg != nullptr) HRIEMO_FORMS_LAUNCH(true, true); else HRIEMO_FORMS_LAUNCH(false, true);
+  } else {
+    if (avg != nullptr) HRIEMO_FORMS_LAUNCH(true, false); else HRIEMO_FORMS_LAUNCH(false, false);
+  }
+#undef HRIEMO_FORMS_LAUNCH
+  HRIEMO_LAUNCH_CHECK("adamw_flat_groups_forms_kernel");
+  return 0;
+}
+
+extern "C" int hriemo_adamw_flat_groups_forms(float* p, const float* g, float* m, float* v, long n, const long long* seg,
+                                              const int* seg_group, int S, const float* hyper, const float* state, int G, float* avg,
+                                              const float* avg_state, const void* spans, int F, hipStream_t st) {
+  if (form_tab_check("adamw_flat_groups_forms", spans, F)) return 1;
+  if (F == 0) return avg != nullptr ? hriemo_adamw_flat_groups_avg(p, g, m, v, n, seg, seg_group, S, hyper, state, G, avg, avg_state, st)
+                                    : hriemo_adamw_flat_groups(p, g, m, v, n, seg, seg_group, S, hyper, state, G, st);
+  return adamw_flat_groups_forms_launch("adamw_flat_groups_forms", p, g, m, v, n, seg, seg_group, nullptr, S, hyper, state, G, nullptr, 0,
+                                        avg, avg_state, spans, F, st);
+}
+
+extern "C" int hriemo_adamw_flat_units_forms(float* p, const float* g, float* m, float* v, long n, const long long* seg,
+                                             const int* seg_group, const int* seg_unit, int S, const float* hyper, const float* state, int G,
+                                             const float* clip_state, int U, float* avg, const float* avg_state, const void* spans, int F,
+                                             hipStream_t st) {
+  if (form_tab_check("adamw_flat_units_forms", spans, F)) return 1;
+  HRIEMO_CHECK(seg_unit != nullptr, "adamw_flat_units_forms: seg_unit is required");
+  if (F == 0) return adamw_flat_units_launch("adamw_flat_units_forms", p, g, m, v, n, seg, seg_group, seg_unit, S, hyper, state, G, clip_state, U,
+                                             avg, avg_state, st);
+  return adamw_flat_groups_forms_launch("adamw_flat_units_forms", p, g, m, v, n, seg, seg_group, seg_unit, S, hyper, state, G, clip_state, U,
+                                        avg, avg_state, spans, F, st);
+}
diff --git a/hri-emo_amd/csrc/rowops.hip b/hri-emo_amd/csrc/rowops.hip
--- a/hri-emo_amd/csrc/rowops.hip
+++ b/hri-emo_amd/csrc/rowops.hip
@@ -1,4 +1,5 @@
 #include "common.h"
+#include "forms.h"
 #include <string.h>
 #include <stdlib.h>
 
@@ -2118,9 +2119,17 @@
   if (threadIdx.x == 0) partial[blockIdx.x] = red[0] + red[1] + red[2] + red[3];
 }
 
-__global__ __launch_bounds__(256) void adamw_flat_kernel(float* __restrict__ p, const float* __restrict__ g, float* __restrict__ m,
-                                                         float* __restrict__ v, long n, float lr, float b1, float b2, float eps,
-                                                         float wd, float bc1, float bc2, float max_norm, const float* __restrict__ norm2) {
+template <bool FORMS>
+__device__ __forceinline__ void adamw_flat_body(float* __restrict__ p, const float* __restrict__ g, float* __restrict__ m,
+                                                float* __restrict__ v, long n, float lr, float b1, float b2, float eps,
+                                                float wd, float bc1, float bc2, float max_norm, const float* __restrict__ norm2,
+                                                const FormTab ft) {
+  extern __shared__ __attribute__((aligned(16))) long long form_lds[];
+  FormCur fc = {0, 0, 0ull, 0ull, 0, 0};
+  if (FORMS) {
+    form_stage(ft, form_lds);
+    __syncthreads();
+  }
   float coef = 1.f;
   if (max_norm > 0.f) coef = fminf(1.f, max_norm / (sqrtf(norm2[0]) + 1e-6f));
   const float step = lr / bc1, isb2 = 1.f / sqrtf(bc2);
@@ -2136,7 +2145,21 @@
       pp[e] -= step * mm[e] / (sqrtf(vv[e]) * isb2 + eps);
     }
     *(f32x4*)(p + i * 4) = pp; *(f32x4*)(m + i * 4) = mm; *(f32x4*)(v + i * 4) = vv;
-  }
+    if (FORMS) form_vec4(fc, ft, form_lds, i, n, pp);
+  }
+}
+
+__global__ __launch_bounds__(256) void adamw_flat_kernel(float* __restrict__ p, const float* __restrict__ g, float* __restrict__ m,
+                                                         float* __restrict__ v, long n, float lr, float b1, float b2, float eps,
+                                                         float wd, float bc1, float bc2, float max_norm, const float* __restrict__ norm2) {
+  adamw_flat_body<false>(p, g, m, v, n, lr, b1, b2, eps, wd, bc1, bc2, max_norm, norm2, FormTab{});
+}
+
+__global__ __launch_bounds__(256) void adamw_flat_forms_kernel(float* __restrict__ p, const float* __restrict__ g, float* __restrict__ m,
+                                                               float* __restrict__ v, long n, float lr, float b1, float b2, float eps,
+                                                               float wd, float bc1, float bc2, float max_norm, const float* __restrict__ norm2,
+                                                               const FormTab ft) {
+  adamw_flat_body<true>(p, g, m, v, n, lr, b1, b2, eps, wd, bc1, bc2, max_norm, norm2, ft);
 }
 
 extern "C" int hriemo_sumsq_f32(const float* x, long n, float* partial, int nblocks, hipStream_t st) {
@@ -2158,6 +2181,26 @@
   hipLaunchKernelGGL(adamw_flat_kernel, dim3((int)gsz), dim3(256), 0, st, p, g, m, v, n, lr, beta1, beta2, eps, weight_decay, bc1, bc2,
                      max_norm, norm2);
   HRIEMO_LAUNCH_CHECK("adamw_flat_kernel");
+  return 0;
+}
+
+extern "C" int hriemo_adamw_flat_forms(float* p, const float* g, float* m, float* v, long n, float lr, float beta1, float beta2, float eps,
+                                       float weight_decay, int step, float max_norm, const float* norm2, const void* spans, int F,
+                                       hipStream_t st) {
+  HRIEMO_CHECK(F >= 0 && F <= FORM_MAX_SPANS, "adamw_flat_forms: F=%d spans (0 .. %d)", F, (int)FORM_MAX_SPANS);
+  if (F == 0) return hriemo_adamw_flat(p, g, m, v, n, lr, beta1, beta2, eps, weight_decay, step, max_norm, norm2, st);
+  HRIEMO_CHECK(spans != nullptr && ((uintptr_t)spans % 8) == 0, "adamw_flat_forms: spans (int64 [F][6], hriemo_form_table_build) is required, 8-byte aligned");
+  HRIEMO_CHECK(p != nullptr && g != nullptr && m != nullptr && v != nullptr, "adamw_flat_forms: p, g, m and v are required");
+  HRIEMO_CHECK(n > 0 && n % 4 == 0 && step >= 1, "adamw_flat_forms: n=%ld must be a positive multiple of 4 and step >= 1", n);
+  HRIEMO_CHECK(((uintptr_t)p % 16) == 0 && ((uintptr_t)g % 16) == 0 && ((uintptr_t)m % 16) == 0 && ((uintptr_t)v % 16) == 0, "adamw_flat_forms: unaligned buffer");
+  HRIEMO_CHECK(max_norm <= 0.f || norm2 != nullptr, "adamw_flat_forms: clipping needs the squared gradient norm");
+  const float bc1 = 1.f - powf(beta1, (float)step), bc2 = 1.f - powf(beta2, (float)step);
+  long gsz = (n / 4 + 255) / 256;
+  if (gsz > 4096) gsz = 4096;
+  const FormTab ft = {(const long long*)spans, F};
+  hipLaunchKernelGGL(adamw_flat_forms_kernel, dim3((int)gsz), dim3(256), (size_t)F * sizeof(long long), st, p, g, m, v, n, lr, beta1, beta2, eps,
+                     weight_decay, bc1, bc2, max_norm, norm2, ft);
+  HRIEMO_LAUNCH_CHECK("adamw_flat_forms_kernel");
   return 0;
 }
 
diff --git a/hri-emo_amd/dp.py b/hri-emo_amd/dp.py
--- a/hri-emo_amd/dp.py
+++ b/hri-emo_amd/dp.py
@@ -545,6 +545,8 @@
 class DataParallelStep(_RaggedStep):
 
     _label = "packed step"
+    _formset = None
+    _forms_in_graph = False
 
     def __init__(self, model, loss_fn, group=None, bucket_bytes=32 << 20, overlap=True, comm_dtype=torch.float32, force_exchange=False,
                  launch_from="notify", force_queue=None):
@@ -778,6 +780,8 @@
             self._optimizer._upload_hyper()
         key = load((first, last))
         rec = self._packed_graph(key)
+        if self._formset is not None:
+            self._formset.sync("DataParallelStep.step_packed")
         rec.graph.replay()
         self._micro = 0 if last else self._micro + 1
         if last:
@@ -840,18 +844,33 @@
     def _capture_graph(self, seqs):
         from . import _ops
         collectives = self._exchange_in_graph
+        ctx = _ops.CTX
+        front = self._pb.front if self._pb is not None else None
+        accumulating = front is not None and front.accum > 1
+        log = _ops.FormLog() if (_ops.FORMS_IN_UPDATE and self._formset is None and not accumulating) else None
+        if self._formset is not None:
+            self._formset.sync("DataParallelStep (bucket capture)")
 
         def warm():
-            if self._act_log is not None:
-                with self._act_log.paused():
+            ctx.forms = log
+            try:
+                if self._act_log is not None:
+                    with self._act_log.paused():
+                        self._fwd_bwd(*self._static)
+                else:
                     self._fwd_bwd(*self._static)
-            else:
-                self._fwd_bwd(*self._static)
+            finally:
+                ctx.forms = None
             if collectives:
                 self.buckets.finish()
 
         def warmed():
             self._outputs = None
+            if log is not None:
+                self._formset = _ops.FormSet(log.take())
+                self._formset.attach()
+            if self._formset is not None:
+                ctx.owned = self._formset.owned
 
         def body():
             _ops.bump_seed_word(self._static[0].device)
@@ -862,11 +881,16 @@
             if self._optimizer is not None:
                 front = self._pb.front if self._pb is not None else None
                 ctl = front.ctl.dev if (front is not None and front.accum > 1) else None
+                fs = self._formset
+                self._forms_in_graph = fs is not None and fs.table_for(self._optimizer) is not None
                 self._optimizer._enqueue(ctl=ctl)
             return loss, None
 
-        return _record_graph(self._static[0].device, seqs, self._pb.pool if seqs is not None else None, warm, body, warmed,
-                             settle=0.25 if collectives else 0.0)
+        try:
+            return _record_graph(self._static[0].device, seqs, self._pb.pool if seqs is not None else None, warm, body, warmed,
+                                 settle=0.25 if collectives else 0.0)
+        finally:
+            ctx.owned = None
 
     def release_graph(self):
         was = self.captured
@@ -874,6 +898,9 @@
             torch.cuda.synchronize()
             self._record.release()
         self._release_buckets()
+        if self._formset is not None:
+            self._formset.release()
+        self._formset, self._forms_in_graph = None, False
         if was:
             self._record = self._pb = self._optimizer = None
 
@@ -887,6 +914,8 @@
         if self._optimizer is not None:
             from . import _ops
             _ops.bump_weights_epoch()
+            if self._formset is not None and self._forms_in_graph:
+                self._formset.restamp()
             self._optimizer._opt_called = True
 
     @_in_step_context
@@ -913,6 +942,8 @@
                 if s is not None and t is not None and s.data_ptr() != t.data_ptr():
                     s.copy_(t)
             rec = self._packed_graph(key) if pb is not None else self._record
+            if self._formset is not None:
+                self._formset.sync("DataParallelStep.step")
             rec.graph.replay()
             self._after_replay()
             return rec.loss
diff --git a/hri-emo_amd/optim.py b/hri-emo_amd/optim.py
--- a/hri-emo_amd/optim.py
+++ b/hri-emo_amd/optim.py
@@ -26,6 +26,8 @@
         self._partial = torch.empty(self.nblocks, dtype=torch.float32, device=flat_g.device)
         self._norm2 = torch.zeros(1, dtype=torch.float32, device=flat_g.device)
         self.steps = 0
+        self._forms = None
+        _ops.register_flat_master(self)
 
     @torch.no_grad()
     def step(self):
@@ -33,12 +35,29 @@
         n = g.numel()
         st = _stream()
         self.steps += 1
+        forms, table, current = _form_table(self)
         _lib.call("hriemo_sumsq_f32", _p(g), n, _p(self._partial), self.nblocks, st)
         _lib.call("hriemo_rowsum_f32", _p(self._partial), _p(self._norm2), 1, self.nblocks, st)
-        _lib.call("hriemo_adamw_flat", _p(self.flat_p), _p(g), _p(self.m), _p(self.v), n, self.lr, self.betas[0], self.betas[1],
-                  self.eps, self.wd, self.steps, self.max_norm if self.max_norm else 0.0, _p(self._norm2), st)
-        _ops.bump_weights_epoch()
+        if table is None:
+            _lib.call("hriemo_adamw_flat", _p(self.flat_p), _p(g), _p(self.m), _p(self.v), n, self.lr, self.betas[0], self.betas[1],
+                      self.eps, self.wd, self.steps, self.max_norm if self.max_norm else 0.0, _p(self._norm2), st)
+        else:
+            _lib.call("hriemo_adamw_flat_forms", _p(self.flat_p), _p(g), _p(self.m), _p(self.v), n, self.lr, self.betas[0], self.betas[1],
+                      self.eps, self.wd, self.steps, self.max_norm if self.max_norm else 0.0, _p(self._norm2), _p(table[0]), table[1], st)
+        _forms_updated(forms, table, current)
         return self._norm2.sqrt()
+
+
+def _form_table(opt):
+    forms = opt._forms
+    table = forms.table_for(opt) if forms is not None else None
+    return forms, table, (table is not None and forms.current())
+
+
+def _forms_updated(forms, table, current):
+    _ops.bump_weights_epoch()
+    if table is not None and current:
+        forms.restamp()
 
 
 MAX_GROUPS = 16
@@ -390,6 +409,8 @@
         self.health = health
         if health is not None:
             health._attach(self, {id(p): gi for gi, group in enumerate(self.param_groups) for p in group["params"]})
+        self._forms = None
+        _ops.register_flat_master(self)
 
     @staticmethod
     def _check_scalars(lr, betas, eps, weight_decay, where):
@@ -453,6 +474,8 @@
         g = self.buckets.flat
         n = g.numel()
         st = _stream()
+        table = _form_table(self)[1]
+        spans = (_p(table[0]), table[1]) if table is not None else None
         if self.clip != "global":
             G, S, U, C = len(self.param_groups), self._seg_group.numel(), self._unit_group.numel(), self._partial.numel()
             avg = self.averaging is not None
@@ -460,7 +483,11 @@
             _lib.call("hriemo_optim_finalize_units", _p(self._partial), C, _p(self._unit_chunks), _p(self._unit_group), U, _p(self._hyper), G,
                       _p(grad_scale), _p(found_inf), _p(self._state), _p(ctl), _p(self._clip_state),
                       _p(self._avg_hyper) if avg else None, _p(self._avg_state) if avg else None, st)
-            if avg:
+            if spans is not None:
+                _lib.call("hriemo_adamw_flat_units_forms", _p(self.flat_p), _p(g), _p(self.m), _p(self.v), n, _p(self._seg),
+                          _p(self._seg_group), _p(self._seg_unit), S, _p(self._hyper), _p(self._state), G, _p(self._clip_state), U,
+                          _p(self.avg) if avg else None, _p(self._avg_state) if avg else None, *spans, st)
+            elif avg:
                 _lib.call("hriemo_adamw_flat_units_avg", _p(self.flat_p), _p(g), _p(self.m), _p(self.v), n, _p(self._seg), _p(self._seg_group),
                           _p(self._seg_unit), S, _p(self._hyper), _p(self._state), G, _p(self._clip_state), U, _p(self.avg),
                           _p(self._avg_state), st)
@@ -473,7 +500,14 @@
             G = len(self.param_groups)
             _lib.call("hriemo_optim_finalize_avg", _p(self._partial), self.nblocks, _p(self._hyper), G, _p(grad_scale), _p(found_inf),
                       _p(self._state), _p(ctl), _p(self._avg_hyper), _p(self._avg_state), st)
-            if self._grouped:
+            if spans is not None and self._grouped:
+                _lib.call("hriemo_adamw_flat_groups_forms", _p(self.flat_p), _p(g), _p(self.m), _p(self.v), n, _p(self._seg),
+                          _p(self._seg_group), self._seg_group.numel(), _p(self._hyper), _p(self._state), G, _p(self.avg),
+                          _p(self._avg_state), *spans, st)
+            elif spans is not None:
+                _lib.call("hriemo_adamw_flat_dev_forms", _p(self.flat_p), _p(g), _p(self.m), _p(self.v), n, _p(self._hyper), _p(self._state),
+                          _p(self.avg), _p(self._avg_state), *spans, st)
+            elif self._grouped:
                 _lib.call("hriemo_adamw_flat_groups_avg", _p(self.flat_p), _p(g), _p(self.m), _p(self.v), n, _p(self._seg),
                           _p(self._seg_group), self._seg_group.numel(), _p(self._hyper), _p(self._state), G, _p(self.avg),
                           _p(self._avg_state), st)
@@ -485,8 +519,12 @@
             G = len(self.param_groups)
             _lib.call("hriemo_optim_finalize_groups", _p(self._partial), self.nblocks, _p(self._hyper), G, _p(grad_scale), _p(found_inf),
                       _p(self._state), _p(ctl), st)
-            _lib.call("hriemo_adamw_flat_groups", _p(self.flat_p), _p(g), _p(self.m), _p(self.v), n, _p(self._seg), _p(self._seg_group),
-                      self._seg_group.numel(), _p(self._hyper), _p(self._state), G, st)
+            if spans is not None:
+                _lib.call("hriemo_adamw_flat_groups_forms", _p(self.flat_p), _p(g), _p(self.m), _p(self.v), n, _p(self._seg),
+                          _p(self._seg_group), self._seg_group.numel(), _p(self._hyper), _p(self._state), G, None, None, *spans, st)
+            else:
+                _lib.call("hriemo_adamw_flat_groups", _p(self.flat_p), _p(g), _p(self.m), _p(self.v), n, _p(self._seg), _p(self._seg_group),
+                          self._seg_group.numel(), _p(self._hyper), _p(self._state), G, st)
             return
         if ctl is None:
             _lib.call("hriemo_optim_finalize", _p(self._partial), self.nblocks, _p(self._hyper), _p(grad_scale), _p(found_inf),
@@ -494,7 +532,11 @@
         else:
             _lib.call("hriemo_optim_finalize_ctl", _p(self._partial), self.nblocks, _p(self._hyper), _p(grad_scale), _p(found_inf),
                       _p(self._state), _p(ctl), st)
-        _lib.call("hriemo_adamw_flat_dev", _p(self.flat_p), _p(g), _p(self.m), _p(self.v), n, _p(self._hyper), _p(self._state), st)
+        if spans is not None:
+            _lib.call("hriemo_adamw_flat_dev_forms", _p(self.flat_p), _p(g), _p(self.m), _p(self.v), n, _p(self._hyper), _p(self._state),
+                      None, None, *spans, st)
+        else:
+            _lib.call("hriemo_adamw_flat_dev", _p(self.flat_p), _p(g), _p(self.m), _p(self.v), n, _p(self._hyper), _p(self._state), st)
 
     def _amp_word(self, name):
         t = getattr(self, name, None)
@@ -509,8 +551,9 @@
         if closure is not None:
             raise RuntimeError("DeviceAdamW.step() takes no closure: the gradients are read from the flat buffer")
         self._upload_hyper()
+        forms, table, current = _form_table(self)
         self._enqueue(self._amp_word("grad_scale"), self._amp_word("found_inf"))
-        _ops.bump_weights_epoch()
+        _forms_updated(forms, table, current)
 
     def zero_grad(self, set_to_none=True):
         self.buckets.zero_grad()
diff --git a/include/hriemo.h b/include/hriemo.h
--- a/include/hriemo.h
+++ b/include/hriemo.h
@@ -227,6 +227,18 @@
 int hriemo_adamw_flat_units_avg(float* p, const float* g, float* m, float* v, long n, const long long* seg, const int* seg_group,
                                 const int* seg_unit, int S, const float* hyper, const float* state, int G, const float* clip_state, int U,
                                 float* avg, const float* avg_state, hriemo_stream_t stream);
+int hriemo_form_table_build(const void* segs_host, int nseg, long n, void* spans_host, int max_spans, int* nspans);
+int hriemo_adamw_flat_forms(float* p, const float* g, float* m, float* v, long n, float lr, float beta1, float beta2, float eps,
+                            float weight_decay, int step, float max_norm, const float* norm2, const void* spans, int F,
+                            hriemo_stream_t stream);
+int hriemo_adamw_flat_dev_forms(float* p, const float* g, float* m, float* v, long n, const float* hyper, const float* state, float* avg,
+                                const float* avg_state, const void* spans, int F, hriemo_stream_t stream);
+int hriemo_adamw_flat_groups_forms(float* p, const float* g, float* m, float* v, long n, const long long* seg, const int* seg_group, int S,
+                                   const float* hyper, const float* state, int G, float* avg, const float* avg_state, const void* spans,
+                                   int F, hriemo_stream_t stream);
+int hriemo_adamw_flat_units_forms(float* p, const float* g, float* m, float* v, long n, const long long* seg, const int* seg_group,
+                                  const int* seg_unit, int S, const float* hyper, const float* state, int G, const float* clip_state,
+                                  int U, float* avg, const float* avg_state, const void* spans, int F, hriemo_stream_t stream);
 int hriemo_health_sweep(const float* g, const float* p, const float* m, const float* v, long n, const long long* chunks, int C,
                         const float* hyper, const float* state, int G, const int* ctl, int every, float* partial,
                         hriemo_stream_t stream);
diff --git a/scripts_dev/ab_forms_in_update.py b/scripts_dev/ab_forms_in_update.py
--- /dev/null
+++ b/scripts_dev/ab_forms_in_update.py
@@ -0,0 +1,62 @@
+import os, statistics, sys, torch
+sys.path.insert(0, os.path.dirname(os.path.dirname(os.path.abspath(__file__))))
+import hri_emo_amd as H
+from hri_emo_amd.dp import DataParallelStep
+from hri_emo_amd.optim import FusedClipAdamW
+from hri_emo_amd.train import fusion_step_loss
+import bench
+dev = torch.device("cuda", 0)
+args = sys.argv[1:]
+workload = "cfg2"
+if "--workload" in args:
+    i = args.index("--workload")
+    workload, args = args[i + 1], args[:i] + args[i + 2:]
+ROUNDS = int(args[0]) if len(args) > 0 else 7
+REPLAYS = int(args[1]) if len(args) > 1 else 30
+wl = bench.WORKLOADS[workload]
+bench.CFG = dict(wl["model"], beta_hidden=256, dropout=0.1)
+bench.T_A, bench.T_T = wl["T_a"], wl["T_t"]
+H.set_gemm_mode(wl["gemm"])
+steps = {}
+for arm in ("off", "on"):
+    H.set_forms_in_update(arm == "on")
+    torch.manual_seed(1234)
+    model = H.FusionWithEmotionDecoder(**bench.CFG).to(dev).train()
+    dp = DataParallelStep(model, fusion_step_loss, overlap=False)
+    opt = FusedClipAdamW(dp.buckets, lr=1e-4, weight_decay=1e-2, max_norm=5.0)
+    dp.set_global_batch(wl["batch"])
+    batch = bench.synth(wl["batch"], 0, dev)
+    dp.step(*batch)
+    dp.capture(*batch)
+    steps[arm] = (dp, opt, batch)
+H.set_forms_in_update(True)
+fs = steps["on"][0]._formset
+print(f"{workload}: the step owns {len(fs.stamps)} forms in {len(fs.segs)} segments ({sum(s[2] for s in fs.segs)} elements); "
+      f"form table: {fs.table[2] if fs.table else 0} spans", flush=True)
+res = {arm: [] for arm in steps}
+for rnd in range(ROUNDS):
+    for arm, (dp, opt, batch) in steps.items():
+        for _ in range(3): dp.step(*batch)
+        torch.cuda.synchronize()
+        e0, e1 = torch.cuda.Event(enable_timing=True), torch.cuda.Event(enable_timing=True)
+        e0.record()
+        for _ in range(REPLAYS): dp.step(*batch)
+        e1.record(); torch.cuda.synchronize()
+        res[arm].append(e0.elapsed_time(e1) / REPLAYS)
+for arm, ts in res.items():
+    print(f"{workload} forms_in_update {arm:3s} median {statistics.median(ts):.3f} ms  max-min {max(ts) - min(ts):.3f}  (" + " ".join(f"{x:.3f}" for x in ts) + ")", flush=True)
+d = statistics.median(res["on"]) - statistics.median(res["off"])
+print(f"on - off = {d * 1e3:+.1f} us; weights passes run by the 'on' arm: {fs.passes}", flush=True)
+res2 = {arm: [] for arm in steps}
+for rnd in range(ROUNDS):
+    for arm, (dp, opt, batch) in steps.items():
+        for _ in range(2): dp.step(*batch); opt.step()
+        torch.cuda.synchronize()
+        e0, e1 = torch.cuda.Event(enable_timing=True), torch.cuda.Event(enable_timing=True)
+        e0.record()
+        for _ in range(REPLAYS // 3): dp.step(*batch); opt.step()
+        e1.record(); torch.cuda.synchronize()
+        res2[arm].append(e0.elapsed_time(e1) / (REPLAYS // 3))
+for arm, ts in res2.items():
+    print(f"{workload} replay + opt.step() forms_in_update {arm:3s} median {statistics.median(ts):.3f} ms  max-min {max(ts) - min(ts):.3f}  (" + " ".join(f"{x:.3f}" for x in ts) + ")", flush=True)
+print(f"weights passes run by the 'on' arm in all: {fs.passes}", flush=True)
```

Result: no change. 8825 utterances/s (median of 6 runs) (+0.4%).
